# DS4SD/MarkushGrapher

Hardware: AMD Instinct MI355X
Metric: images/sec whole-node (greedy CXSMILES decode, 1024px crops, bs=32/GPU) (higher is better)
Workload: dtype bf16

## Files before the change

include/mgrapher.h:

```cpp
#ifndef MGRAPHER_H
#define MGRAPHER_H
#include <stddef.h>
#include <stdint.h>
#ifdef __cplusplus
extern "C" {
#endif

enum { MG_OK = 0, MG_E_SHAPE = -1, MG_E_ARG = -2, MG_E_STATE = -3, MG_E_HIP = -4, MG_E_UNSUPPORTED = -5,
       MG_E_WORKSPACE = -6, MG_E_KEY = -7, MG_E_INPUT = -8 };
enum { MG_KEY_IGNORED = 1 };
enum { MG_F32 = 0, MG_BF16 = 1 };

typedef struct mg_config {
    int vocab_size, d_model, d_kv, d_ff, num_layers, num_decoder_layers, num_heads;
    int relative_attention_num_buckets, relative_attention_max_distance;
    int max_2d_position_embeddings, image_size, patch_size, num_channels;
    int pad_token_id, eos_token_id, decoder_start_token_id;
    float layer_norm_epsilon;
    int max_decode_len;
    int tie_word_embeddings;
} mg_config;

typedef struct mg_model mg_model;

int mg_create(const mg_config* cfg, mg_model** out);
void mg_destroy(mg_model* m);
const char* mg_last_error(void);

size_t mg_weights_bytes(const mg_model* m);
int mg_bind_weights(mg_model* m, void* arena);
int mg_load_tensor(mg_model* m, void* stream, const char* hf_key, const void* src, int dtype, const int64_t* shape,
                   int ndim);
int mg_finalize(mg_model* m, void* stream);

int mg_clone(const mg_model* src, mg_model** out);

int mg_workspace_bytes(const mg_model* m, int B, int L, int num_beams, int max_length, int T, int M_e1, size_t* out_bytes);

int mg_encode(mg_model* m, void* stream, void* ws, size_t ws_bytes, const int64_t* input_ids, const float* bbox,
              const uint8_t* attention_mask, const float* pixel_values, const float* e1, int M_e1, int B, int L,
              float* enc_out, uint8_t* enc_mask);

int mg_decoder_forward(mg_model* m, void* stream, void* ws, size_t ws_bytes, const int64_t* decoder_input_ids,
                       const uint8_t* decoder_attention_mask, int B, int T, float* logits);

int mg_generate(mg_model* m, void* stream, void* ws, size_t ws_bytes, const int64_t* input_ids, const float* bbox,
                const uint8_t* attention_mask, const float* pixel_values, const float* e1 ,
                int M_e1, int B, int L, int num_beams, int max_length,
                int min_length, float length_penalty, int early_stopping, int64_t* out_ids, int* out_cols_host,
                float* out_scores, float* step_top2);

typedef struct mg_gen_opts {
    int num_return;
    float* token_scores;
    float* seq_scores;
    int32_t* beam_indices;
} mg_gen_opts;
int mg_generate_scored(mg_model* m, void* stream, void* ws, size_t ws_bytes, const int64_t* input_ids, const float* bbox,
                       const uint8_t* attention_mask, const float* pixel_values, const float* e1, int M_e1, int B, int L, int num_beams,
                       int max_length, int min_length, float length_penalty, int early_stopping, int64_t* out_ids, int* out_cols_host,
                       float* out_scores, float* step_top2, const mg_gen_opts* opts);


typedef struct mg_sample_opts {
    float temperature;
    int top_k;
    float top_p;
    uint64_t seed;
    const uint64_t* stream_ids;
    int num_return;
    float* token_scores;
} mg_sample_opts;
int mg_sampled_workspace_bytes(const mg_model* m, int B, int L, int num_return, int max_length, int M_e1, size_t* out_bytes);
int mg_generate_sampled(mg_model* m, void* stream, void* ws, size_t ws_bytes, const int64_t* input_ids, const float* bbox,
                        const uint8_t* attention_mask, const float* pixel_values, const float* e1, int M_e1, int B, int L, int max_length,
                        int min_length, int64_t* out_ids, int* out_cols_host, float* step_top2, const mg_sample_opts* opts);

int mg_stream_workspace_bytes(const mg_model* m, int chunk, int L, int slots, int pool_chunks, size_t* out_bytes);
int mg_generate_stream(mg_model* m, void* stream, void* ws, size_t ws_bytes, const int64_t* input_ids, const float* bbox,
                       const uint8_t* attention_mask, const float* pixel_values, int N, int L, int chunk, int slots, int pool_chunks,
                       int max_length, int min_length, int64_t* out_ids, int32_t* out_len, long* steps_host);
int mg_generate_stream_sampled(mg_model* m, void* stream, void* ws, size_t ws_bytes, const int64_t* input_ids, const float* bbox,
                               const uint8_t* attention_mask, const float* pixel_values, int N, int L, int chunk, int slots,
                               int pool_chunks, int max_length, int min_length, int64_t* out_ids, int32_t* out_len, long* steps_host,
                               const mg_sample_opts* opts);
int mg_stream_beam_workspace_bytes(const mg_model* m, int chunk, int L, int slots, int pool_chunks, int num_beams, int max_length, size_t* out_bytes);
int mg_generate_stream_beam(mg_model* m, void* stream, void* ws, size_t ws_bytes, const int64_t* input_ids, const float* bbox,
                            const uint8_t* attention_mask, const float* pixel_values, int N, int L, int chunk, int slots, int pool_chunks,
                            int num_beams, int max_length, int min_length, float length_penalty, int early_stopping, int64_t* out_ids,
                            int32_t* out_len, float* out_scores, long* steps_host);
int mg_generate_stream_scored(mg_model* m, void* stream, void* ws, size_t ws_bytes, const int64_t* input_ids, const float* bbox,
                              const uint8_t* attention_mask, const float* pixel_values, int N, int L, int chunk, int slots, int pool_chunks,
                              int max_length, int min_length, int64_t* out_ids, int32_t* out_len, long* steps_host, const mg_gen_opts* opts);
int mg_generate_stream_beam_scored(mg_model* m, void* stream, void* ws, size_t ws_bytes, const int64_t* input_ids, const float* bbox,
                                   const uint8_t* attention_mask, const float* pixel_values, int N, int L, int chunk, int slots, int pool_chunks,
                                   int num_beams, int max_length, int min_length, float length_penalty, int early_stopping, int64_t* out_ids,
                                   int32_t* out_len, long* steps_host, const mg_gen_opts* opts);
int mg_stream_encoder_mode(mg_model* m, int mode, const uint32_t* cu_mask, int nwords);

int mg_debug_decode_capture(mg_model* m, float* logits_capture, int capture_steps, const int64_t* forced_ids);

int mg_beam_reorder(void* stream, const void* kv_src, void* kv_dst, const int32_t* beam_idx, int layers, int rows,
                    int H, int t_cap, int t_used);

int mg_profile_cross_attention(mg_model* m, int every, int max_samples);
int mg_profile_read(mg_model* m, long* launches_host, double* total_ms_host, double* total_keys_host);
int mg_profile_read_overhead(mg_model* m, double* empty_ms_host);
int mg_profile_phases(mg_model* m, int enable);
int mg_profile_phases_read(mg_model* m, long* calls_host, double* enc_ms_host, double* dec_ms_host);
int mg_debug_bucket_table(const mg_model* m, int which, int* out_host, int n);

int mg_set_decode_graph(mg_model* m, int enable);
int mg_set_padding_semantics(mg_model* m, int per_image);
int mg_set_shared_gpu(mg_model* m, int shared);
int mg_set_cross_absorb(mg_model* m, int absorb, int key_splits);
int mg_set_beam_cross_absorb(mg_model* m, int absorb, int key_splits);
int mg_decode_graph_active(const mg_model* m);

typedef struct mg_dist mg_dist;
int mg_dist_unique_id(void* out, int bytes);
int mg_dist_create(const void* unique_id, int bytes, int rank, int world, mg_dist** out);
int mg_dist_allgather(mg_dist* d, void* stream, const void* send, void* recv, size_t bytes_per_rank);
void mg_dist_destroy(mg_dist* d);

size_t mg_preprocess_scratch_bytes(int B, int Hs, int Ws, int out_size);
int mg_preprocess_pages(void* stream, const uint8_t* pages_u8, int B, int Hs, int Ws, int out_size, float* pixel_values,
                        void* scratch, size_t scratch_bytes);

int mg_selftest(void* stream, void* scratch_256k, char* msg_host, int msg_len);

int mgk_pack_weight(void* stream, const void* src, int src_is_bf16, int N, int K, void* dst_pk, int Npad);
int mgk_rmsnorm_pack(void* stream, const float* h, const float* gain, void* x_pk, float* out_f32, int M, int d,
                     float eps, float scale);
int mgk_im2col_pack(void* stream, const float* pix, void* x_pk, int B, int C, int I, int ps);
int mgk_set_rows_split(int mode);
int mgk_set_resid_f16(int on);
int mgk_set_rows_ft2(int mode);
int mgk_set_rows_mt(int on);
int mgk_set_attention_qt(int qt);
int mgk_set_pp_parts(int mode);
int mgk_gemm_resid_mt(void* stream, const void* X_pk, const void* W_pk, float* h, const float* gain, float gscale, void* x_pk,
                      float* part, int M, int N, int K, const float* rs_part, int rs_nparts, float rs_inv_d, float rs_eps, int wide_tiles,
                      float* kpart, int* ticket);
int mgk_gemm(void* stream, int mode, int epi, const void* X_pk, const void* W_pk, int M, int N, int K, float* out_f32,
             int ldo, const float* bias, void* out_pk);
int mgk_gemm_norm(void* stream, int epi, const void* X_pk, const void* W_pk, int M, int N, int K, float* h_tiled, const float* gain,
                  void* out_pk, float* part, int part_ld, const float* rs_part, int rs_nparts, float rs_inv_d, float rs_eps);
int mgk_gemm_row_tiles(void* stream, int epi, const void* X_pk, const void* W_pk, int M, int N, int K, float* out_f32, const float* gain,
                       void* out_pk, float* part, int part_ld, const float* rs_part, int rs_nparts, float rs_inv_d, float rs_eps,
                       const uint8_t* row_mask, int* list_scratch);
int mgk_gemm_heads(void* stream, int mode, const void* X_pk, const void* W_pk, int M, int N, int K, void* p0, void* p1,
                   void* p2, int f0, int f1, int f2, int H, int S_in, int S_cap, const int* row_map, int pos);
int mgk_attention(void* stream, int mode, const void* Q, const void* K, const void* Vt, void* ctx_pk, int B, int H,
                  int Sq, int Sk, int Sq_cap, int Sk_cap, const uint8_t* kmask, const float* tab1, int tab1_len,
                  const float* tabh, const float* tabv, const double* cx, const double* cy, const int* bk1, const int* bkhv,
                  void* bidx_scratch);
int mgk_attention_enc_skip(void* stream, const void* Q, const void* K, const void* Vt, void* ctx_pk, int B, int H, int S, int S_cap,
                           const uint8_t* kmask, const float* tab1, const float* tabh, const float* tabv, const double* cx,
                           const double* cy, const int* bk1, const int* bkhv, void* bidx_scratch, int* kst_scratch,
                           uint8_t* qbv_scratch);
int mgk_attention_step(void* stream, const void* q, const void* Kc, const void* Vc, void* ctx_pk, int rows, int H,
                       int group, int cap, const int* len, int n_keys, const float* bias, const int* anc, int t);
int mgk_attention_step_ex(void* stream, const void* q, const void* Kc, const void* Vc, void* ctx_pk, int rows, int H, int group, int cap,
                          const int* len, int n_keys, const float* bias, const int* anc, int t, const int* t_dev, int t_off,
                          const int* pos_rows, const int* kv_owner, const int* live, const float* qrs_part, int qrs_nparts, float qrs_inv_d,
                          float qrs_eps, int ctx_ld, int ctx_col0, int one_wg_per_cu);
int mgk_attention_step_rope(void* stream, const float* qkv, int ld, const float* cs, const float* rs_part, int rs_nparts, float rs_inv_d,
                            float rs_eps, float qscale, void* Kc, void* Vc, void* ctx_pk, int rows, int H_kv, int group, int cap, int t,
                            const int* t_dev, int t_off, const int* pos_rows, const int* t_off_rows, const int* kv_owner, const int* live,
                            int ctx_ld, int ctx_col0);
int mgk_xattn(void* stream, const void* q, const float* wkv, const void* enc, const int* len, const int* kv_owner, int rows, int H, int d,
              int cap, int nsplit, int nstg, void* wk, void* wv, void* qx, void* part, float* ml, void* ctx_pk);
int mgk_xattn_beams(void* stream, const void* q, const float* wkv, const void* enc, const int* len, const int* kv_owner, const int* live,
                    int rows, int H, int d, int cap, int group, int nsplit, int nstg, int beams_per_wg, int nt, void* wk, void* wv, void* qx,
                    void* part, float* ml, void* ctx_pk);
int mgk_enc_rows(void* stream, const void* src_pk, const int* row_map, void* dst, int B, int rows_per_image, int cap, int d);
int mgk_embed_assemble(void* stream, void* meta_ws, const int64_t* input_ids, const float* bbox,
                       const uint8_t* attention_mask, const float* patch_emb, const void* tok_emb, const void* x_emb,
                       const void* y_emb, int B, int L, int P, int d, int n_side, int M2, int V, int S_cap,
                       float* hidden, double* cx, double* cy, uint8_t* mask, int* xrow, int* xlen, int* err);
size_t mgk_embed_meta_bytes(int B, int S_cap);
int mgk_greedy_select(void* stream, const float* logits, int rows, int V, int ldl, int eos, int pad, int min_len,
                      int64_t* next_ids, int64_t* out_ids, int max_len, int pos, int* unfinished, int* n_unfinished,
                      float* top2);

int mgk_sample_select(void* stream, const float* logits, int rows, int V, int ldl, int eos, int pad, int min_len, float temperature,
                      int top_k, float top_p, uint64_t seed, const uint64_t* stream_ids, int64_t* next_ids, int64_t* out_ids, int max_len,
                      int pos, int* unfinished, int* n_unfinished, float* token_scores, int ts_ld);
int mgk_philox(uint64_t seed, uint64_t stream_id, uint32_t pos, uint32_t* out_host);
typedef struct mgk_slot_table {
    int* pos; int* img; int* pool; int* ctr; int* out_len;
    int pool_cap, start_id;
    const int64_t* first_tok;
    int n_stop, stop[4], max_len, nsamp;
} mgk_slot_table;
typedef struct mgk_select_desc {
    int fused;
    const float* logits; int rows, V, ldl;
    int eos, pad, suppress_eos, n_eos_more, eos_more[3];
    int64_t* next_ids; int64_t* out_ids; int max_len, pos;
    const int* pos_dev;
    int min_len;
    int* unfinished; int* n_unfinished;
    float* top2;
    int* step_ctr;
    mgk_slot_table slots;
    const void* ptop; const float* stopv; int ntiles;
    const void* tok_emb; float* h; const float* gain; void* x_pk; void* x2_pk; int x2_ld, x2_col0, d; float eps;
    float* token_scores; int ts_ld;
} mgk_select_desc;
int mgk_select_ex(void* stream, const mgk_select_desc* s);
int mgk_sample_select_queue(void* stream, const float* logits, int rows, int V, int ldl, int eos, int pad, int min_len, float temperature,
                            int top_k, float top_p, uint64_t seed, const uint64_t* stream_ids, int64_t* next_ids, int64_t* out_ids, int max_len,
                            int pos, int* unfinished, int* n_unfinished, float* token_scores, int ts_ld, const mgk_slot_table* slots);
int mgk_slot_refill(void* stream, const mgk_slot_table* slots, int64_t* next_ids, int* unfinished, int rows);

int mgk_swin_attention(void* stream, const void* qkv_pk, void* ctx_pk, const float* table_HT, int B, int R, int C, int H, int w, int shift);
int mgk_swin_layernorm(void* stream, const float* h_in, int in_tiled, float* h_out, int h_out_norm, const float* w, const float* b,
                       const float* add_bias, void* x_pk, float* out_f32, int M, int C, int merge_R, float eps, int kaug);
int mgk_swin_resize(void* stream, const float* src, float* dst, int B, int C, int S, int I, const float* scale_host, const float* shift_host);
int mgk_swin_im2col_pack(void* stream, const float* pix, void* x_pk, int B, int C, int I, int ps, int Kp);
int mgk_swin_transpose(void* stream, const float* src, float* dst, int n, int H);

int mgk_ocr_layernorm_pack(void* stream, float* h, const float* w, const float* b, const float* add_bias, void* x_pk, float* out_f32, int M,
                           int d, int Kaug, float eps);
int mgk_ocr_gelu_pack(void* stream, const float* in, void* y_pk, int M, int N, int Kaug);
int mgk_ocr_silu_mul_pack(void* stream, const float* in, void* y_pk, int M, int I);
int mgk_ocr_silu_mul_rows(void* stream, const float* in, const float* rs_part, int rs_nparts, float rs_inv_d, float rs_eps, void* y_pk, int M,
                          int I);
int mgk_ocr_add_pos(void* stream, const float* patch, const void* pos, const int* pos_ids, const uint8_t* patch_mask, uint8_t* vmask,
                    float* hidden, int N, int P, int P_cap, int d);
int mgk_ocr_pixel_shuffle_pack(void* stream, const float* vis, void* x_pk, int N, int g, int P_cap, int e, int sf);
int mgk_ocr_merge_embed(void* stream, const int64_t* ids, const void* tok_emb, const float* feats, float* h, int B, int L, int T_cap, int d,
                        int V, int image_token, int per_seq, int* err);
int mgk_ocr_rope_heads(void* stream, const float* qkv, int B, int T, int T_cap, int H, int KV, float theta, void* Q, void* K, void* Vt, void* Kc,
                       void* Vc, int cap);
int mgk_ocr_rope_table(void* stream, float* cs, int positions, float theta);
int mgk_ocr_pack_aug(void* stream, const float* W, const float* bias, float scale, void* dst_pk, int row0, int N, int K, int Kaug, int Nfill,
                     int rstride);
int mgk_ocr_tile_f32(void* stream, const float* src, float* dst, int M, int d, int to_tiled);
int mgk_ocr_row_maps(void* stream, int* last_rows, int* all_rows, uint8_t* key_mask, int B, int T, int T_cap, const int* lens);
int mgk_ocr_len_delta(void* stream, const int* lens, int* delta, int N, int L, int* err);
int mgk_gemm_swiglu(void* stream, const void* X_pk, int x_kts, int x_k0, const void* W_pk, int M, int N, int K, const float* rs_part,
                    int rs_nparts, float rs_inv_d, float rs_eps, void* out_pk, int out_ld, int out_col0);
int mgk_rmsnorm_pack_tiled(void* stream, const float* h_tiled, const float* gain, void* x_pk, float* out_f32, int M, int d, float eps);
int mgk_embed_norm_rows(void* stream, const int64_t* ids, const void* tok_emb, float* h, const float* gain, void* x_pk, void* x2_pk, int x2_ld,
                        int x2_col0, int rows, int d, int V, int* err, float eps);

int mgk_gemm_splitk(void* stream, const void* X_pk, const void* W_pk, float* P, int M, int N, int K, int ldp,
                    size_t slab_stride, int KS);
int mgk_splitk_factor(int N, int K);
int mgk_gemm_set_variant(int v);
int mgk_gemm_resid(void* stream, const void* X_pk, const void* W_pk, float* h, const float* gain, float gscale, void* x_pk,
                   float* part, int M, int N, int K, const float* rs_part, int rs_nparts, float rs_inv_d, float rs_eps);
int mgk_gemm_pair(void* stream, const void* Wn_pk, const void* Wr_pk, const float* gain, int N2, int d, int inner, void* W2_pk,
                  float* scratch_f32, const void* xwin_pk, float* h, void* hb_out_pk, float* part, void* out2_pk, int M, int relu);
typedef struct mgk_resid_desc {
    const void* X; int x_kts, x_k0;
    const void* W;
    float* h;
    const float* gain; float gscale;
    void* x_pk; int x_ld, x_col0;
    void* x2_pk; int x2_ld, x2_col0;
    float* part;
    int M, N, K;
    const float* rs_part; int rs_nparts; float rs_inv_d, rs_eps;
    int wide_tiles, alone;
    float* kpart; int* ticket;
} mgk_resid_desc;
typedef struct mgk_proj_desc {
    const void* X; int x_kts, x_k0;
    const void* W;
    int N, K;
    const float* rs_part; int rs_nparts; float rs_inv_d, rs_eps;
    int both_halves;
    void* q;
    void* out_pk;
    float* out_f32; int ldo;
} mgk_proj_desc;
int mgk_gemm_resid_ex(void* stream, const mgk_resid_desc* r);
int mgk_gemm_pair_ex(void* stream, const mgk_resid_desc* r, const mgk_proj_desc* g, int epi);
int mgk_gemm_heads_step(void* stream, const void* X_pk, int x_kts, int x_k0, const void* W_pk, int M, int N, int K, void* p0, void* p1, void* p2,
                        int f0, int f1, int f2, int H, int S_cap, const float* rs_part, int rs_nparts, float rs_inv_d, float rs_eps, int pos,
                        const int* pos_dev, const int* pos_rows, int both_halves);
int mgk_lm_head_step(void* stream, const void* X_pk, const void* W_pk, float* P, int M, int N, int K, int ldp, const float* rs_part, int rs_nparts,
                     float rs_inv_d, float rs_eps, void* ptop, float* stopv, const int* stop4_host, int write_logits, int lse);
int mgk_add_norm_pack(void* stream, float* h, const float* P, int KS, int ldp, size_t slab_stride, const float* gain,
                      void* x_pk, int M, int d, float eps, float scale);
int mgk_relu_pack(void* stream, const float* P, int KS, int ldp, size_t slab_stride, void* y_pk, int M, int N);
size_t mgk_beam_state_bytes(int B, int K, int max_len);
float mgk_beam_length_divisor(int cur_len, float length_penalty);
int mgk_beam_init(void* stream, void* state, int B, int K, int max_len, int pad, int eos, int start, int64_t* next_ids, int* anc, int T_cap,
                  int* counters);
int mgk_beam_step(void* stream, void* state, const float* logits, int ldl, int V, int B, int K, int max_len, int cur_len, const int* tdev,
                  const float* div_table, int eos, int min_len, float length_penalty, int early_stopping, int64_t* next_ids, int* beam_idx,
                  int* counters, const int* slot_pos, const int* slot_live);
int mgk_beam_reorder_anc(void* stream, int* anc, const int* beam_idx, int rows, int t_written, const int* tdev, const int* counters,
                         const int* slot_pos, const int* slot_live);
int mgk_beam_finalize(void* stream, void* state, int B, int K, int max_len, int64_t* out_ids, int* out_cols, float* out_scores, int num_return,
                      int* beam_indices, float* token_scores);
int mgk_beam_slots_step(void* stream, void* state, int slots, int K, int max_len, int pad, int eos, int start, int early_stopping, int* pos,
                        int* img, int* pool, int* bpool, int* live, int* assign, int64_t* next_ids, int* anc, int T_cap, int pool_cap,
                        int64_t* out_ids, int* out_len, float* out_scores, int* ctr, int end_first, int num_return, int* beam_indices,
                        float* token_scores);

typedef struct mg_ocr_model mg_ocr_model;
typedef struct mg_ocr_config {
    int v_hidden, v_inter, v_layers, v_heads, image_size, patch_size;
    int t_hidden, t_inter, t_layers, t_heads, t_kv_heads, vocab;
    int scale_factor, image_token_id, eos_token_id, pad_token_id, tie_word_embeddings;
    float v_eps, rms_eps, rope_theta;
    int n_eos_extra, eos_extra[3];
} mg_ocr_config;

int mg_ocr_create(const mg_ocr_config* cfg, mg_ocr_model** out);
void mg_ocr_destroy(mg_ocr_model* m);
int mg_ocr_clone(const mg_ocr_model* src, mg_ocr_model** out);
size_t mg_ocr_weights_bytes(const mg_ocr_model* m);
int mg_ocr_bind_weights(mg_ocr_model* m, void* arena);
int mg_ocr_load_tensor(mg_ocr_model* m, void* stream, const char* hf_key, const void* src, int src_is_bf16, const int64_t* shape, int ndim);
int mg_ocr_finalize(mg_ocr_model* m, void* stream);
int mg_ocr_workspace_bytes(const mg_ocr_model* m, int B, int n_img, int L, int max_new_tokens, int full_logits, size_t* out_bytes);
int mg_ocr_image_features(mg_ocr_model* m, void* stream, void* ws, size_t ws_bytes, const float* pixel_values, const int32_t* patch_pos,
                          const uint8_t* patch_mask, int N, float* out);
int mg_ocr_forward(mg_ocr_model* m, void* stream, void* ws, size_t ws_bytes, const int64_t* input_ids, const float* pixel_values,
                   const int32_t* patch_pos, const uint8_t* patch_mask, int B, int n_img, int L, float* logits);
int mg_ocr_generate(mg_ocr_model* m, void* stream, void* ws, size_t ws_bytes, const int64_t* input_ids, const float* pixel_values,
                    const int32_t* patch_pos, const uint8_t* patch_mask, int B, int n_img, int L, int max_new_tokens, int64_t* out_ids,
                    int* out_cols_host, float* step_logits, int capture_steps);

int mg_ocr_stream_workspace_bytes(const mg_ocr_model* m, int N, int n_img, int L, int max_new_tokens, int slots, int chunk, size_t* out_bytes);
int mg_ocr_generate_stream(mg_ocr_model* m, void* stream, void* ws, size_t ws_bytes, const int64_t* input_ids, const float* pixel_values,
                           const int32_t* patch_pos, const uint8_t* patch_mask, int N, int n_img, int L, int max_new_tokens, int slots, int chunk,
                           int64_t* out_ids, int32_t* out_len, long* steps_host);
int mg_ocr_generate_stream_ragged(mg_ocr_model* m, void* stream, void* ws, size_t ws_bytes, const int64_t* input_ids, const int32_t* prompt_len,
                                  const float* pixel_values, const int32_t* patch_pos, const uint8_t* patch_mask, int N, int n_img, int L,
                                  int max_new_tokens, int slots, int chunk, int64_t* out_ids, int32_t* out_len, long* steps_host);

typedef struct mg_e1_model mg_e1_model;
typedef struct mg_e1_config {
    int image_size, patch_size, num_channels, embed_dim, n_stages;
    int depths[4], num_heads[4];
    int window_size, mlp_ratio;
    float layer_norm_eps;
    int n_proj, proj_dims[4], proj_act;
    int src_image_size;
    float pix_scale[3], pix_shift[3];
} mg_e1_config;

int mg_e1_create(const mg_e1_config* cfg, mg_e1_model** out);
void mg_e1_destroy(mg_e1_model* m);
size_t mg_e1_weights_bytes(const mg_e1_model* m);
int mg_e1_bind_weights(mg_e1_model* m, void* arena);
int mg_e1_load_tensor(mg_e1_model* m, void* stream, const char* key, const void* src, int src_is_bf16, const int64_t* shape, int ndim);
int mg_e1_finalize(mg_e1_model* m, void* stream);
int mg_e1_out_tokens(const mg_e1_model* m);
int mg_e1_workspace_bytes(const mg_e1_model* m, int B, size_t* out_bytes);
int mg_e1_encode(const mg_e1_model* m, void* stream, void* ws, size_t ws_bytes, const float* pixel_values, int B, float* e1_out,
                 float* features_out);
int mg_attach_e1(mg_model* m, const mg_e1_model* e1);

#ifdef __cplusplus
}
#endif
#endif
```

markushgrapher_amd/csrc/c_ops.hip:

```cpp
#include "mg_kernels.h"
#include "mg_swin.h"
#include "mg_ocr.h"
#include <stdlib.h>
#include "../../include/mgrapher.h"

using namespace mg;

extern "C" {

int mgk_pack_weight(void* stream, const void* src, int src_is_bf16, int N, int K, void* dst_pk, int Npad) {
    if ((K & 15) || (Npad & 31) || Npad < N) return MG_E_SHAPE;
    pack_weight(src, src_is_bf16, N, K, (uint16_t*)dst_pk, Npad, (mgStream_t)stream);
    return MG_OK;
}

int mgk_rmsnorm_pack(void* stream, const float* h, const float* gain, void* x_pk, float* out_f32, int M, int d,
                     float eps, float scale) {
    if (d & 15) return MG_E_SHAPE;
    rmsnorm_pack(h, gain, (uint16_t*)x_pk, out_f32, M, d, eps, scale, (mgStream_t)stream);
    return MG_OK;
}

int mgk_im2col_pack(void* stream, const float* pix, void* x_pk, int B, int C, int I, int ps) {
    if ((ps & 7) || (I % ps)) return MG_E_SHAPE;
    im2col_pack(pix, (uint16_t*)x_pk, B, C, I, ps, (mgStream_t)stream);
    return MG_OK;
}

int mgk_set_rows_split(int mode) { gemm_rows_set_split(mode); return MG_OK; }
int mgk_set_resid_f16(int on) { gemm_rows_set_resid_f16(on); return MG_OK; }
int mgk_set_rows_ft2(int mode) { gemm_rows_set_ft2(mode); return MG_OK; }
int mgk_gemm(void* stream, int mode, int epi, const void* X_pk, const void* W_pk, int M, int N, int K, float* out_f32,
             int ldo, const float* bias, void* out_pk) {
    const bool swin_epi = epi == EPI_PK_BIAS || epi == EPI_PK_GELU_ERF;
    if ((K & 63) || epi < 0 || (epi > EPI_PK && epi != EPI_PK_GELU && !swin_epi)) return MG_E_SHAPE;
    if (epi == EPI_PK_GELU && !(mode == 0 && gemm_has_gelu_epilogue(M, N))) return MG_E_UNSUPPORTED;
    if (swin_epi && mode != 0) return MG_E_UNSUPPORTED;
    if (swin_epi && ((N & 15) || !out_pk)) return MG_E_SHAPE;
    GemmArgs a{};
    a.X = (const uint16_t*)X_pk; a.W = (const uint16_t*)W_pk; a.M = M; a.N = N; a.K = K;
    a.out_f32 = out_f32; a.ldo = ldo; a.bias = bias; a.out_pk = (uint16_t*)out_pk;
    if (mode == 0) gemm(a, epi, (mgStream_t)stream); else gemm_rows(a, epi, (mgStream_t)stream);
    return MG_OK;
}

int mgk_gemm_norm(void* stream, int epi, const void* X_pk, const void* W_pk, int M, int N, int K, float* h_tiled, const float* gain,
                  void* out_pk, float* part, int part_ld, const float* rs_part, int rs_nparts, float rs_inv_d, float rs_eps) {
    const bool plain_resid = epi == EPI_RESID_NORM && !gain && !out_pk && !part && !rs_part;
    if ((K & 63) || (N & 31) || ((M & 31) && !plain_resid) || M < 1) return MG_E_SHAPE;
    GemmArgs a{};
    a.X = (const uint16_t*)X_pk; a.W = (const uint16_t*)W_pk; a.M = M; a.N = N; a.K = K;
    a.out_f32 = h_tiled; a.gain = gain; a.out_pk = (uint16_t*)out_pk; a.part = part; a.ldo = part_ld;
    a.rs = RowScale{rs_part, rs_nparts, rs_inv_d, rs_eps};
    gemm(a, epi, (mgStream_t)stream);
    return MG_OK;
}

int mgk_gemm_row_tiles(void* stream, int epi, const void* X_pk, const void* W_pk, int M, int N, int K, float* out_f32, const float* gain,
                       void* out_pk, float* part, int part_ld, const float* rs_part, int rs_nparts, float rs_inv_d, float rs_eps,
                       const uint8_t* row_mask, int* list_scratch) {
    if ((K & 63) || (N & 31) || (M & 31) || !row_mask || !list_scratch) return MG_E_SHAPE;
    row_tile_list(row_mask, M, list_scratch + 1, list_scratch, (mgStream_t)stream);
    GemmArgs a{};
    a.X = (const uint16_t*)X_pk; a.W = (const uint16_t*)W_pk; a.M = M; a.N = N; a.K = K;
    a.out_f32 = out_f32; a.gain = gain; a.out_pk = (uint16_t*)out_pk; a.part = part; a.ldo = (epi == EPI_RESID_NORM) ? part_ld : N;
    a.rs = RowScale{rs_part, rs_nparts, rs_inv_d, rs_eps};
    a.row_tiles = list_scratch + 1; a.n_row_tiles = list_scratch;
    gemm(a, epi, (mgStream_t)stream);
    return MG_OK;
}

int mgk_gemm_heads(void* stream, int mode, const void* X_pk, const void* W_pk, int M, int N, int K, void* p0, void* p1,
                   void* p2, int f0, int f1, int f2, int H, int S_in, int S_cap, const int* row_map, int pos) {
    if ((K & 63) || (N % (H * 64))) return MG_E_SHAPE;
    GemmArgs a{};
    a.X = (const uint16_t*)X_pk; a.W = (const uint16_t*)W_pk; a.M = M; a.N = N; a.K = K;
    a.heads.ptr[0] = (uint16_t*)p0; a.heads.ptr[1] = (uint16_t*)p1; a.heads.ptr[2] = (uint16_t*)p2;
    a.heads.fmt[0] = f0; a.heads.fmt[1] = f1; a.heads.fmt[2] = f2;
    a.heads.inner = H * 64; a.heads.H = H; a.heads.S_in = S_in; a.heads.S_cap = S_cap; a.heads.row_map = row_map;
    a.heads.pos = pos;
    if (mode == 0) gemm(a, EPI_HEADS, (mgStream_t)stream); else gemm_rows(a, EPI_HEADS, (mgStream_t)stream);
    return MG_OK;
}

int mgk_gemm_heads_step(void* stream, const void* X_pk, int x_kts, int x_k0, const void* W_pk, int M, int N, int K, void* p0, void* p1, void* p2,
                        int f0, int f1, int f2, int H, int S_cap, const float* rs_part, int rs_nparts, float rs_inv_d, float rs_eps, int pos,
                        const int* pos_dev, const int* pos_rows, int both_halves) {
    if (!X_pk || !W_pk) return MG_E_ARG;
    if (K < 64 || (K & 63) || H < 1 || N < H * 64 || (N % (H * 64)) || N > 3 * H * 64 || M < 1 || M > 256 || S_cap < 1) return MG_E_SHAPE;
    if (x_kts ? (x_k0 < 0 || x_k0 + (K >> 4) > x_kts) : x_k0 != 0) return MG_E_SHAPE;
    if (rs_part && (rs_nparts < 8 || (rs_nparts & 7))) return MG_E_SHAPE;
    void* const ptr[3] = {p0, p1, p2};
    const int fmt[3] = {f0, f1, f2};
    bool kv = false;
    for (int i = 0; i < 3; ++i) {
        if (fmt[i] != HF_NONE && fmt[i] != HF_STEP_Q && fmt[i] != HF_STEP_KV) return MG_E_UNSUPPORTED;
        if (i < N / (H * 64) && fmt[i] != HF_NONE && !ptr[i]) return MG_E_ARG;
        kv = kv || fmt[i] == HF_STEP_KV;
    }
    if (kv && !pos_dev && !pos_rows && (pos < 0 || pos >= S_cap)) return MG_E_SHAPE;
    GemmArgs a{};
    a.X = (const uint16_t*)X_pk; a.x_kts = x_kts; a.x_k0 = x_k0; a.W = (const uint16_t*)W_pk; a.M = M; a.N = N; a.K = K;
    for (int i = 0; i < 3; ++i) { a.heads.ptr[i] = (uint16_t*)ptr[i]; a.heads.fmt[i] = fmt[i]; }
    a.heads.inner = H * 64; a.heads.H = H; a.heads.S_in = M; a.heads.S_cap = S_cap;
    a.heads.pos = pos; a.heads.pos_dev = pos_dev; a.heads.pos_rows = pos_rows;
    a.rs = RowScale{rs_part, rs_nparts, rs_inv_d, rs_eps};
    a.both_halves = both_halves;
    gemm_rows(a, EPI_HEADS, (mgStream_t)stream);
    return MG_OK;
}

int mgk_attention(void* stream, int mode, const void* Q, const void* K, const void* Vt, void* ctx_pk, int B, int H,
                  int Sq, int Sk, int Sq_cap, int Sk_cap, const uint8_t* kmask, const float* tab1, int tab1_len,
                  const float* tabh, const float* tabv, const double* cx, const double* cy, const int* bk1, const int* bkhv,
                  void* bidx_scratch) {
    if ((Sq_cap & 31) || (Sk_cap & 63) || Sk > Sk_cap || Sq > Sq_cap || mode < 0 || mode > 2) return MG_E_SHAPE;
    AttnArgs a{};
    a.Q = (const uint16_t*)Q; a.K = (const uint16_t*)K; a.Vt = (const uint16_t*)Vt; a.ctx = (uint16_t*)ctx_pk;
    a.B = B; a.H = H; a.Sq = Sq; a.Sk = Sk; a.Sq_cap = Sq_cap; a.Sk_cap = Sk_cap; a.mode = mode; a.kmask = kmask;
    a.tab1 = tab1; a.tab1_len = tab1_len; a.tabh = tabh; a.tabv = tabv;
    if (mode == ATT_ENC) {
        if (!bidx_scratch || !bk1 || !bkhv || !cx || !cy || Sq_cap != Sk_cap) return MG_E_ARG;
        bias_index((uint16_t*)bidx_scratch, cx, cy, kmask, bk1, bkhv, B, Sk, Sk_cap, (mgStream_t)stream);
        a.bidx = (const uint16_t*)bidx_scratch;
        a.bk1 = bk1;
    }
    attention(a, (mgStream_t)stream);
    return MG_OK;
}

int mgk_attention_enc_skip(void* stream, const void* Q, const void* K, const void* Vt, void* ctx_pk, int B, int H, int S, int S_cap,
                           const uint8_t* kmask, const float* tab1, const float* tabh, const float* tabv, const double* cx,
                           const double* cy, const int* bk1, const int* bkhv, void* bidx_scratch, int* kst_scratch,
                           uint8_t* qbv_scratch) {
    if ((S_cap & 63) || S > S_cap || !kmask || !bidx_scratch || !kst_scratch || !qbv_scratch) return MG_E_ARG;
    AttnArgs a{};
    a.Q = (const uint16_t*)Q; a.K = (const uint16_t*)K; a.Vt = (const uint16_t*)Vt; a.ctx = (uint16_t*)ctx_pk;
    a.B = B; a.H = H; a.Sq = S; a.Sk = S; a.Sq_cap = S_cap; a.Sk_cap = S_cap; a.mode = ATT_ENC; a.kmask = kmask;
    a.tab1 = tab1; a.tab1_len = 32; a.tabh = tabh; a.tabv = tabv;
    bias_index((uint16_t*)bidx_scratch, cx, cy, kmask, bk1, bkhv, B, S, S_cap, (mgStream_t)stream);
    attn_lists(kmask, B, S, S_cap, kst_scratch, qbv_scratch, (mgStream_t)stream);
    a.bidx = (const uint16_t*)bidx_scratch; a.bk1 = bk1; a.kst = kst_scratch; a.qbv = qbv_scratch;
    attention(a, (mgStream_t)stream);
    return MG_OK;
}

int mgk_attention_step(void* stream, const void* q, const void* Kc, const void* Vc, void* ctx_pk, int rows, int H,
                       int group, int cap, const int* len, int n_keys, const float* bias, const int* anc, int t) {
    if (group < 1 || group > 8) return MG_E_SHAPE;
    AttnStepArgs a{};
    a.q = (const uint16_t*)q; a.Kc = (const uint16_t*)Kc; a.Vc = (const uint16_t*)Vc; a.ctx = (uint16_t*)ctx_pk;
    a.rows = rows; a.H = H; a.group = group; a.cap = cap; a.len = len; a.n_keys = n_keys; a.bias = bias; a.anc = anc;
    a.t = t;
    attention_step(a, (mgStream_t)stream);
    return MG_OK;
}

int mgk_attention_step_ex(void* stream, const void* q, const void* Kc, const void* Vc, void* ctx_pk, int rows, int H, int group, int cap,
                          const int* len, int n_keys, const float* bias, const int* anc, int t, const int* t_dev, int t_off,
                          const int* pos_rows, const int* kv_owner, const int* live, const float* qrs_part, int qrs_nparts, float qrs_inv_d,
                          float qrs_eps, int ctx_ld, int ctx_col0, int one_wg_per_cu) {
    if (group < 1 || group > 8 || rows < 1) return MG_E_SHAPE;
    if (ctx_ld ? ((ctx_ld & 15) || ctx_col0 < 0 || ctx_col0 + H * 64 > ctx_ld) : ctx_col0 != 0) return MG_E_SHAPE;
    if (one_wg_per_cu) attention_step_allow_shared();
    AttnStepArgs a{};
    a.q = (const uint16_t*)q; a.Kc = (const uint16_t*)Kc; a.Vc = (const uint16_t*)Vc; a.ctx = (uint16_t*)ctx_pk;
    a.rows = rows; a.H = H; a.group = group; a.cap = cap; a.len = len; a.n_keys = n_keys; a.bias = bias; a.anc = anc;
    a.t = t; a.t_dev = t_dev; a.t_off = t_off; a.pos_rows = pos_rows; a.kv_owner = kv_owner; a.live = live;
    a.qrs = RowScale{qrs_part, qrs_nparts, qrs_inv_d, qrs_eps};
    a.ctx_ld = ctx_ld; a.ctx_col0 = ctx_col0; a.one_wg_per_cu = one_wg_per_cu;
    attention_step(a, (mgStream_t)stream);
    return MG_OK;
}

int mgk_attention_step_rope(void* stream, const float* qkv, int ld, const float* cs, const float* rs_part, int rs_nparts, float rs_inv_d,
                            float rs_eps, float qscale, void* Kc, void* Vc, void* ctx_pk, int rows, int H_kv, int group, int cap, int t,
                            const int* t_dev, int t_off, const int* pos_rows, const int* t_off_rows, const int* kv_owner, const int* live,
                            int ctx_ld, int ctx_col0) {
    if (group < 1 || group > 8 || group == 5 || group == 7 || rows < 1) return MG_E_SHAPE;
    if (!qkv || !cs || ld < (group + 2) * H_kv * 64 || (ld & 3)) return MG_E_ARG;
    if (ctx_ld ? ((ctx_ld & 15) || ctx_col0 < 0 || ctx_col0 + H_kv * group * 64 > ctx_ld) : ctx_col0 != 0) return MG_E_SHAPE;
    AttnStepArgs a{};
    a.Kc = (const uint16_t*)Kc; a.Vc = (const uint16_t*)Vc; a.Kc_w = (uint16_t*)Kc; a.Vc_w = (uint16_t*)Vc; a.ctx = (uint16_t*)ctx_pk;
    a.rows = rows; a.H = H_kv; a.group = group; a.cap = cap; a.n_keys = t + 1; a.t = t; a.t_dev = t_dev; a.t_off = t_off;
    a.pos_rows = pos_rows; a.t_off_rows = t_off_rows; a.kv_owner = kv_owner; a.live = live;
    a.rope.qkv = qkv; a.rope.ld = ld; a.rope.cs = cs; a.rope.rs = RowScale{rs_part, rs_nparts, rs_inv_d, rs_eps}; a.rope.qscale = qscale;
    a.ctx_ld = ctx_ld; a.ctx_col0 = ctx_col0;
    attention_step(a, (mgStream_t)stream);
    return MG_OK;
}

#ifdef MG_TOOLS
int mgk_attention_step_trace(void* stream, const void* q, const void* Kc, const void* Vc, void* ctx_pk, int rows, int H, int cap,
                             const int* len, long long* trace) {
    AttnStepArgs a{};
    a.q = (const uint16_t*)q; a.Kc = (const uint16_t*)Kc; a.Vc = (const uint16_t*)Vc; a.ctx = (uint16_t*)ctx_pk;
    a.rows = rows; a.H = H; a.group = 1; a.cap = cap; a.len = len;
    attention_step_trace(a, trace, (mgStream_t)stream);
    return MG_OK;
}
#endif

int mgk_xattn(void* stream, const void* q, const float* wkv, const void* enc, const int* len, const int* kv_owner, int rows, int H, int d,
              int cap, int nsplit, int nstg, void* wk, void* wv, void* qx, void* part, float* ml, void* ctx_pk) {
    if (!xattn_supported(d, H) || nsplit < 1 || nsplit > 4 || (nstg != 3 && nstg != 4)) return MG_E_UNSUPPORTED;
    mgStream_t st = (mgStream_t)stream;
    xattn_pack_weights(wkv, (uint16_t*)wk, (uint16_t*)wv, H, d, st);
    xattn_stream_prepare(d, nstg);
    XAttnArgs a{};
    a.q = (const uint16_t*)q; a.qx = (uint16_t*)qx; a.wk = (const uint16_t*)wk; a.wv = (const uint16_t*)wv; a.enc = (const uint16_t*)enc;
    a.len = len; a.kv_owner = kv_owner; a.part = (uint16_t*)part; a.ml = ml; a.ctx = (uint16_t*)ctx_pk;
    a.rows = rows; a.H = H; a.d = d; a.cap = cap; a.nsplit = nsplit; a.nstg = nstg;
    { const char* e = getenv("MG_XATTN_NT"); a.nt = e ? atoi(e) : 1; }
    xattn_expand(a, st);
    xattn_stream(a, st);
    xattn_contract(a, st);
    return MG_OK;
}
int mgk_xattn_beams(void* stream, const void* q, const float* wkv, const void* enc, const int* len, const int* kv_owner, const int* live,
                    int rows, int H, int d, int cap, int group, int nsplit, int nstg, int beams_per_wg, int nt, void* wk, void* wv, void* qx,
                    void* part, float* ml, void* ctx_pk) {
    if (!xattn_supported(d, H) || nsplit < 1 || nsplit > 4 || (nstg != 3 && nstg != 4)) return MG_E_UNSUPPORTED;
    if (group < 1 || rows < group || rows % group != 0 || beams_per_wg < 0 || !xattn_beams_bp(d, nstg, beams_per_wg)) return MG_E_UNSUPPORTED;
    mgStream_t st = (mgStream_t)stream;
    xattn_pack_weights(wkv, (uint16_t*)wk, (uint16_t*)wv, H, d, st);
    xattn_beams_prepare(d);
    XAttnArgs a{};
    a.q = (const uint16_t*)q; a.qx = (uint16_t*)qx; a.wk = (const uint16_t*)wk; a.wv = (const uint16_t*)wv; a.enc = (const uint16_t*)enc;
    a.len = len; a.kv_owner = kv_owner; a.live = live; a.part = (uint16_t*)part; a.ml = ml; a.ctx = (uint16_t*)ctx_pk;
    a.rows = rows; a.H = H; a.d = d; a.cap = cap; a.nsplit = nsplit; a.nstg = nstg; a.nt = nt ? 1 : 0; a.group = group; a.bpw = beams_per_wg;
    xattn_expand(a, st);
    xattn_stream_beams(a, st);
    xattn_contract(a, st);
    return MG_OK;
}
int mgk_enc_rows(void* stream, const void* src_pk, const int* row_map, void* dst, int B, int rows_per_image, int cap, int d) {
    enc_rows((const uint16_t*)src_pk, row_map, (uint16_t*)dst, B, rows_per_image, cap, d, (mgStream_t)stream);
    return MG_OK;
}

size_t mgk_embed_meta_bytes(int B, int S_cap) { return embed_meta_bytes(B, S_cap); }

int mgk_embed_assemble(void* stream, void* meta_ws, const int64_t* input_ids, const float* bbox,
                       const uint8_t* attention_mask, const float* patch_emb, const void* tok_emb, const void* x_emb,
                       const void* y_emb, int B, int L, int P, int d, int n_side, int M2, int V, int S_cap,
                       float* hidden, double* cx, double* cy, uint8_t* mask, int* xrow, int* xlen, int* err) {
    if (S_cap < L + P || (d & 3) || P != n_side * n_side) return MG_E_SHAPE;
    EmbedArgs a{};
    a.input_ids = input_ids; a.bbox = bbox; a.attn_mask = attention_mask; a.patch_emb = patch_emb;
    a.tok_emb = (const uint16_t*)tok_emb; a.x_emb = (const uint16_t*)x_emb; a.y_emb = (const uint16_t*)y_emb;
    a.B = B; a.L = L; a.P = P; a.d = d; a.n_side = n_side; a.M2 = M2; a.V = V; a.S_cap = S_cap;
    a.hidden = hidden; a.cx = cx; a.cy = cy; a.mask = mask; a.xrow = xrow; a.xlen = xlen; a.err = err;
    embed_assemble(a, meta_ws, (mgStream_t)stream);
    return MG_OK;
}

int mgk_greedy_select(void* stream, const float* logits, int rows, int V, int ldl, int eos, int pad, int min_len,
                      int64_t* next_ids, int64_t* out_ids, int max_len, int pos, int* unfinished, int* n_unfinished,
                      float* top2) {
    ArgmaxArgs a{};
    a.logits = logits; a.rows = rows; a.V = V; a.ldl = ldl; a.eos = eos; a.pad = pad; a.min_len = min_len;
    a.next_ids = next_ids; a.out_ids = out_ids; a.max_len = max_len; a.pos = pos; a.unfinished = unfinished;
    a.n_unfinished = n_unfinished; a.top2 = top2;
    mg_memset_async(n_unfinished, 0, sizeof(int), (mgStream_t)stream);
    greedy_select(a, (mgStream_t)stream);
    return MG_OK;
}

int mgk_greedy_select_scored(void* stream, const float* logits, int rows, int V, int ldl, int eos, int pad, int min_len,
                             int64_t* next_ids, int64_t* out_ids, int max_len, int pos, int* unfinished, int* n_unfinished,
                             float* token_scores, int ts_ld) {
    ArgmaxArgs a{};
    a.logits = logits; a.rows = rows; a.V = V; a.ldl = ldl; a.eos = eos; a.pad = pad; a.min_len = min_len;
    a.next_ids = next_ids; a.out_ids = out_ids; a.max_len = max_len; a.pos = pos; a.unfinished = unfinished;
    a.n_unfinished = n_unfinished; a.token_scores = token_scores; a.ts_ld = ts_ld;
    mg_memset_async(n_unfinished, 0, sizeof(int), (mgStream_t)stream);
    greedy_select(a, (mgStream_t)stream);
    return MG_OK;
}

int mgk_sample_select(void* stream, const float* logits, int rows, int V, int ldl, int eos, int pad, int min_len, float temperature,
                      int top_k, float top_p, uint64_t seed, const uint64_t* stream_ids, int64_t* next_ids, int64_t* out_ids, int max_len,
                      int pos, int* unfinished, int* n_unfinished, float* token_scores, int ts_ld) {
    if (!logits || !next_ids || !out_ids || !unfinished || !n_unfinished || rows < 1 || ldl < V || (ldl & 3)) return MG_E_ARG;
    if (!(temperature > 0.f) || top_k < 0 || !(top_p >= 0.f)) return MG_E_ARG;
    if (!sample_select_supported(V)) return MG_E_UNSUPPORTED;
    SampleArgs a{};
    a.logits = logits; a.rows = rows; a.V = V; a.ldl = ldl; a.eos = eos; a.pad = pad; a.min_len = min_len;
    a.temperature = temperature; a.top_k = top_k; a.top_p = top_p; a.seed = seed; a.stream_ids = stream_ids;
    a.next_ids = next_ids; a.out_ids = out_ids; a.max_len = max_len; a.pos = pos; a.unfinished = unfinished;
    a.n_unfinished = n_unfinished; a.token_scores = token_scores; a.ts_ld = ts_ld;
    mg_memset_async(n_unfinished, 0, sizeof(int), (mgStream_t)stream);
    sample_select(a, (mgStream_t)stream);
    return MG_OK;
}

static SlotTable slot_table(const mgk_slot_table* t) {
    SlotTable s{};
    if (!t) return s;
    s.pos = t->pos; s.img = t->img; s.pool = t->pool; s.ctr = t->ctr; s.out_len = t->out_len; s.pool_cap = t->pool_cap; s.start_id = t->start_id;
    s.first_tok = t->first_tok; s.n_stop = t->n_stop; s.max_len = t->max_len; s.nsamp = t->nsamp;
    for (int k = 0; k < 4; ++k) s.stop[k] = t->stop[k];
    return s;
}
int mgk_select_ex(void* stream, const mgk_select_desc* s) {
    if (!s || !s->next_ids || !s->out_ids || !s->unfinished) return MG_E_ARG;
    const bool queue = s->slots.pos != nullptr;
    if (s->fused && queue) return MG_E_ARG;
    if (queue ? (!s->slots.img || !s->slots.ctr || !s->slots.out_len) : !s->n_unfinished) return MG_E_ARG;
    if (s->n_eos_more < 0 || s->n_eos_more > 3) return MG_E_ARG;
    if (s->rows < 1 || s->rows > 256 || s->V < 1 || s->max_len < 1 || s->pos < 0) return MG_E_SHAPE;
    if (s->token_scores && (s->ts_ld < s->max_len - 1 || (!queue && !s->pos_dev && s->pos < 1))) return MG_E_SHAPE;
    if (s->fused) {
        if (!s->ptop || !s->stopv || !s->tok_emb || !s->gain || !s->h || !s->x_pk) return MG_E_ARG;
        if (s->d < 16 || s->d > 2048 || (s->d & 15) || s->ntiles != (s->V + 31) / 32) return MG_E_SHAPE;
        if (s->pad < 0 || s->pad >= s->V) return MG_E_ARG;
        if (s->x2_pk && ((s->x2_ld & 15) || s->x2_col0 < 0 || (s->x2_col0 & 7) || s->x2_col0 + s->d > s->x2_ld)) return MG_E_SHAPE;
    } else {
        if (!s->logits) return MG_E_ARG;
        if (s->ldl < s->V || (s->ldl & 3)) return MG_E_SHAPE;
    }
    ArgmaxArgs a{};
    a.logits = s->logits; a.rows = s->rows; a.V = s->V; a.ldl = s->ldl; a.eos = s->eos; a.pad = s->pad; a.suppress_eos = s->suppress_eos;
    a.n_eos_more = s->n_eos_more;
    for (int k = 0; k < 3; ++k) a.eos_more[k] = s->eos_more[k];
    a.next_ids = s->next_ids; a.out_ids = s->out_ids; a.max_len = s->max_len; a.pos = s->pos; a.pos_dev = s->pos_dev; a.min_len = s->min_len;
    a.unfinished = s->unfinished; a.n_unfinished = s->n_unfinished; a.top2 = s->top2; a.step_ctr = s->step_ctr;
    if (queue) a.slots = slot_table(&s->slots);
    a.ptop = (const float4*)s->ptop; a.stopv = s->stopv; a.ntiles = s->ntiles; a.tok_emb = (const uint16_t*)s->tok_emb; a.h = s->h;
    a.gain = s->gain; a.x_pk = (uint16_t*)s->x_pk; a.x2_pk = (uint16_t*)s->x2_pk; a.x2_ld = s->x2_ld; a.x2_col0 = s->x2_col0; a.d = s->d;
    a.eps = s->eps; a.token_scores = s->token_scores; a.ts_ld = s->ts_ld;
    if (s->fused) greedy_select_fused(a, (mgStream_t)stream); else greedy_select(a, (mgStream_t)stream);
    return MG_OK;
}
// ... 412 lines not shown
```

markushgrapher_amd/csrc/k_gemm.hip:

```cpp
#include "k_gemm_epi.h"
#include <atomic>

namespace mg {

constexpr int GB_M = 128, GB_N = 128, GB_K = 64;
constexpr int GB_STAGE_BYTES = (GB_M + GB_N) / 32 * (GB_K / 16) * TILE_BYTES;

template <int EPI>
__global__ __launch_bounds__(256) void gemm_big_kernel(GemmArgs a) {
    MG_DYN_SMEM(smem);
    const int tid = threadIdx.x, lane = tid & 63, w = tid >> 6;
    const int nbn = (a.N + GB_N - 1) / GB_N;
    const int nbm = (a.M + GB_M - 1) / GB_M;
    int bid = blockIdx.x;
    const int nblk = nbm * nbn;
    if ((nblk & 7) == 0) bid = (bid & 7) * (nblk >> 3) + (bid >> 3);
    const int bm = bid / nbn, bn = bid - bm * nbn;
    const int mt32 = (a.M + 31) >> 5, nt32 = (a.N + 31) >> 5, kt16 = a.K >> 4;
    const int nks = a.K / GB_K;

    const char* src[8];
#pragma unroll
    for (int i = 0; i < 8; ++i) {
        const int f = w * 8 + i, ff = f & 15, rt = ff >> 2, kt = ff & 3;
// ... 172 lines not shown
                tile_epilogue<EPI, false>(a, acc[i][j], m0, n0, lane);
            } else if constexpr (EPI == EPI_HEADS) {
                if (tor) tile_epilogue<EPI_HEADS, true, true>(a, acc[i][j], m0, n0, lane, 3, rsv[i]);
                else tile_epilogue<EPI_HEADS, false, true>(a, acc[i][j], m0, n0, lane, 3, rsv[i]);
            } else if constexpr (EPI != EPI_RESID_NORM) {
                tile_epilogue<EPI, true, true>(a, acc[i][j], m0, n0, lane, 3, rsv[i]);
            }
        }
}



template <int EPI, int TI, int XP = 0>
__global__ __launch_bounds__(512) void gemm_xl_kernel(GemmArgs a) {
    MG_DYN_SMEM(smem);
    constexpr int BM = 64 * TI, XT = 2 * TI;
    constexpr int FRAGS = (XT + 8) * 4;
    constexpr int STAGE_BYTES = FRAGS * TILE_BYTES;
    constexpr int PER_WAVE = (FRAGS + 7) / 8;
    const int tid = threadIdx.x, lane = tid & 63, w = tid >> 6;
    const int nbn = (a.N + GX_N - 1) / GX_N;
    const int n_list = a.row_tiles ? *a.n_row_tiles : 0;
    const int M_run = a.row_tiles ? n_list * 32 : a.M;
    const int nbm = (M_run + BM - 1) / BM;
    int bid = blockIdx.x;
    const int nblk = nbm * nbn;
    if (bid >= nblk) return;
    if ((nblk & 7) == 0) bid = (bid & 7) * (nblk >> 3) + (bid >> 3);
    const int bm = bid / nbn, bn = bid - bm * nbn;
    const int mt32 = (a.M + 31) >> 5, nt32 = (a.N + 31) >> 5;
    const int nks = a.K / GX_K;

    const char* src[PER_WAVE];
#pragma unroll
    for (int i = 0; i < PER_WAVE; ++i) {
        int f = w * PER_WAVE + i;
        f = f < FRAGS ? f : FRAGS - 1;
        const bool isW = f >= 4 * XT;
        const int ff = isW ? f - 4 * XT : f, rt = ff >> 2, kt = ff & 3;
        int trow = isW ? (bn * 8 + rt) : (bm * XT + rt);
        if (!isW && a.row_tiles) trow = a.row_tiles[trow < n_list ? trow : n_list - 1];
        const int tmax = isW ? nt32 - 1 : mt32 - 1;
        trow = trow < tmax ? trow : tmax;
        src[i] = (const char*)((isW ? a.W : a.X) + pk_tile_off(trow, kt, a.K)) + lane * 16;
    }
    const mg_lds_t sm0 = mg_lds_addr(smem);
    auto stage = [&](int buf, int ks) {
#pragma unroll
        for (int i = 0; i < PER_WAVE; ++i)
            if (w * PER_WAVE + i < FRAGS)
                glds16_async_lds(src[i] + (size_t)ks * (4 * TILE_BYTES), sm0 + buf * STAGE_BYTES + (w * PER_WAVE + i) * TILE_BYTES);
    };

    const int wr = w >> 2, wc = w & 3;
    const int m0w = bm * BM + wr * (32 * TI), n0w = bn * GX_N + wc * 64;
    bool tor;
    if (EPI == EPI_F32_STORE || EPI == EPI_F32_RESID) tor = false;
    else if (EPI == EPI_HEADS) tor = !heads_region_is_T(a.heads, n0w < a.N ? n0w : 0);
    else tor = true;

    f32x16 acc[TI][2];
#pragma unroll
    for (int i = 0; i < TI; ++i)
#pragma unroll
        for (int j = 0; j < 2; ++j) acc[i][j] = acc_zero();

    struct Frags { mg_raw16 x[TI], w[2]; };
    const mg_lds_t lx0 = sm0 + lane * 16 + wr * (TI * 4 * TILE_BYTES);
    const mg_lds_t lw0 = sm0 + lane * 16 + (4 * XT + wc * 8) * TILE_BYTES;
    auto rd = [&](int buf, auto ktc, Frags& f) {
        constexpr int kt = (XP & 1) ? 0 : decltype(ktc)::value;
        const mg_lds_t lx = lx0 + buf * STAGE_BYTES, lw = lw0 + buf * STAGE_BYTES;
        lds_rd16_async<(0 * 4 + kt) * TILE_BYTES>(f.w[0], lw);
        lds_rd16_async<(1 * 4 + kt) * TILE_BYTES>(f.w[1], lw);
        lds_rd16_async<(0 * 4 + kt) * TILE_BYTES>(f.x[0], lx);
        lds_rd16_async<(1 * 4 + kt) * TILE_BYTES>(f.x[1], lx);
        lds_rd16_async<(2 * 4 + kt) * TILE_BYTES>(f.x[2], lx);
        lds_rd16_async<(3 * 4 + kt) * TILE_BYTES>(f.x[3], lx);
        if constexpr (TI > 4) lds_rd16_async<(4 * 4 + kt) * TILE_BYTES>(f.x[TI - 1], lx);
    };
    auto landed = [&](Frags& f) {
        MG_WAIT_LGKM_TIE(0, f.w[0]);
        MG_TIE(f.w[1]);
#pragma unroll
        for (int i = 0; i < TI; ++i) MG_TIE(f.x[i]);
    };
    auto mm = [&](const Frags& f) {
        uint4 xw[2], xx[TI];
#pragma unroll
        for (int j = 0; j < 2; ++j) xw[j] = raw16_get(f.w[j]);
#pragma unroll
        for (int i = 0; i < TI; ++i) xx[i] = raw16_get(f.x[i]);
        if (tor) {
#pragma unroll
            for (int i = 0; i < TI; ++i)
#pragma unroll
                for (int j = 0; j < 2; ++j) acc[i][j] = mfma32(xw[j], xx[i], acc[i][j]);
        } else {
#pragma unroll
            for (int i = 0; i < TI; ++i)
#pragma unroll
                for (int j = 0; j < 2; ++j) acc[i][j] = mfma32(xx[i], xw[j], acc[i][j]);
        }
    };
    Frags fa, fb;
    using K0 = std::integral_constant<int, 0>; using K1 = std::integral_constant<int, 1>;
    using K2 = std::integral_constant<int, 2>; using K3 = std::integral_constant<int, 3>;
    stage(0, 0);
    MG_WAIT_VMCNT(0);
    MG_BARRIER_RAW();
    if (nks > 1) stage(1, 1);
    rd(0, K0{}, fa);
    for (int ks = 0; ks < nks; ++ks) {
        const int cur = ks & 1;
        landed(fa);
        rd(cur, K1{}, fb);
        MG_SCHED_FENCE();
        mm(fa);
        MG_SCHED_FENCE();
        landed(fb);
        rd(cur, K2{}, fa);
        MG_SCHED_FENCE();
        mm(fb);
        MG_SCHED_FENCE();
        landed(fa);
        rd(cur, K3{}, fb);
        MG_SCHED_FENCE();
        mm(fa);
        MG_SCHED_FENCE();
        landed(fb);
        if (ks + 1 < nks) {
            MG_WAIT_VMCNT(0);
            MG_BARRIER_RAW();
            if (ks + 2 < nks && !(XP & 2)) stage(cur, ks + 2);
            rd(cur ^ 1, K0{}, fa);
        }
        MG_SCHED_FENCE();
        mm(fb);
        MG_SCHED_FENCE();
    }

    int mrow[TI];
#pragma unroll
    for (int i = 0; i < TI; ++i) {
        if (a.row_tiles) {
            const int e = bm * XT + wr * TI + i;
            mrow[i] = e < n_list ? a.row_tiles[e] * 32 : a.M;
        } else {
            mrow[i] = m0w + 32 * i;
        }
    }
    xl_epilogue<EPI, TI, XP>(a, acc, mrow, n0w, tor, lane);
}
template <int EPI, int TI>
static void launch_xl(const GemmArgs& a, mgStream_t stream) {
    constexpr int BM = 64 * TI;
    const int nblk = ((a.M + BM - 1) / BM) * ((a.N + GX_N - 1) / GX_N);
    const size_t sh = (size_t)2 * (2 * TI + 8) * 4 * TILE_BYTES;
    static bool once = false;
    if (!once) { MG_SET_MAX_SMEM((&gemm_xl_kernel<EPI, TI>), sh); once = true; }
#ifdef MG_TOOLS
    if constexpr (EPI == EPI_PK && TI == 5) {
        static int xp = -1;
        if (xp < 0) { const char* e = getenv("MG_GEMM_EXP"); xp = e ? atoi(e) : 0; }
        if (xp) {
#define MG_XP(N) case N: { static bool o = false; if (!o) { MG_SET_MAX_SMEM((&gemm_xl_kernel<EPI, TI, N>), sh); o = true; } \
                             MG_LAUNCH((gemm_xl_kernel<EPI, TI, N>), dim3(nblk), dim3(512), sh, stream, a); } break;
            switch (xp) { MG_XP(1) MG_XP(2) MG_XP(3) MG_XP(4) MG_XP(5) MG_XP(6) default: MG_XP(7) }
#undef MG_XP
            return;
        }
    }
#endif
    MG_LAUNCH((gemm_xl_kernel<EPI, TI>), dim3(nblk), dim3(512), sh, stream, a);
}

template <int EPI>
static void launch_wide(const GemmArgs& a, mgStream_t stream) {
    const int nblk = ((a.M + GW_M - 1) / GW_M) * ((a.N + GW_N - 1) / GW_N);
    const size_t sh = (size_t)GW_STAGES * GW_STAGE_BYTES;
    static bool once = false;
    if (!once) { MG_SET_MAX_SMEM(&gemm_wide_kernel<EPI>, sh); once = true; }
    MG_LAUNCH((gemm_wide_kernel<EPI>), dim3(nblk), dim3(512), sh, stream, a);
}

static std::atomic<int> g_gemm_variant{3};
void gemm_set_variant(int v) { g_gemm_variant = v; }

bool gemm_has_gelu_epilogue(int M, int N) { return g_gemm_variant >= 2 && M >= 320 && N >= GX_N; }

void gemm(const GemmArgs& a, int epi, mgStream_t stream) {
    static bool env_read = false;
    if (!env_read) { env_read = true; if (const char* e = getenv("MG_GEMM_VARIANT")) g_gemm_variant = atoi(e); }
    const int gv = g_gemm_variant;
    static int small_env = -1;
    if (small_env < 0) { const char* e = getenv("MG_GEMM_SMALL"); small_env = e ? atoi(e) : 256; if (small_env == 1) small_env = 256; }
    const long tiles_xl = (long)((a.M + 319) / 320) * ((a.N + GX_N - 1) / GX_N);
    const bool small = gv == 3 && small_env && tiles_xl < small_env && epi != EPI_PK_GELU && !a.row_tiles && !a.part && !a.gain && !a.rs.part;
    if (!small && (gv == 3 || gv == 5 || gv == 6) && a.M >= 320 && a.N >= GX_N) {
        if (gemm_pp(a, epi, gv == 5 ? 4 : 5, stream)) return;
    }
    if (!small && gv >= 2 && a.M >= 320 && a.N >= GX_N) {
        const bool five = gv >= 3;
        const bool four = gv == 2;
        if (five) {
            switch (epi) {
                case EPI_F32_STORE: launch_xl<EPI_F32_STORE, 5>(a, stream); break;
                case EPI_F32_RESID: launch_xl<EPI_F32_RESID, 5>(a, stream); break;
                case EPI_PK_RELU: launch_xl<EPI_PK_RELU, 5>(a, stream); break;
                case EPI_PK_GELU: launch_xl<EPI_PK_GELU, 5>(a, stream); break;
                case EPI_PK: launch_xl<EPI_PK, 5>(a, stream); break;
                case EPI_PK_BIAS: launch_xl<EPI_PK_BIAS, 5>(a, stream); break;
                case EPI_PK_GELU_ERF: launch_xl<EPI_PK_GELU_ERF, 5>(a, stream); break;
                case EPI_RESID_NORM: launch_xl<EPI_RESID_NORM, 5>(a, stream); break;
                default: launch_xl<EPI_HEADS, 5>(a, stream); break;
            }
            return;
        }
        if (four) {
            switch (epi) {
                case EPI_F32_STORE: launch_xl<EPI_F32_STORE, 4>(a, stream); break;
                case EPI_F32_RESID: launch_xl<EPI_F32_RESID, 4>(a, stream); break;
                case EPI_PK_RELU: launch_xl<EPI_PK_RELU, 4>(a, stream); break;
                case EPI_PK_GELU: launch_xl<EPI_PK_GELU, 4>(a, stream); break;
                case EPI_PK: launch_xl<EPI_PK, 4>(a, stream); break;
                case EPI_PK_BIAS: launch_xl<EPI_PK_BIAS, 4>(a, stream); break;
                case EPI_PK_GELU_ERF: launch_xl<EPI_PK_GELU_ERF, 4>(a, stream); break;
                case EPI_RESID_NORM: launch_xl<EPI_RESID_NORM, 4>(a, stream); break;
                default: launch_xl<EPI_HEADS, 4>(a, stream); break;
            }
            return;
        }
    }
    const long tiles_w = (long)((a.M + GW_M - 1) / GW_M) * ((a.N + GW_N - 1) / GW_N);
    if (gv >= 1 && a.M >= GW_M && !(small && tiles_w < 96)) {
        switch (epi) {
            case EPI_F32_STORE: launch_wide<EPI_F32_STORE>(a, stream); break;
            case EPI_F32_RESID: launch_wide<EPI_F32_RESID>(a, stream); break;
            case EPI_PK_RELU: launch_wide<EPI_PK_RELU>(a, stream); break;
            case EPI_PK: launch_wide<EPI_PK>(a, stream); break;
            case EPI_PK_BIAS: launch_wide<EPI_PK_BIAS>(a, stream); break;
            case EPI_PK_GELU_ERF: launch_wide<EPI_PK_GELU_ERF>(a, stream); break;
            case EPI_RESID_NORM: launch_wide<EPI_RESID_NORM>(a, stream); break;
            default: launch_wide<EPI_HEADS>(a, stream); break;
        }
        return;
    }
    const int nblk = ((a.M + GB_M - 1) / GB_M) * ((a.N + GB_N - 1) / GB_N);
    const dim3 grid(nblk), block(256);
    const size_t sh = 2 * GB_STAGE_BYTES;
    switch (epi) {
        case EPI_F32_STORE: MG_LAUNCH((gemm_big_kernel<EPI_F32_STORE>), grid, block, sh, stream, a); break;
        case EPI_F32_RESID: MG_LAUNCH((gemm_big_kernel<EPI_F32_RESID>), grid, block, sh, stream, a); break;
        case EPI_PK_RELU: MG_LAUNCH((gemm_big_kernel<EPI_PK_RELU>), grid, block, sh, stream, a); break;
        case EPI_PK: MG_LAUNCH((gemm_big_kernel<EPI_PK>), grid, block, sh, stream, a); break;
        case EPI_PK_BIAS: MG_LAUNCH((gemm_big_kernel<EPI_PK_BIAS>), grid, block, sh, stream, a); break;
        case EPI_PK_GELU_ERF: MG_LAUNCH((gemm_big_kernel<EPI_PK_GELU_ERF>), grid, block, sh, stream, a); break;
        case EPI_RESID_NORM: MG_LAUNCH((gemm_big_kernel<EPI_RESID_NORM>), grid, block, sh, stream, a); break;
        default: MG_LAUNCH((gemm_big_kernel<EPI_HEADS>), grid, block, sh, stream, a); break;
    }
}

static std::atomic<int> g_rows_split_mode{-1};
void gemm_rows_set_split(int mode) { g_rows_split_mode = mode; }
static int rows_split_tiles(int mt, size_t weight_elems) {
    static bool env_read = false;
    if (!env_read) { env_read = true; if (const char* e = getenv("MG_ROWS_SPLIT")) g_rows_split_mode = atoi(e); }
    if (mt <= 1 || g_rows_split_mode == 0) return mt;
    const bool small = weight_elems * sizeof(uint16_t) <= ((size_t)4 << 20);
    return (g_rows_split_mode == 1 || (g_rows_split_mode < 0 && small)) ? 1 : mt;
}
template <int EPI>
MG_DEV void shift_rows(GemmArgs& a, int rt) {
    if (rt == 0) return;
    const int xkts = a.x_kts ? a.x_kts : (a.K >> 4);
    a.X += (size_t)rt * xkts * TILE_ELEMS;
    if (a.out_f32) a.out_f32 += (size_t)rt * 32 * a.ldo;
    if (a.out_pk) a.out_pk += (size_t)rt * ((EPI == EPI_PK_SWIGLU ? (a.out_ld ? a.out_ld : a.N >> 1) : a.N) >> 4) * TILE_ELEMS;
    if constexpr (EPI == EPI_HEADS) {
#pragma unroll
        for (int ri = 0; ri < 3; ++ri) {
            if (!a.heads.ptr[ri]) continue;
            if (a.heads.fmt[ri] == HF_STEP_Q) a.heads.ptr[ri] += (size_t)rt * 32 * a.heads.H * 64;
            else if (a.heads.fmt[ri] == HF_STEP_KV && !a.heads.row_map) a.heads.ptr[ri] += (size_t)rt * 32 * a.heads.H * (size_t)a.heads.S_cap * 64;
        }
        if (a.heads.row_map) a.heads.row_map += 32 * rt;
        if (a.heads.pos_rows) a.heads.pos_rows += 32 * rt;
    }
    if (a.rs.part) a.rs.part += (size_t)rt * 32 * a.rs.nparts;
    a.M -= 32 * rt;
}
MG_DEV void shift_rows(ResidArgs& a, int rt) {
    if (rt == 0) return;
    const int xkts = a.x_kts ? a.x_kts : (a.K >> 4);
    a.X += (size_t)rt * xkts * TILE_ELEMS;
    a.h += (size_t)rt * 32 * a.N;
    if (a.x_pk) a.x_pk += (size_t)rt * ((a.x_ld ? a.x_ld : a.N) >> 4) * TILE_ELEMS;
    if (a.x2_pk) a.x2_pk += (size_t)rt * ((a.x2_ld ? a.x2_ld : a.N) >> 4) * TILE_ELEMS;
    if (a.part) a.part += (size_t)rt * 32 * (a.N >> 3);
    if (a.rs.part) a.rs.part += (size_t)rt * 32 * a.rs.nparts;
    a.M -= 32 * rt;
}

template <int EPI, int MT, bool HALF, int NW, int U>
MG_DEV void rows_block(const GemmArgs& a, int bid, char* smem) {
    const int tid = threadIdx.x, lane = tid & 63, w = tid >> 6;
    const int nt = HALF ? (bid >> 1) : bid;
    const int sub = HALF ? (bid & 1) : 0;
    const bool wvalid = !HALF || (((lane & 31) >> 4) == sub);
    const uint4 zero4 = make_uint4(0, 0, 0, 0);
    const int kt16 = a.K >> 4;
    const int per = (kt16 + NW - 1) / NW;
    const int k0 = w * per, k1 = (k0 + per) < kt16 ? (k0 + per) : kt16;
    constexpr bool TOR = !(EPI == EPI_F32_STORE || EPI == EPI_F32_RESID);
    float* rsl = (float*)(smem + NW * 16 * 64 * sizeof(float));
    const char* wp = (const char*)(a.W + pk_tile_off(nt, 0, a.K)) + lane * 16;
    const int xkts = a.x_kts ? a.x_kts : kt16;
    const char* xp = (const char*)a.X + ((size_t)a.x_k0 * TILE_BYTES + lane * 16);
    int kt = k0;
    uint4 wf[U];
    const bool first_full = kt + U <= k1;
    if (first_full) {
#pragma unroll
        for (int u = 0; u < U; ++u) wf[u] = wvalid ? ld16_stream(wp + (size_t)(kt + u) * TILE_BYTES) : zero4;
    }
    if (TOR) block_row_scales(a.rs, a.M, 32 * MT, rsl, tid, NW * 64);

    f32x16 acc[MT];
#pragma unroll
    for (int i = 0; i < MT; ++i) acc[i] = acc_zero();
    for (bool first = true; kt + U <= k1; kt += U, first = false) {
        if (!first) {
#pragma unroll
            for (int u = 0; u < U; ++u) wf[u] = wvalid ? ld16_stream(wp + (size_t)(kt + u) * TILE_BYTES) : zero4;
        }
#pragma unroll
        for (int u = 0; u < U; ++u) {
#pragma unroll
            for (int i = 0; i < MT; ++i) {
                const uint4 xf = ld16(xp + ((size_t)i * xkts + (kt + u)) * TILE_BYTES);
                acc[i] = TOR ? mfma32(wf[u], xf, acc[i]) : mfma32(xf, wf[u], acc[i]);
            }
        }
    }
    for (; kt < k1; ++kt) {
        const uint4 wf = wvalid ? ld16_stream(wp + (size_t)kt * TILE_BYTES) : zero4;
#pragma unroll
        for (int i = 0; i < MT; ++i) {
            const uint4 xf = ld16(xp + ((size_t)i * xkts + kt) * TILE_BYTES);
            acc[i] = TOR ? mfma32(wf, xf, acc[i]) : mfma32(xf, wf, acc[i]);
        }
    }
    float* slab = (float*)smem;
#pragma unroll
    for (int i = 0; i < MT; ++i) {
#pragma unroll
        for (int r = 0; r < 16; ++r) slab[(w * 16 + r) * 64 + lane] = acc[i][r];
        __syncthreads();
        if constexpr (TOR && !HALF) {
#pragma unroll
            for (int q = 0; q < 2; ++q) {
                if (((2 * i + q) % NW) == w) {
                    f32x16 s = acc_zero();
#pragma unroll
                    for (int r = 8 * q; r < 8 * q + 8; ++r) {
                        float v = 0.f;
#pragma unroll
                        for (int ww = 0; ww < NW; ++ww) v += slab[(ww * 16 + r) * 64 + lane];
                        s[r] = v * rsl[32 * i + (lane & 31)];
                    }
                    tile_epilogue<EPI, TOR>(a, s, 32 * i, 32 * nt, lane, 1 << q);
                }
            }
        } else if ((i % NW) == w) {
            f32x16 s;
#pragma unroll
            for (int r = 0; r < 16; ++r) {
                float v = 0.f;
#pragma unroll
                for (int ww = 0; ww < NW; ++ww) v += slab[(ww * 16 + r) * 64 + lane];
                s[r] = TOR ? v * rsl[32 * i + (lane & 31)] : v;
            }
            tile_epilogue<EPI, TOR>(a, s, 32 * i, 32 * nt, lane, HALF ? (1 << sub) : 3);
        }
        __syncthreads();
    }
}
template <int EPI, int MT, int NW, int U, int FT = 1>
MG_DEV void rows_block16(const GemmArgs& a, int bid, char* smem) {
    static_assert(EPI == EPI_PK || EPI == EPI_PK_RELU || EPI == EPI_HEADS || EPI == EPI_PK_SWIGLU || EPI == EPI_F32_STORE,
                  "half-tile form: packed, per-head, SwiGLU and plain fp32 epilogues");
    static_assert(FT == 1 || MT > 1, "both halves per workgroup: several row tiles only");
    const int tid = threadIdx.x, lane = tid & 63, w = tid >> 6;
    const int r16 = lane & 15, kg = lane >> 4;
    const int nt = FT == 2 ? bid : bid >> 1, sub0 = FT == 2 ? 0 : (bid & 1);
    const int kt16 = a.K >> 4, kp = kt16 >> 1;
    const int per = (kp + NW - 1) / NW;
    const int p0 = w * per, p1 = (p0 + per) < kp ? (p0 + per) : kp;
    float* rsl = (float*)(smem + NW * 8 * FT * 64 * sizeof(float));
    const size_t lane_off = (size_t)(kg >> 1) * TILE_BYTES + (size_t)(kg & 1) * 512;
    const char* wp = (const char*)(a.W + pk_tile_off(nt, 0, a.K)) + lane_off + (size_t)(16 * sub0 + r16) * 16;
    const int xkts = a.x_kts ? a.x_kts : kt16;
    const char* xp = (const char*)a.X + (size_t)a.x_k0 * TILE_BYTES + lane_off + (size_t)r16 * 16;
    RsRegs rsr;
    rs_issue(a.rs, a.M, 32 * MT, tid, NW * 64, rsr);
    int p = p0;
    uint4 wf[U][FT];
    constexpr bool XPF = MT == 1;
    uint4 xf[XPF ? U : 1][2];
    if (p + U <= p1) {
#pragma unroll
        for (int u = 0; u < U; ++u)
#pragma unroll
            for (int f = 0; f < FT; ++f) wf[u][f] = ld16_stream(wp + (size_t)(p + u) * (2 * TILE_BYTES) + f * 256);
        if constexpr (XPF) {
#pragma unroll
            for (int u = 0; u < U; ++u) {
                const char* xt = xp + (size_t)(2 * (p + u)) * TILE_BYTES;
                xf[u][0] = ld16(xt); xf[u][1] = ld16(xt + 256);
            }
        }
    }
    rs_finish(a.rs, a.M, 32 * MT, rsl, tid, NW * 64, rsr);
    f32x4 acc[MT][2][FT];
#pragma unroll
    for (int i = 0; i < MT; ++i)
#pragma unroll
        for (int f = 0; f < FT; ++f) { acc[i][0][f] = acc4_zero(); acc[i][1][f] = acc4_zero(); }
    for (bool first = true; p + U <= p1; p += U, first = false) {
        if (!first) {
#pragma unroll
            for (int u = 0; u < U; ++u)
#pragma unroll
                for (int f = 0; f < FT; ++f) wf[u][f] = ld16_stream(wp + (size_t)(p + u) * (2 * TILE_BYTES) + f * 256);
        }
#pragma unroll
        for (int u = 0; u < U; ++u) {
#pragma unroll
            for (int i = 0; i < MT; ++i) {
                const char* xt = xp + ((size_t)i * xkts + 2 * (p + u)) * TILE_BYTES;
                if (XPF && first) {
                    acc[i][0][0] = mfma16(wf[u][0], xf[XPF ? u : 0][0], acc[i][0][0]);
                    acc[i][1][0] = mfma16(wf[u][0], xf[XPF ? u : 0][1], acc[i][1][0]);
                } else {
                    const uint4 xa = ld16(xt), xb = ld16(xt + 256);
#pragma unroll
                    for (int f = 0; f < FT; ++f) {
                        acc[i][0][f] = mfma16(wf[u][f], xa, acc[i][0][f]);
                        acc[i][1][f] = mfma16(wf[u][f], xb, acc[i][1][f]);
                    }
                }
            }
        }
    }
    for (; p < p1; ++p) {
        uint4 w1[FT];
#pragma unroll
        for (int f = 0; f < FT; ++f) w1[f] = ld16_stream(wp + (size_t)p * (2 * TILE_BYTES) + f * 256);
#pragma unroll
        for (int i = 0; i < MT; ++i) {
            const char* xt = xp + ((size_t)i * xkts + 2 * p) * TILE_BYTES;
            const uint4 xa = ld16(xt), xb = ld16(xt + 256);
#pragma unroll
            for (int f = 0; f < FT; ++f) {
                acc[i][0][f] = mfma16(w1[f], xa, acc[i][0][f]);
                acc[i][1][f] = mfma16(w1[f], xb, acc[i][1][f]);
            }
        }
    }
    float* slab = (float*)smem;
#pragma unroll
    for (int i = 0; i < MT; ++i) {
#pragma unroll
        for (int f = 0; f < FT; ++f)
#pragma unroll
            for (int g = 0; g < 2; ++g)
#pragma unroll
                for (int j = 0; j < 4; ++j) slab[(w * 8 * FT + f * 8 + g * 4 + j) * 64 + lane] = acc[i][g][f][j];
        __syncthreads();
#pragma unroll
        for (int g = 0; g < 2; ++g) {
#pragma unroll
          for (int f = 0; f < FT; ++f) {
            if ((((2 * i + g) * FT + f) % NW) == w) {
                const int sub = sub0 + f;
                const int m = 32 * i + 16 * g + r16;
                float v[4];
#pragma unroll
                for (int j = 0; j < 4; ++j) {
                    float t = 0.f;
                    for (int ww = 0; ww < NW; ++ww) t += slab[(ww * 8 * FT + f * 8 + g * 4 + j) * 64 + lane];
                    t *= rsl[32 * i + 16 * g + r16];
                    v[j] = (EPI == EPI_PK_RELU) ? fmaxf(t, 0.f) : t;
                }
                if constexpr (EPI == EPI_F32_STORE) {
                    const int n = nt * 32 + 16 * sub + 4 * kg;
                    if (m < a.M && n < a.N) *(float4*)(a.out_f32 + (size_t)m * a.ldo + n) = make_float4(v[0], v[1], v[2], v[3]);
                    continue;
                }
                if constexpr (EPI == EPI_PK_SWIGLU) {
                    const uint32_t mine = pack_bf16(v[0] / (1.0f + fast_exp(-v[0])) * v[1], v[2] / (1.0f + fast_exp(-v[2])) * v[3]);
                    const uint32_t other = __shfl_xor(mine, 16);
                    const int n = nt * 32 + 16 * sub + 4 * kg;
                    if ((kg & 1) == 0 && m < a.M && n < a.N)
                        *(uint2*)(a.out_pk + pk_off(m, a.out_col0 + (n >> 1), a.out_ld ? a.out_ld : a.N >> 1)) = make_uint2(mine, other);
                    continue;
                }
                const uint32_t lo = pack_bf16(v[0], v[1]), hi = pack_bf16(v[2], v[3]);
                const uint32_t plo = __shfl_xor(lo, 16), phi = __shfl_xor(hi, 16);
                if ((kg & 1) == 0 && m < a.M) {
                    const uint4 ch = make_uint4(lo, hi, plo, phi);
                    const int n = nt * 32 + 16 * sub + 4 * kg;
                    if (n < a.N) {
                        if constexpr (EPI == EPI_HEADS) {
                            const HeadsOut& ho = a.heads;
                            const int ri = n / ho.inner, nn = n - ri * ho.inner;
                            heads_store(ho, ri, nn >> 6, m, nn & 63, ch);
                        } else {
                            st16(a.out_pk + pk_off(m, n, a.N), ch);
                        }
                    }
                }
            }
          }
        }
        __syncthreads();
    }
}
template <int EPI, int NW, int U>
MG_DEV void rows_split_block(const GemmArgs& a, int ht, int g, char* smem) {
    static_assert(EPI == EPI_PK || EPI == EPI_PK_RELU || EPI == EPI_HEADS, "packed / per-head epilogues only");
    const int tid = threadIdx.x, lane = tid & 63, w = tid >> 6;
    const int r16 = lane & 15, kg = lane >> 4;
    const int nt = ht >> 1, sub = ht & 1;
    const int kt16 = a.K >> 4, kp = kt16 >> 1;
    const int per = (kp + NW - 1) / NW;
    const int p0 = w * per, p1 = (p0 + per) < kp ? (p0 + per) : kp;
    float* rsl = (float*)(smem + NW * 4 * 64 * sizeof(float));
    const size_t lane_off = (size_t)(kg >> 1) * TILE_BYTES + (size_t)(kg & 1) * 512;
    const char* wp = (const char*)(a.W + pk_tile_off(nt, 0, a.K)) + lane_off + (size_t)(16 * sub + r16) * 16;
    const char* xp = (const char*)a.X + (size_t)a.x_k0 * TILE_BYTES + lane_off + (size_t)(16 * g + r16) * 16;
    RsRegs rsr;
    rs_issue(a.rs, a.M, 32, tid, NW * 64, rsr);
    int p = p0;
    uint4 wf[U], xf[U];
    const bool full = p + U <= p1;
    if (full) {
#pragma unroll
        for (int u = 0; u < U; ++u) wf[u] = ld16_stream(wp + (size_t)(p + u) * (2 * TILE_BYTES));
#pragma unroll
        for (int u = 0; u < U; ++u) xf[u] = ld16(xp + (size_t)(2 * (p + u)) * TILE_BYTES);
    }
    rs_finish(a.rs, a.M, 32, rsl, tid, NW * 64, rsr);
    f32x4 acc = acc4_zero();
    if (full) {
#pragma unroll
        for (int u = 0; u < U; ++u) acc = mfma16(wf[u], xf[u], acc);
        p += U;
    }
    for (; p < p1; ++p) acc = mfma16(ld16_stream(wp + (size_t)p * (2 * TILE_BYTES)), ld16(xp + (size_t)(2 * p) * TILE_BYTES), acc);
    float* slab = (float*)smem;
#pragma unroll
    for (int j = 0; j < 4; ++j) slab[(w * 4 + j) * 64 + lane] = acc[j];
    __syncthreads();
    if (w == 0) {
        const int m = 16 * g + r16;
        float v[4];
#pragma unroll
        for (int j = 0; j < 4; ++j) {
            float t = 0.f;
            for (int ww = 0; ww < NW; ++ww) t += slab[(ww * 4 + j) * 64 + lane];
            t *= rsl[m];
            v[j] = (EPI == EPI_PK_RELU) ? fmaxf(t, 0.f) : t;
        }
        const uint32_t lo = pack_bf16(v[0], v[1]), hi = pack_bf16(v[2], v[3]);
        const uint32_t plo = __shfl_xor(lo, 16), phi = __shfl_xor(hi, 16);
        if ((kg & 1) == 0 && m < a.M) {
            const uint4 ch = make_uint4(lo, hi, plo, phi);
            const int n = nt * 32 + 16 * sub + 4 * kg;
            if (n < a.N) {
                if constexpr (EPI == EPI_HEADS) {
                    const HeadsOut& ho = a.heads;
                    const int ri = n / ho.inner, nn = n - ri * ho.inner;
                    heads_store(ho, ri, nn >> 6, m, nn & 63, ch);
                } else {
                    st16(a.out_pk + pk_off(m, n, a.N), ch);
                }
            }
        }
    }
}
template <int EPI, int MT, bool HALF, int NW = 4, int FT = 1>
__global__ __launch_bounds__(NW * 64) void gemm_rows_kernel(GemmArgs a) {
    MG_DYN_SMEM(smem);
    if constexpr (HALF && (EPI == EPI_PK || EPI == EPI_PK_RELU || EPI == EPI_HEADS || EPI == EPI_PK_SWIGLU || EPI == EPI_F32_STORE)) rows_block16<EPI, MT, NW, 4, FT>(a, blockIdx.x, smem);
    else rows_block<EPI, MT, HALF, NW, 8>(a, blockIdx.x, smem);
}

template <int EPI, bool HALF, int NW>
__global__ __launch_bounds__(NW * 64) void gemm_rows_split_kernel(GemmArgs a) {
    MG_DYN_SMEM(smem);
    shift_rows<EPI>(a, blockIdx.y);
    if constexpr (HALF && (EPI == EPI_PK || EPI == EPI_PK_RELU || EPI == EPI_HEADS || EPI == EPI_PK_SWIGLU || EPI == EPI_F32_STORE)) rows_block16<EPI, 1, NW, 4>(a, blockIdx.x, smem);
    else rows_block<EPI, 1, HALF, NW, 8>(a, blockIdx.x, smem);
}

static int g_rows_ft2 = [] { const char* e = getenv("MG_ROWS_FT2"); return (e && (e[0] == '0' || e[0] == '1')) ? e[0] - '0' : -1; }();
void gemm_rows_set_ft2(int mode) { g_rows_ft2 = mode < 0 ? -1 : (mode ? 1 : 0); }
static bool rows_ft2(const GemmArgs& a) { return g_rows_ft2 < 0 ? a.both_halves != 0 : g_rows_ft2 != 0; }
template <int EPI>
static void gemm_rows_mt(const GemmArgs& a, int mt, bool half, mgStream_t stream) {
    const int NW = half ? 8 : 4;
    const int mts = rows_split_tiles(mt, (size_t)a.N * a.K);
    const bool split = mts < mt;
    const dim3 grid(((a.N + 31) / 32) * (half ? 2 : 1), split ? (mt + mts - 1) / mts : 1), block(NW * 64);
    if (split) mt = mts;
    const size_t sh = (size_t)NW * 16 * 64 * sizeof(float) + (size_t)32 * mt * sizeof(float);
    if (split) {
        if (half) MG_LAUNCH((gemm_rows_split_kernel<EPI, true, 8>), grid, block, sh, stream, a);
        else MG_LAUNCH((gemm_rows_split_kernel<EPI, false, 4>), grid, block, sh, stream, a);
        return;
    }
    if constexpr (EPI == EPI_PK || EPI == EPI_PK_RELU || EPI == EPI_HEADS || EPI == EPI_F32_STORE) {
        if (half && mt >= 3 && rows_ft2(a) && (a.N % 32) == 0) {
            const dim3 grid2((a.N + 31) / 32);
#define MG_GR2(MTV) case MTV: MG_LAUNCH((gemm_rows_kernel<EPI, MTV, true, 8, 2>), grid2, block, sh, stream, a); return;
            switch (mt) { MG_GR2(3) MG_GR2(4) MG_GR2(5) MG_GR2(6) MG_GR2(7) MG_GR2(8) default: break; }
#undef MG_GR2
        }
    }
#define MG_GR(MTV)                                                                                   \
    case MTV:                                                                                        \
        if (half) MG_LAUNCH((gemm_rows_kernel<EPI, MTV, true, 8>), grid, block, sh, stream, a);      \
        else MG_LAUNCH((gemm_rows_kernel<EPI, MTV, false, 4>), grid, block, sh, stream, a);          \
        break;
    switch (mt) {
        MG_GR(1) MG_GR(2) MG_GR(3) MG_GR(4) MG_GR(5) MG_GR(6) MG_GR(7) MG_GR(8)
        default: break;
    }
#undef MG_GR
}

template <int EPI>
static void gemm_rows_mt_half(const GemmArgs& a, int mt, mgStream_t stream) {
    const int mts = rows_split_tiles(mt, (size_t)a.N * a.K);
    const bool split = mts < mt;
    const dim3 grid(((a.N + 31) / 32) * 2, split ? (mt + mts - 1) / mts : 1), block(8 * 64);
    if (split) mt = mts;
    const size_t sh = (size_t)8 * 16 * 64 * sizeof(float) + (size_t)32 * mt * sizeof(float);
    if (split) { MG_LAUNCH((gemm_rows_split_kernel<EPI, true, 8>), grid, block, sh, stream, a); return; }
#define MG_GR(MTV) case MTV: MG_LAUNCH((gemm_rows_kernel<EPI, MTV, true, 8>), grid, block, sh, stream, a); break;
    switch (mt) {
        MG_GR(1) MG_GR(2) MG_GR(3) MG_GR(4) MG_GR(5) MG_GR(6) MG_GR(7) MG_GR(8)
        default: break;
    }
#undef MG_GR
}

template <int MT>
__global__ __launch_bounds__(256) void gemm_rows_splitk_kernel(const uint16_t* X, const uint16_t* W, float* P, int M, int N, int K, int ldp,
                                                          size_t slab_stride, int KS, RowScale rs, TopOut top) {
    MG_DYN_SMEM(smem);
    const int tid = threadIdx.x, lane = tid & 63, w = tid >> 6;
    float* rsl = (float*)(smem + 4 * 16 * 64 * sizeof(float));
    RsRegs rsr;
    rs_issue(rs, M, 32 * MT, tid, 256, rsr);
    const int ntiles = (N + 31) >> 5;
    const int nt = blockIdx.x % ntiles, ks = blockIdx.x / ntiles;
    const int kt16 = K >> 4;
    const int per_blk = (kt16 + KS - 1) / KS;
    const int kb0 = ks * per_blk, kb1 = (kb0 + per_blk) < kt16 ? (kb0 + per_blk) : kt16;
    const int per = (kb1 - kb0 + 3) >> 2;
    const int k0 = kb0 + w * per, k1 = (k0 + per) < kb1 ? (k0 + per) : kb1;

    f32x16 acc[MT];
#pragma unroll
    for (int i = 0; i < MT; ++i) acc[i] = acc_zero();
    const char* wp = (const char*)(W + pk_tile_off(nt, 0, K)) + lane * 16;
    const char* xp = (const char*)X + lane * 16;
    constexpr int U = MT <= 2 ? 16 : 8;
    int kt = k0;
    uint4 wf[U];
    const bool first_full = kt + U <= k1;
    if (first_full) {
#pragma unroll
        for (int u = 0; u < U; ++u) wf[u] = ld16_stream(wp + (size_t)(kt + u) * TILE_BYTES);
    }
    rs_finish(rs, M, 32 * MT, rsl, tid, 256, rsr);
    for (bool first = true; kt + U <= k1; kt += U, first = false) {
        if (!first) {
#pragma unroll
            for (int u = 0; u < U; ++u) wf[u] = ld16_stream(wp + (size_t)(kt + u) * TILE_BYTES);
        }
#pragma unroll
        for (int u = 0; u < U; ++u) {
#pragma unroll
            for (int i = 0; i < MT; ++i)
                acc[i] = mfma32(ld16(xp + ((size_t)i * kt16 + (kt + u)) * TILE_BYTES), wf[u], acc[i]);
        }
    }
    for (; kt < k1; ++kt) {
        const uint4 wf = ld16_stream(wp + (size_t)kt * TILE_BYTES);
#pragma unroll
        for (int i = 0; i < MT; ++i) acc[i] = mfma32(ld16(xp + ((size_t)i * kt16 + kt) * TILE_BYTES), wf, acc[i]);
    }
    float* slab = (float*)smem;
    float* tl = (float*)(smem + 4 * 16 * 64 * sizeof(float) + 32 * MT * sizeof(float));
    float* out = P + (size_t)ks * slab_stride;
    const int half = lane >> 5, n = nt * 32 + (lane & 31);
#pragma unroll
    for (int i = 0; i < MT; ++i) {
#pragma unroll
        for (int r = 0; r < 16; ++r) slab[(w * 16 + r) * 64 + lane] = acc[i][r];
        __syncthreads();
#pragma unroll
        for (int j = 0; j < 4; ++j) {
            const int r = w * 4 + j;
            float v = slab[(0 * 16 + r) * 64 + lane];
            v += slab[(1 * 16 + r) * 64 + lane];
            v += slab[(2 * 16 + r) * 64 + lane];
            v += slab[(3 * 16 + r) * 64 + lane];
            const int m = 32 * i + acc_row(r, half);
            const float lg = v * rsl[m < M ? m : 0];
            if (m < M && n < N && (!top.ptop || top.write_logits)) out[(size_t)m * ldp + n] = lg;
            if (top.ptop) {
                const bool is_stop = n == top.stop[0] || n == top.stop[1] || n == top.stop[2] || n == top.stop[3];
                if (is_stop && m < M) {
                    const int k = n == top.stop[0] ? 0 : (n == top.stop[1] ? 1 : (n == top.stop[2] ? 2 : 3));
                    top.stopv[(size_t)m * 4 + k] = lg;
                }
                tl[(w * 8 + j * 2 + half) * 33 + (lane & 31)] = (n < N && !is_stop) ? lg : -3.0e38f;
            }
        }
        if (top.ptop) {
            __syncthreads();
            if (lane < 8) {
                const float* rowv = tl + (w * 8 + lane) * 33;
                float b1 = -3.0e38f, b2 = -3.0e38f;
                int i1 = 0x7fffffff;
#pragma unroll
                for (int k = 0; k < 32; ++k) {
                    const float x = rowv[k];
                    if (x > b1) { b2 = b1; b1 = x; i1 = k; }
                    else b2 = fmaxf(b2, x);
                }
                float se = 0.f;
                if (top.lse) {
#pragma unroll
                    for (int k = 0; k < 32; ++k) {
                        const float x = rowv[k];
                        se += x > -3.0e38f ? expf(x - b1) : 0.f;
                    }
                }
                const int jj = lane >> 1, hh = lane & 1;
                const int m = 32 * i + acc_row(w * 4 + jj, hh);
                if (m < M) top.ptop[(size_t)m * ntiles + nt] = make_float4(b1, b2, __int_as_float(b1 > -3.0e38f ? nt * 32 + i1 : 0x7fffffff), se);
            }
        }
        __syncthreads();
    }
}

template <int MT, int NW>
MG_DEV void resid_block(const ResidArgs& a, int bid, char* smem) {
    const int tid = threadIdx.x, lane = tid & 63, w = tid >> 6;
    const int half = lane >> 5, l32 = lane & 31;
    const int nt = bid >> 2, sub = bid & 3;
    const bool wvalid = (l32 >> 3) == sub;
    const uint4 zero4 = make_uint4(0, 0, 0, 0);
    const int M = a.M, N = a.N;
    const int kt16 = a.K >> 4;
    const int per = (kt16 + NW - 1) / NW;
    const int k0 = w * per, k1 = (k0 + per) < kt16 ? (k0 + per) : kt16;
    float* rsl = (float*)(smem + NW * 4 * 64 * sizeof(float));
    const char* wp = (const char*)(a.W + pk_tile_off(nt, 0, a.K)) + lane * 16;
    const int xkts = a.x_kts ? a.x_kts : kt16;
    const char* xp = (const char*)a.X + ((size_t)a.x_k0 * TILE_BYTES + lane * 16);
    constexpr int U = (NW >= 16 && MT <= 2) ? 16 : 8;
    int kt = k0;
    uint4 wf[U];
    const bool first_full = kt + U <= k1;
    if (first_full) {
#pragma unroll
        for (int u = 0; u < U; ++u) wf[u] = wvalid ? ld16_stream(wp + (size_t)(kt + u) * TILE_BYTES) : zero4;
    }
    const int n0 = nt * 32 + sub * 8 + half * 4;
    const int my_i = w < MT ? w : -1;
    float4 h_pre = make_float4(0.f, 0.f, 0.f, 0.f);
    if (my_i >= 0 && 32 * my_i + l32 < M) h_pre = *(const float4*)(a.h + (size_t)(32 * my_i + l32) * N + n0);
    block_row_scales(a.rs, M, 32 * MT, rsl, tid, NW * 64);
    f32x16 acc[MT];
#pragma unroll
    for (int i = 0; i < MT; ++i) acc[i] = acc_zero();
    for (bool first = true; kt + U <= k1; kt += U, first = false) {
        if (!first) {
#pragma unroll
            for (int u = 0; u < U; ++u) wf[u] = wvalid ? ld16_stream(wp + (size_t)(kt + u) * TILE_BYTES) : zero4;
        }
#pragma unroll
        for (int u = 0; u < U; ++u) {
#pragma unroll
            for (int i = 0; i < MT; ++i) acc[i] = mfma32(wf[u], ld16(xp + ((size_t)i * xkts + (kt + u)) * TILE_BYTES), acc[i]);
        }
    }
    for (; kt < k1; ++kt) {
        const uint4 wf = wvalid ? ld16_stream(wp + (size_t)kt * TILE_BYTES) : zero4;
#pragma unroll
        for (int i = 0; i < MT; ++i) acc[i] = mfma32(wf, ld16(xp + ((size_t)i * xkts + kt) * TILE_BYTES), acc[i]);
    }
    float* slab = (float*)smem;
    const int nparts = N >> 3;
    const int x_ld = a.x_ld ? a.x_ld : N, x2_ld = a.x2_ld ? a.x2_ld : N;
#pragma unroll
    for (int i = 0; i < MT; ++i) {
#pragma unroll
        for (int j = 0; j < 4; ++j) {
            float v = 0.f;
#pragma unroll
            for (int r = 0; r < 16; ++r) if (r == 4 * sub + j) v = acc[i][r];
            slab[(w * 4 + j) * 64 + lane] = v;
        }
        __syncthreads();
        if ((i % NW) == w) {
            float v[4];
#pragma unroll
            for (int j = 0; j < 4; ++j) {
                float t = 0.f;
                for (int ww = 0; ww < NW; ++ww) t += slab[(ww * 4 + j) * 64 + lane];
                v[j] = t * rsl[32 * i + l32];
            }
            const int m = 32 * i + l32;
            float ss = 0.f;
            if (m < M) {
                float4 hv = h_pre;
                hv.x += v[0]; hv.y += v[1]; hv.z += v[2]; hv.w += v[3];
                *(float4*)(a.h + (size_t)m * N + n0) = hv;
                ss = (hv.x * hv.x + hv.y * hv.y) + (hv.z * hv.z + hv.w * hv.w);
                if (a.x_pk) {
                    const float4 g = *(const float4*)(a.gain + n0);
                    const float gs = a.gscale;
                    *(uint2*)(a.x_pk + pk_off(m, a.x_col0 + n0, x_ld)) =
                        make_uint2(pack_bf16(hv.x * g.x * gs, hv.y * g.y * gs), pack_bf16(hv.z * g.z * gs, hv.w * g.w * gs));
                }
                if (a.x2_pk)
                    *(uint2*)(a.x2_pk + pk_off(m, a.x2_col0 + n0, x2_ld)) = make_uint2(pack_bf16(hv.x, hv.y), pack_bf16(hv.z, hv.w));
            }
            ss += __shfl_xor(ss, 32);
            if (m < M && half == 0) a.part[(size_t)m * nparts + bid] = ss;
        }
        __syncthreads();
    }
}
template <int MT, int NW, int U, bool TRACE = false, bool F16 = false>
MG_DEV void resid_block16(const ResidArgs& a, int bid, char* smem, long long* trace = nullptr) {
    static_assert(MT <= NW, "at most two finishing units per wave");
    const int tid = threadIdx.x, lane = tid & 63, w = tid >> 6;
    auto stamp = [&](int k) {
#ifndef MG_EMU
        if constexpr (TRACE) { if (lane == 0) trace[((size_t)bid * NW + w) * 8 + k] = (long long)__builtin_readcyclecounter(); }
#endif
        (void)k;
    };
    stamp(0);
    const int r16 = lane & 15, kg = lane >> 4;
    const int nt = F16 ? bid >> 1 : bid >> 2, sub = F16 ? bid & 1 : bid & 3;
    const bool wvalid = F16 || r16 < 8;
    const bool kgvalid = F16 || kg < 2;
    const uint4 zero4 = make_uint4(0, 0, 0, 0);
    const int M = a.M, N = a.N;
    const int kt16 = a.K >> 4, kp = kt16 >> 1;
    const int per = (kp + NW - 1) / NW;
    const int p0 = w * per, p1 = (p0 + per) < kp ? (p0 + per) : kp;
    float* rsl = (float*)(smem + NW * 8 * 64 * sizeof(float));
    const size_t lane_off = (size_t)(kg >> 1) * TILE_BYTES + (size_t)(kg & 1) * 512;
    const char* wp = (const char*)(a.W + pk_tile_off(nt, 0, a.K)) + lane_off + (size_t)((F16 ? 16 : 8) * sub + r16) * 16;
    const int xkts = a.x_kts ? a.x_kts : kt16;
    const char* xp = (const char*)a.X + (size_t)a.x_k0 * TILE_BYTES + lane_off + (size_t)r16 * 16;
    RsRegs rsr;
    rs_issue(a.rs, M, 32 * MT, tid, NW * 64, rsr);
    const int n0 = nt * 32 + sub * (F16 ? 16 : 8) + kg * 4;
    float4 h_pre[2] = {make_float4(0.f, 0.f, 0.f, 0.f), make_float4(0.f, 0.f, 0.f, 0.f)};
#pragma unroll
    for (int q = 0; q < 2; ++q) {
        const int f = w + q * NW;
        if (f < 2 * MT && kgvalid) {
            const int m = 32 * (f >> 1) + 16 * (f & 1) + r16;
            if (m < M) h_pre[q] = *(const float4*)(a.h + (size_t)m * N + n0);
        }
    }
    int p = p0;
    uint4 wf[U];
    constexpr bool XPF = MT == 1 && NW <= 8;
    uint4 xf[XPF ? U : 1][2];
    if (p + U <= p1) {
#pragma unroll
        for (int u = 0; u < U; ++u) wf[u] = wvalid ? ld16_stream(wp + (size_t)(p + u) * (2 * TILE_BYTES)) : zero4;
        if constexpr (XPF) {
#pragma unroll
            for (int u = 0; u < U; ++u) {
                const char* xt = xp + (size_t)(2 * (p + u)) * TILE_BYTES;
                xf[u][0] = ld16(xt); xf[u][1] = ld16(xt + 256);
            }
        }
    }
    stamp(1);
    rs_finish(a.rs, M, 32 * MT, rsl, tid, NW * 64, rsr);
    stamp(2);
    f32x4 acc[MT][2];
#pragma unroll
    for (int i = 0; i < MT; ++i) { acc[i][0] = acc4_zero(); acc[i][1] = acc4_zero(); }
    for (bool first = true; p + U <= p1; p += U, first = false) {
        if (!first) {
#pragma unroll
            for (int u = 0; u < U; ++u) wf[u] = wvalid ? ld16_stream(wp + (size_t)(p + u) * (2 * TILE_BYTES)) : zero4;
        }
#pragma unroll
        for (int u = 0; u < U; ++u) {
#pragma unroll
            for (int i = 0; i < MT; ++i) {
                const char* xt = xp + ((size_t)i * xkts + 2 * (p + u)) * TILE_BYTES;
                if (XPF && first) {
                    acc[i][0] = mfma16(wf[u], xf[XPF ? u : 0][0], acc[i][0]);
                    acc[i][1] = mfma16(wf[u], xf[XPF ? u : 0][1], acc[i][1]);
                } else {
                    acc[i][0] = mfma16(wf[u], ld16(xt), acc[i][0]);
                    acc[i][1] = mfma16(wf[u], ld16(xt + 256), acc[i][1]);
                }
            }
        }
    }
    for (; p < p1; ++p) {
        const uint4 w1 = wvalid ? ld16_stream(wp + (size_t)p * (2 * TILE_BYTES)) : zero4;
#pragma unroll
        for (int i = 0; i < MT; ++i) {
            const char* xt = xp + ((size_t)i * xkts + 2 * p) * TILE_BYTES;
            acc[i][0] = mfma16(w1, ld16(xt), acc[i][0]);
            acc[i][1] = mfma16(w1, ld16(xt + 256), acc[i][1]);
        }
    }
    if constexpr (TRACE) { if (acc[0][0][0] == 123456.f) a.part[0] = 0.f; }
    stamp(3);
    float* slab = (float*)smem;
    const int nparts = N >> 3;
    const int x_ld = a.x_ld ? a.x_ld : N, x2_ld = a.x2_ld ? a.x2_ld : N;
#pragma unroll
    for (int i = 0; i < MT; ++i) {
#pragma unroll
        for (int g = 0; g < 2; ++g)
#pragma unroll
            for (int j = 0; j < 4; ++j) slab[(w * 8 + g * 4 + j) * 64 + lane] = acc[i][g][j];
        __syncthreads();
        stamp(4);
#pragma unroll
        for (int q = 0; q < 2; ++q) {
            const int f = w + q * NW;
            if (f < 2 * MT && (f >> 1) == i) {
                const int g = f & 1;
                const int m = 32 * i + 16 * g + r16;
                float v[4];
#pragma unroll
                for (int j = 0; j < 4; ++j) {
                    float t = 0.f;
                    for (int ww = 0; ww < NW; ++ww) t += slab[(ww * 8 + g * 4 + j) * 64 + lane];
                    v[j] = t * rsl[32 * i + 16 * g + r16];
                }
                float ss = 0.f;
                if (m < M && kgvalid) {
                    float4 hv = h_pre[q];
                    hv.x += v[0]; hv.y += v[1]; hv.z += v[2]; hv.w += v[3];
                    *(float4*)(a.h + (size_t)m * N + n0) = hv;
                    ss = (hv.x * hv.x + hv.y * hv.y) + (hv.z * hv.z + hv.w * hv.w);
                    if (a.x_pk) {
                        const float4 gn = *(const float4*)(a.gain + n0);
                        const float gs = a.gscale;
                        *(uint2*)(a.x_pk + pk_off(m, a.x_col0 + n0, x_ld)) =
                            make_uint2(pack_bf16(hv.x * gn.x * gs, hv.y * gn.y * gs), pack_bf16(hv.z * gn.z * gs, hv.w * gn.w * gs));
                    }
                    if (a.x2_pk)
                        *(uint2*)(a.x2_pk + pk_off(m, a.x2_col0 + n0, x2_ld)) = make_uint2(pack_bf16(hv.x, hv.y), pack_bf16(hv.z, hv.w));
                }
                ss += __shfl_xor(ss, 16);
                if (F16) { if (m < M && (kg & 1) == 0) a.part[(size_t)m * nparts + 2 * bid + (kg >> 1)] = ss; }
                else if (m < M && kg == 0) a.part[(size_t)m * nparts + bid] = ss;
            }
            stamp(5);
        }
        __syncthreads();
    }
    stamp(6);
}
template <int MT, int NW, bool F16 = false>
__global__ __launch_bounds__(NW * 64) void gemm_rows_resid_kernel(ResidArgs a) {
    MG_DYN_SMEM(smem);
    resid_block16<MT, NW, (NW >= 16 ? 8 : 4), false, F16>(a, blockIdx.x, smem);
}

template <int MT, int PER>
__global__ __launch_bounds__(64 * MT) void gemm_rows_resid_mt_kernel(ResidArgs a, int S, int fmode) {
    MG_DYN_SMEM(smem);
    float* rsl = (float*)smem;
    int* flag = (int*)(rsl + 32 * MT);
    const int tid = threadIdx.x, lane = tid & 63, w = tid >> 6;
    const int r16 = lane & 15, kg = lane >> 4;
    const int M = a.M, N = a.N;
    const int bid = blockIdx.x, xcd = bid & 7, j = bid >> 3;
    const int nt = (j / S) * 8 + xcd, s = j - (j / S) * S;
    const int kt16 = a.K >> 4, xkts = a.x_kts ? a.x_kts : kt16;
    const int p0 = s * PER;
    const size_t lane_off = (size_t)(kg >> 1) * TILE_BYTES + (size_t)(kg & 1) * 512;
    const char* wp = (const char*)(a.W + pk_tile_off(nt, 0, a.K)) + lane_off + (size_t)r16 * 16 + (size_t)(2 * p0) * TILE_BYTES;
    const char* xp = (const char*)a.X + ((size_t)a.x_k0 + (size_t)w * xkts + 2 * p0) * TILE_BYTES + lane_off + (size_t)r16 * 16;
    uint4 wf[2][PER], xf[PER][2];
#pragma unroll
    for (int u = 0; u < PER; ++u) {
        wf[0][u] = ld16_stream(wp + (size_t)u * (2 * TILE_BYTES));
        wf[1][u] = ld16_stream(wp + (size_t)u * (2 * TILE_BYTES) + 256);
        xf[u][0] = ld16(xp + (size_t)u * (2 * TILE_BYTES));
        xf[u][1] = ld16(xp + (size_t)u * (2 * TILE_BYTES) + 256);
    }
    f32x4 acc[2][2];
#pragma unroll
    for (int ft = 0; ft < 2; ++ft)
#pragma unroll
        for (int g = 0; g < 2; ++g) acc[ft][g] = acc4_zero();
#pragma unroll
    for (int u = 0; u < PER; ++u)
#pragma unroll
        for (int ft = 0; ft < 2; ++ft)
#pragma unroll
            for (int g = 0; g < 2; ++g) acc[ft][g] = mfma16(wf[ft][u], xf[u][g], acc[ft][g]);
    const int Mp = 32 * MT;
#pragma unroll
    for (int ft = 0; ft < 2; ++ft)
#pragma unroll
        for (int g = 0; g < 2; ++g) {
            float* dst = a.kpart + ((size_t)s * Mp + (size_t)(32 * w + 16 * g + r16)) * N + nt * 32 + 16 * ft + 4 * kg;
            *(float4*)dst = make_float4(acc[ft][g][0], acc[ft][g][1], acc[ft][g][2], acc[ft][g][3]);
        }
    if (fmode == 6) return;
#ifndef MG_EMU
    asm volatile("s_waitcnt vmcnt(0)" ::: "memory");
#endif
    __syncthreads();
    if (tid == 0) {
#ifndef MG_EMU
        __builtin_amdgcn_fence(__ATOMIC_RELEASE, "agent");
        asm volatile("s_waitcnt vmcnt(0)" ::: "memory");
        *flag = __hip_atomic_fetch_add(a.ticket + nt, 1, __ATOMIC_RELAXED, __HIP_MEMORY_SCOPE_AGENT);
#else
        *flag = atomicAdd(a.ticket + nt, 1);
#endif
    }
    __syncthreads();
    if (*flag != S - 1) return;
    if (fmode == 5) { if (tid == 0) a.ticket[nt] = 0; return; }
    if (tid == 0) {
#ifndef MG_EMU
        __builtin_amdgcn_fence(__ATOMIC_ACQUIRE, "agent");
#endif
        a.ticket[nt] = 0;
    }
    __syncthreads();
    block_row_scales(a.rs, M, Mp, rsl, tid, 64 * MT);
    __syncthreads();
    const int nparts = N >> 3;
    const int x_ld = a.x_ld ? a.x_ld : N, x2_ld = a.x2_ld ? a.x2_ld : N;
#pragma unroll
    for (int ft = 0; ft < 2; ++ft)
#pragma unroll
        for (int g = 0; g < 2; ++g) {
            const int m = 32 * w + 16 * g + r16;
            const int n0 = nt * 32 + 16 * ft + 4 * kg;
            const float* src = a.kpart + (size_t)m * N + n0;
            float v[4] = {0.f, 0.f, 0.f, 0.f};
            for (int s0 = 0; s0 < S; s0 += 8) {
                float4 pv[8];
#pragma unroll
                for (int q = 0; q < 8; ++q) pv[q] = *(const float4*)(src + (size_t)(s0 + q < S ? s0 + q : S - 1) * Mp * N);
#pragma unroll
                for (int q = 0; q < 8; ++q)
                    if (s0 + q < S) { v[0] += pv[q].x; v[1] += pv[q].y; v[2] += pv[q].z; v[3] += pv[q].w; }
            }
            const float rs = rsl[m];
#pragma unroll
            for (int q = 0; q < 4; ++q) v[q] *= rs;
            float ss2 = 0.f;
            if (m < M) {
                float4 hv = *(const float4*)(a.h + (size_t)m * N + n0);
                hv.x += v[0]; hv.y += v[1]; hv.z += v[2]; hv.w += v[3];
                *(float4*)(a.h + (size_t)m * N + n0) = hv;
                ss2 = (hv.x * hv.x + hv.y * hv.y) + (hv.z * hv.z + hv.w * hv.w);
                if (a.x_pk) {
                    const float4 gn = *(const float4*)(a.gain + n0);
                    const float gs = a.gscale;
                    *(uint2*)(a.x_pk + pk_off(m, a.x_col0 + n0, x_ld)) =
                        make_uint2(pack_bf16(hv.x * gn.x * gs, hv.y * gn.y * gs), pack_bf16(hv.z * gn.z * gs, hv.w * gn.w * gs));
                }
                if (a.x2_pk)
                    *(uint2*)(a.x2_pk + pk_off(m, a.x2_col0 + n0, x2_ld)) = make_uint2(pack_bf16(hv.x, hv.y), pack_bf16(hv.z, hv.w));
            }
            ss2 += __shfl_xor(ss2, 16);
            if (m < M && (kg & 1) == 0) a.part[(size_t)m * nparts + 2 * (2 * nt + ft) + (kg >> 1)] = ss2;
        }
}

__global__ __launch_bounds__(256) void gemm_rows_resid_merge_kernel(ResidArgs a, int S, int Mp) {
    MG_DYN_SMEM(smem);
    float* rsl = (float*)smem;
    const int tid = threadIdx.x, lane = tid & 63, wv = tid >> 6;
    const int r16 = lane & 15, kg = lane >> 4;
    const int ft = wv >> 1, g = wv & 1;
    const int nt = blockIdx.x, w = blockIdx.y;
    const int M = a.M, N = a.N;
    const int m = 32 * w + 16 * g + r16;
    const int n0 = nt * 32 + 16 * ft + 4 * kg;
    const float* src = a.kpart + (size_t)m * N + n0;
    float4 pv[16];
#pragma unroll
    for (int q = 0; q < 16; ++q) pv[q] = *(const float4*)(src + (size_t)(q < S ? q : S - 1) * Mp * N);
    float4 hv = make_float4(0.f, 0.f, 0.f, 0.f);
    if (m < M) hv = *(const float4*)(a.h + (size_t)m * N + n0);
    {
        RowScale rs = a.rs;
        if (rs.part) rs.part += (size_t)32 * w * rs.nparts;
        block_row_scales(rs, M - 32 * w, 32, rsl, tid, 256);
    }
    __syncthreads();
    float v[4] = {0.f, 0.f, 0.f, 0.f};
#pragma unroll
    for (int q = 0; q < 16; ++q)
        if (q < S) { v[0] += pv[q].x; v[1] += pv[q].y; v[2] += pv[q].z; v[3] += pv[q].w; }
    const float rs = rsl[16 * g + r16];
#pragma unroll
    for (int q = 0; q < 4; ++q) v[q] *= rs;
    const int nparts = N >> 3;
    const int x_ld = a.x_ld ? a.x_ld : N, x2_ld = a.x2_ld ? a.x2_ld : N;
    float ss2 = 0.f;
    if (m < M) {
        hv.x += v[0]; hv.y += v[1]; hv.z += v[2]; hv.w += v[3];
        *(float4*)(a.h + (size_t)m * N + n0) = hv;
        ss2 = (hv.x * hv.x + hv.y * hv.y) + (hv.z * hv.z + hv.w * hv.w);
        if (a.x_pk) {
            const float4 gn = *(const float4*)(a.gain + n0);
            const float gs = a.gscale;
            *(uint2*)(a.x_pk + pk_off(m, a.x_col0 + n0, x_ld)) =
                make_uint2(pack_bf16(hv.x * gn.x * gs, hv.y * gn.y * gs), pack_bf16(hv.z * gn.z * gs, hv.w * gn.w * gs));
        }
        if (a.x2_pk)
            *(uint2*)(a.x2_pk + pk_off(m, a.x2_col0 + n0, x2_ld)) = make_uint2(pack_bf16(hv.x, hv.y), pack_bf16(hv.z, hv.w));
    }
    ss2 += __shfl_xor(ss2, 16);
    if (m < M && (kg & 1) == 0) a.part[(size_t)m * nparts + 2 * (2 * nt + ft) + (kg >> 1)] = ss2;
}

template <int NW>
__global__ __launch_bounds__(NW * 64) void gemm_rows_resid_rowsplit_kernel(ResidArgs a) {
    MG_DYN_SMEM(smem);
    shift_rows(a, blockIdx.y);
    resid_block16<1, NW, (NW >= 16 ? 8 : 4)>(a, blockIdx.x, smem);
}

template <int NW, int U>
__global__ __launch_bounds__(NW * 64) void gemm_rows_resid_split_kernel(ResidArgs a) {
    MG_DYN_SMEM(smem);
    const int tid = threadIdx.x, lane = tid & 63, w = tid >> 6;
    const int r16 = lane & 15, kg = lane >> 4;
    const int bid = blockIdx.x;
    const int g = (bid >> 3) & 1, slice = (bid >> 4) * 8 + (bid & 7);
    const int nt = slice >> 2, sub = slice & 3;
    const bool wvalid = r16 < 8;
    const uint4 zero4 = make_uint4(0, 0, 0, 0);
    const int M = a.M, N = a.N;
    const int kt16 = a.K >> 4, kp = kt16 >> 1;
    const int per = (kp + NW - 1) / NW;
    const int p0 = w * per, p1 = (p0 + per) < kp ? (p0 + per) : kp;
    float* rsl = (float*)(smem + NW * 4 * 64 * sizeof(float));
    const size_t lane_off = (size_t)(kg >> 1) * TILE_BYTES + (size_t)(kg & 1) * 512;
    const char* wp = (const char*)(a.W + pk_tile_off(nt, 0, a.K)) + lane_off + (size_t)(8 * sub + r16) * 16;
    const int xkts = a.x_kts ? a.x_kts : kt16;
    (void)xkts;
    const char* xp = (const char*)a.X + (size_t)a.x_k0 * TILE_BYTES + lane_off + (size_t)(16 * g + r16) * 16;
    RsRegs rsr;
    rs_issue(a.rs, M, 32, tid, NW * 64, rsr);
    const int n0 = nt * 32 + sub * 8 + kg * 4;
    const int m = 16 * g + r16;
    float4 h_pre = make_float4(0.f, 0.f, 0.f, 0.f);
    if (w == 0 && kg < 2 && m < M) h_pre = *(const float4*)(a.h + (size_t)m * N + n0);
    int p = p0;
    uint4 wf[U];
    if (p + U <= p1) {
#pragma unroll
        for (int u = 0; u < U; ++u) wf[u] = wvalid ? ld16_stream(wp + (size_t)(p + u) * (2 * TILE_BYTES)) : zero4;
    }
    rs_finish(a.rs, M, 32, rsl, tid, NW * 64, rsr);
    f32x4 acc = acc4_zero();
    for (bool first = true; p + U <= p1; p += U, first = false) {
        if (!first) {
#pragma unroll
            for (int u = 0; u < U; ++u) wf[u] = wvalid ? ld16_stream(wp + (size_t)(p + u) * (2 * TILE_BYTES)) : zero4;
        }
#pragma unroll
        for (int u = 0; u < U; ++u) acc = mfma16(wf[u], ld16(xp + (size_t)(2 * (p + u)) * TILE_BYTES), acc);
    }
    for (; p < p1; ++p) {
        const uint4 w1 = wvalid ? ld16_stream(wp + (size_t)p * (2 * TILE_BYTES)) : zero4;
        acc = mfma16(w1, ld16(xp + (size_t)(2 * p) * TILE_BYTES), acc);
    }
    float* slab = (float*)smem;
#pragma unroll
    for (int j = 0; j < 4; ++j) slab[(w * 4 + j) * 64 + lane] = acc[j];
    __syncthreads();
    if (w == 0) {
        float v[4];
#pragma unroll
        for (int j = 0; j < 4; ++j) {
            float t = 0.f;
            for (int ww = 0; ww < NW; ++ww) t += slab[(ww * 4 + j) * 64 + lane];
            v[j] = t * rsl[m];
        }
        const int nparts = N >> 3;
        const int x_ld = a.x_ld ? a.x_ld : N, x2_ld = a.x2_ld ? a.x2_ld : N;
        float ss = 0.f;
        if (m < M && kg < 2) {
            float4 hv = h_pre;
            hv.x += v[0]; hv.y += v[1]; hv.z += v[2]; hv.w += v[3];
            *(float4*)(a.h + (size_t)m * N + n0) = hv;
            ss = (hv.x * hv.x + hv.y * hv.y) + (hv.z * hv.z + hv.w * hv.w);
            if (a.x_pk) {
                const float4 gn = *(const float4*)(a.gain + n0);
                const float gs = a.gscale;
                *(uint2*)(a.x_pk + pk_off(m, a.x_col0 + n0, x_ld)) =
                    make_uint2(pack_bf16(hv.x * gn.x * gs, hv.y * gn.y * gs), pack_bf16(hv.z * gn.z * gs, hv.w * gn.w * gs));
            }
            if (a.x2_pk)
                *(uint2*)(a.x2_pk + pk_off(m, a.x2_col0 + n0, x2_ld)) = make_uint2(pack_bf16(hv.x, hv.y), pack_bf16(hv.z, hv.w));
        }
        ss += __shfl_xor(ss, 16);
        if (m < M && kg == 0) a.part[(size_t)m * nparts + slice] = ss;
    }
}

#ifdef MG_TOOLS
__global__ __launch_bounds__(1024) void gemm_rows_resid_trace_kernel(ResidArgs a, long long* trace) {
    MG_DYN_SMEM(smem);
    resid_block16<1, 16, 8, true>(a, blockIdx.x, smem, trace);
}
void gemm_rows_resid_trace(const ResidArgs& r, long long* trace, mgStream_t stream) {
    const size_t sh = (size_t)16 * 8 * 64 * sizeof(float) + 32 * sizeof(float);
    MG_LAUNCH(gemm_rows_resid_trace_kernel, dim3(r.N / 8), dim3(1024), sh, stream, r, trace);
}
#endif

static std::atomic<int> g_resid_f16{1};
static std::atomic<int> g_rows_mt{0};
void gemm_rows_set_mt(int on) { g_rows_mt = on; }
void gemm_rows_set_resid_f16(int on) { g_resid_f16 = on; }
void gemm_rows_resid(const ResidArgs& r, mgStream_t stream) {
    int mt = (r.M + 31) / 32;
    const int mts = rows_split_tiles(mt, (size_t)r.N * r.K);
    const bool split = mts < mt;
    const dim3 grid(r.N / 8, split ? (mt + mts - 1) / mts : 1);
    if (split) mt = mts;
    const bool wide = r.K > 2048 && mt <= (r.wide_tiles > 4 ? r.wide_tiles : 4);
    if (wide && mt == 1 && !split && r.M > 16 && ((r.N >> 3) & 7) == 0 && r.x_kts == 0) {
        const size_t shs = (size_t)16 * 4 * 64 * sizeof(float) + 32 * sizeof(float);
        MG_LAUNCH((gemm_rows_resid_split_kernel<16, 8>), dim3(2 * (r.N >> 3)), dim3(1024), shs, stream, r);
        return;
    }
    const int NW = wide ? 16 : 8;
    const dim3 block(NW * 64);
    const size_t sh = (size_t)NW * 8 * 64 * sizeof(float) + (size_t)32 * mt * sizeof(float);
    if (split) {
        if (wide) MG_LAUNCH((gemm_rows_resid_rowsplit_kernel<16>), grid, block, sh, stream, r);
        else MG_LAUNCH((gemm_rows_resid_rowsplit_kernel<8>), grid, block, sh, stream, r);
        return;
    }
    { static bool env_read = false; if (!env_read) { env_read = true; if (const char* e = getenv("MG_ROWS_MT")) g_rows_mt = atoi(e); } }
    static int alone_env = -1;
    if (alone_env < 0) { const char* e = getenv("MG_ROWS_MT_ALONE"); alone_env = e ? atoi(e) : 0; }
    const int rows_mt = g_rows_mt ? g_rows_mt.load() : ((r.alone && alone_env && mt >= 4) ? 2 : 0);
    if (r.kpart && r.ticket && mt >= 2 && !split && (r.N & 255) == 0 && rows_mt) {
        const int NWf = wide ? 16 : 8, kp = r.K >> 5, per = (kp + NWf - 1) / NWf;
        if (per * NWf == kp && (per == 8 || per == 4 || per == 2)) {
            const int S = NWf;
            static int fmode = -1;
            if (fmode < 0) { const char* e = getenv("MG_MT_FENCE"); fmode = e ? atoi(e) : 0; }
            const dim3 gridk((r.N / 32) * S), blockk(64 * mt);
            const size_t shk = (size_t)32 * mt * sizeof(float) + 16;
            const bool two = rows_mt == 2 && S <= 16;
            const int fm = two ? 6 : fmode;
#define MG_RMT(MTV)                                                                                   \
    case MTV:                                                                                         \
        if (per == 8) MG_LAUNCH((gemm_rows_resid_mt_kernel<MTV, 8>), gridk, blockk, shk, stream, r, S, fm);       \
        else if (per == 4) MG_LAUNCH((gemm_rows_resid_mt_kernel<MTV, 4>), gridk, blockk, shk, stream, r, S, fm);  \
        else MG_LAUNCH((gemm_rows_resid_mt_kernel<MTV, 2>), gridk, blockk, shk, stream, r, S, fm);                \
        break;
            switch (mt) { MG_RMT(2) MG_RMT(3) MG_RMT(4) MG_RMT(5) MG_RMT(6) MG_RMT(7) MG_RMT(8) default: break; }
#undef MG_RMT
            if (two) MG_LAUNCH(gemm_rows_resid_merge_kernel, dim3(r.N / 32, mt), dim3(256), 32 * sizeof(float), stream, r, S, 32 * mt);
            return;
        }
    }
    const bool f16 = mt >= 2 && (r.N & 15) == 0 && g_resid_f16;
    const dim3 grid16(r.N / 16);
#define MG_RR(MTV)                                                                                 \
    case MTV:                                                                                      \
        if (f16 && wide) MG_LAUNCH((gemm_rows_resid_kernel<MTV, 16, true>), grid16, block, sh, stream, r);   \
        else if (f16) MG_LAUNCH((gemm_rows_resid_kernel<MTV, 8, true>), grid16, block, sh, stream, r);       \
        else if (wide) MG_LAUNCH((gemm_rows_resid_kernel<MTV, 16>), grid, block, sh, stream, r);   \
        else MG_LAUNCH((gemm_rows_resid_kernel<MTV, 8>), grid, block, sh, stream, r);              \
        break;
    switch (mt) {
        MG_RR(1) MG_RR(2) MG_RR(3) MG_RR(4) MG_RR(5) MG_RR(6) MG_RR(7) MG_RR(8)
        default: break;
    }
#undef MG_RR
}
void gemm_rows_resid(const uint16_t* X, const uint16_t* W, float* h, const float* gain, float gscale, uint16_t* x_pk, float* part,
                     int M, int N, int K, const RowScale& rs, mgStream_t stream) {
    ResidArgs r{};
    r.X = X; r.W = W; r.h = h; r.gain = gain; r.gscale = gscale; r.x_pk = x_pk; r.part = part; r.M = M; r.N = N; r.K = K; r.rs = rs;
    gemm_rows_resid(r, stream);
}

template <int EPI>
__global__ __launch_bounds__(512) void gemm_rows_pair_split_kernel(ResidArgs r, GemmArgs g, int nres) {
    MG_DYN_SMEM(smem);
    if ((int)blockIdx.x < nres) { resid_block16<1, 8, 4>(r, blockIdx.x, smem); return; }
    const int u = (int)blockIdx.x - nres;
    rows_split_block<EPI, 8, 8>(g, (u >> 4) * 8 + (u & 7), (u >> 3) & 1, smem);
}
template <int EPI, int MT, bool HALF, bool F16 = false, int FT = 1>
__global__ __launch_bounds__(512) void gemm_rows_pair_kernel(ResidArgs r, GemmArgs g, int nres) {
    MG_DYN_SMEM(smem);
    if ((int)blockIdx.x < nres) resid_block16<MT, 8, 4, false, F16>(r, blockIdx.x, smem);
    else if constexpr (HALF) rows_block16<EPI, MT, 8, 8, FT>(g, (int)blockIdx.x - nres, smem);
    else rows_block<EPI, MT, false, 8, 16>(g, (int)blockIdx.x - nres, smem);
}
void gemm_rows_pair(const ResidArgs& r, const GemmArgs& g, int epi, mgStream_t stream) {
    const int mt = (r.M + 31) / 32;
    const bool full = g.N >= 2048 && epi != EPI_F32_STORE;
    const int nhalf = (g.N + 15) / 16;
    if (!full && mt == 1 && r.M > 16 && (nhalf & 7) == 0 && (r.N & 63) == 0 && epi == EPI_HEADS) {
        const int nres_s = r.N / 8;
        const size_t shs = (size_t)8 * 8 * 64 * sizeof(float) + 32 * sizeof(float);
        MG_LAUNCH((gemm_rows_pair_split_kernel<EPI_HEADS>), dim3(nres_s + 2 * nhalf), dim3(512), shs, stream, r, g, nres_s);
        return;
    }
    const bool f16 = mt >= 2 && (r.N & 15) == 0 && g_resid_f16;
    const bool ft2 = !full && mt >= 3 && rows_ft2(g) && (g.N % 32) == 0 && epi == EPI_HEADS && f16;
    const int nres = f16 ? r.N / 16 : r.N / 8, nrows = ((g.N + 31) / 32) * ((full || ft2) ? 1 : 2);
    const dim3 grid(nres + nrows), block(512);
    const size_t sh = (size_t)8 * 16 * 64 * sizeof(float) + (size_t)32 * mt * sizeof(float);
    if (ft2) {
#define MG_RPF(MTV) case MTV: MG_LAUNCH((gemm_rows_pair_kernel<EPI_HEADS, MTV, true, true, 2>), grid, block, sh, stream, r, g, nres); return;
        switch (mt) { MG_RPF(3) MG_RPF(4) MG_RPF(5) MG_RPF(6) MG_RPF(7) MG_RPF(8) default: break; }
#undef MG_RPF
    }
#define MG_RP2(MTV, FV)                                                                                              \
        if (epi == EPI_PK_RELU && full) MG_LAUNCH((gemm_rows_pair_kernel<EPI_PK_RELU, MTV, false, FV>), grid, block, sh, stream, r, g, nres); \
        else if (epi == EPI_PK_RELU) MG_LAUNCH((gemm_rows_pair_kernel<EPI_PK_RELU, MTV, true, FV>), grid, block, sh, stream, r, g, nres); \
        else if (epi == EPI_F32_STORE) MG_LAUNCH((gemm_rows_pair_kernel<EPI_F32_STORE, MTV, true, FV>), grid, block, sh, stream, r, g, nres); \
        else MG_LAUNCH((gemm_rows_pair_kernel<EPI_HEADS, MTV, true, FV>), grid, block, sh, stream, r, g, nres);
#define MG_RP(MTV)                                                                                                   \
    case MTV:                                                                                                        \
        if (f16) { MG_RP2(MTV, true) } else { MG_RP2(MTV, false) }                                                   \
        break;
    switch (mt) {
        MG_RP(1) MG_RP(2) MG_RP(3) MG_RP(4) MG_RP(5) MG_RP(6) MG_RP(7) MG_RP(8)
        default: break;
    }
#undef MG_RP2
#undef MG_RP
}

__global__ __launch_bounds__(256) void unpack_weight_kernel(const uint16_t* W, float* out, int N, int K) {
    const size_t n_el = (size_t)N * K;
    for (size_t i = (size_t)blockIdx.x * blockDim.x + threadIdx.x; i < n_el; i += (size_t)gridDim.x * blockDim.x) {
        const int n = (int)(i / K), k = (int)(i - (size_t)n * K);
        out[i] = bf16_to_f32(W[pk_off(n, k, K)]);
    }
}
void unpack_weight(const uint16_t* W_pk, float* out, int N, int K, mgStream_t stream) {
    MG_LAUNCH(unpack_weight_kernel, dim3(1024), dim3(256), 0, stream, W_pk, out, N, K);
}
__global__ __launch_bounds__(256) void gemm_f32_scaled_kernel(const float* A, const float* gain, const float* B, float* C, int N, int K,
                                                         int J, int ldc) {
    MG_DYN_SMEM(smem);
    float* As = (float*)smem;
    float* Bs = As + 32 * 33;
    const int tx = threadIdx.x & 15, ty = threadIdx.x >> 4;
    const int tiles_j = (J + 31) / 32;
    const int n0 = (blockIdx.x / tiles_j) * 32, j0 = (blockIdx.x % tiles_j) * 32;
    float c00 = 0.f, c01 = 0.f, c10 = 0.f, c11 = 0.f;
    for (int k0 = 0; k0 < K; k0 += 32) {
        for (int e = threadIdx.x; e < 1024; e += 256) {
            const int r = e >> 5, c = e & 31;
            const int n = n0 + r, k = k0 + c;
            As[r * 33 + c] = (n < N && k < K) ? A[(size_t)n * K + k] * gain[k] : 0.f;
            const int kb = k0 + r, j = j0 + c;
            Bs[r * 33 + c] = (kb < K && j < J) ? B[(size_t)kb * J + j] : 0.f;
        }
        __syncthreads();
        for (int kk = 0; kk < 32; ++kk) {
            const float a0 = As[(2 * ty) * 33 + kk], a1 = As[(2 * ty + 1) * 33 + kk];
            const float b0 = Bs[kk * 33 + 2 * tx], b1 = Bs[kk * 33 + 2 * tx + 1];
            c00 += a0 * b0; c01 += a0 * b1; c10 += a1 * b0; c11 += a1 * b1;
        }
        __syncthreads();
    }
    const int n = n0 + 2 * ty, j = j0 + 2 * tx;
    if (n < N && j < J) C[(size_t)n * ldc + j] = c00;
    if (n < N && j + 1 < J) C[(size_t)n * ldc + j + 1] = c01;
    if (n + 1 < N && j < J) C[(size_t)(n + 1) * ldc + j] = c10;
    if (n + 1 < N && j + 1 < J) C[(size_t)(n + 1) * ldc + j + 1] = c11;
}
void gemm_f32_scaled(const float* A, const float* gain, const float* B, float* C, int N, int K, int J, int ldc, mgStream_t stream) {
    const int blocks = ((N + 31) / 32) * ((J + 31) / 32);
    MG_LAUNCH(gemm_f32_scaled_kernel, dim3(blocks), dim3(256), 2 * 32 * 33 * sizeof(float), stream, A, gain, B, C, N, K, J, ldc);
}
__global__ __launch_bounds__(256) void scale_cols_f32_kernel(const float* A, const float* gain, float* C, int N, int J, int ldc) {
    const size_t n_el = (size_t)N * J;
    for (size_t i = (size_t)blockIdx.x * blockDim.x + threadIdx.x; i < n_el; i += (size_t)gridDim.x * blockDim.x) {
        const int n = (int)(i / J), j = (int)(i - (size_t)n * J);
        C[(size_t)n * ldc + j] = A[i] * gain[j];
    }
}
void scale_cols_f32(const float* A, const float* gain, float* C, int N, int J, int ldc, mgStream_t stream) {
    MG_LAUNCH(scale_cols_f32_kernel, dim3(1024), dim3(256), 0, stream, A, gain, C, N, J, ldc);
}

int splitk_factor(int N, int K) {
    const int ntiles = (N + 31) / 32;
    int ks = (320 + ntiles - 1) / ntiles;
    const int ks_max = K / 64;
    if (ks > ks_max) ks = ks_max;
    if (ks > 16) ks = 16;
    if (ks < 1) ks = 1;
    return ks;
}

void gemm_rows_splitk(const uint16_t* X, const uint16_t* W, float* P, int M, int N, int K, int ldp, size_t slab_stride, int KS,
                      const RowScale& rs, mgStream_t stream, const TopOut* top_in) {
    TopOut top{};
    if (top_in && KS == 1) top = *top_in;
    const int mt = (M + 31) / 32;
    const dim3 grid(((N + 31) / 32) * KS), block(256);
    const size_t sh = (size_t)4 * 16 * 64 * sizeof(float) + (size_t)32 * mt * sizeof(float) + (top.ptop ? (size_t)4 * 8 * 33 * sizeof(float) : 0);
    switch (mt) {
        case 1: MG_LAUNCH((gemm_rows_splitk_kernel<1>), grid, block, sh, stream, X, W, P, M, N, K, ldp, slab_stride, KS, rs, top); break;
        case 2: MG_LAUNCH((gemm_rows_splitk_kernel<2>), grid, block, sh, stream, X, W, P, M, N, K, ldp, slab_stride, KS, rs, top); break;
        case 3: MG_LAUNCH((gemm_rows_splitk_kernel<3>), grid, block, sh, stream, X, W, P, M, N, K, ldp, slab_stride, KS, rs, top); break;
        case 4: MG_LAUNCH((gemm_rows_splitk_kernel<4>), grid, block, sh, stream, X, W, P, M, N, K, ldp, slab_stride, KS, rs, top); break;
        case 5: MG_LAUNCH((gemm_rows_splitk_kernel<5>), grid, block, sh, stream, X, W, P, M, N, K, ldp, slab_stride, KS, rs, top); break;
        case 6: MG_LAUNCH((gemm_rows_splitk_kernel<6>), grid, block, sh, stream, X, W, P, M, N, K, ldp, slab_stride, KS, rs, top); break;
        case 7: MG_LAUNCH((gemm_rows_splitk_kernel<7>), grid, block, sh, stream, X, W, P, M, N, K, ldp, slab_stride, KS, rs, top); break;
        case 8: MG_LAUNCH((gemm_rows_splitk_kernel<8>), grid, block, sh, stream, X, W, P, M, N, K, ldp, slab_stride, KS, rs, top); break;
        default: break;
    }
}

void gemm_rows(const GemmArgs& a_in, int epi, mgStream_t stream) {
#ifdef MG_TOOLS
    GemmArgs a = a_in;
    {
        static int wi = -1;
        if (wi < 0) { const char* e = getenv("MG_WHATIF_KV"); wi = e ? atoi(e) : 0; }
        if (wi && epi == EPI_HEADS) {
            for (int ri = 0; ri < 3; ++ri)
                if (a.heads.fmt[ri] == HF_STEP_KV) {
                    if (wi == 1) a.heads.fmt[ri] = HF_NONE;
                    else { a.heads.pos_rows = nullptr; a.heads.pos_dev = nullptr; a.heads.pos = 0; }
                }
        }
    }
#else
    const GemmArgs& a = a_in;
#endif
    const int mt = (a.M + 31) / 32;
    if (mt > 8) {
        gemm(a, epi, stream);
        return;
    }
    const bool half = (epi == EPI_PK_RELU || epi == EPI_PK || epi == EPI_HEADS) && ((a.N + 31) / 32) < 256 && (a.N % 16) == 0;
    switch (epi) {
        case EPI_F32_STORE:
            gemm_rows_mt<EPI_F32_STORE>(a, mt, !a.bias && ((a.N + 31) / 32) < 128 && (a.N % 16) == 0 && (a.ldo % 4) == 0, stream); break;
        case EPI_F32_RESID: gemm_rows_mt<EPI_F32_RESID>(a, mt, false, stream); break;
        case EPI_PK_RELU: gemm_rows_mt<EPI_PK_RELU>(a, mt, half, stream); break;
        case EPI_PK: gemm_rows_mt<EPI_PK>(a, mt, half, stream); break;
        case EPI_PK_SWIGLU: gemm_rows_mt_half<EPI_PK_SWIGLU>(a, mt, stream); break;
        default: gemm_rows_mt<EPI_HEADS>(a, mt, half, stream); break;
    }
}

}
```

markushgrapher_amd/csrc/k_gemm_epi.h:

```cpp
#pragma once
#include "mg_kernels.h"
#include <type_traits>

namespace mg {

MG_DEV void block_row_scales(const RowScale& rs, int M, int nrows, float* out, int tid, int nthreads) {
    for (int base = 0; base < nrows; base += nthreads >> 3) {
        const int row = base + (tid >> 3), j = tid & 7;
        float s = 0.f;
        if (rs.part && row < nrows) {
            const int mr = row < M ? row : M - 1;
            const int per = rs.nparts >> 3;
            const float* p = rs.part + (size_t)mr * rs.nparts + j * per;
            if ((per & 3) == 0) {
                for (int i = 0; i < per; i += 4) { const float4 a = *(const float4*)(p + i); s += (a.x + a.y) + (a.z + a.w); }
            } else {
                for (int i = 0; i < per; ++i) s += p[i];
            }
        }
        s = sum8(s);
        if (j == 0 && row < nrows) out[row] = rs.part ? rsqrtf(s * rs.inv_d + rs.eps) : 1.0f;
    }
}

struct RsRegs { float4 v[4]; bool fast; };
MG_DEV void rs_issue(const RowScale& rs, int M, int nrows, int tid, int nthreads, RsRegs& r) {
    const int per = rs.nparts >> 3;
    r.fast = rs.part && nrows <= (nthreads >> 3) && per <= 16 && (per & 3) == 0;
#pragma unroll
    for (int i = 0; i < 4; ++i) r.v[i] = make_float4(0.f, 0.f, 0.f, 0.f);
    if (r.fast) {
        const int row = tid >> 3, j = tid & 7;
        if (row < nrows) {
            const int mr = row < M ? row : M - 1;
            const float* p = rs.part + (size_t)mr * rs.nparts + j * per;
#pragma unroll
            for (int i = 0; i < 4; ++i)
                if (4 * i < per) r.v[i] = *(const float4*)(p + 4 * i);
        }
    }
}
MG_DEV void rs_finish(const RowScale& rs, int M, int nrows, float* out, int tid, int nthreads, const RsRegs& r) {
    if (!r.fast) { block_row_scales(rs, M, nrows, out, tid, nthreads); return; }
    float s = 0.f;
#pragma unroll
    for (int i = 0; i < 4; ++i) s += (r.v[i].x + r.v[i].y) + (r.v[i].z + r.v[i].w);
    s = sum8(s);
    const int row = tid >> 3;
    if ((tid & 7) == 0 && row < nrows) out[row] = rsqrtf(s * rs.inv_d + rs.eps);
}

MG_DEV void heads_store(const HeadsOut& ho, int ri, int h, int m, int dim0, const uint4& c) {
    const int fmt = ho.fmt[ri];
    uint16_t* base = ho.ptr[ri];
    if (fmt == HF_PK_ROWS) {
        const int b = m / ho.S_in, s = m - b * ho.S_in + ho.s_off;
        size_t off = (((size_t)b * ho.H + h) * (size_t)(ho.S_cap >> 5) + (size_t)(s >> 5)) * (4 * TILE_ELEMS) +
                     (size_t)(dim0 >> 4) * TILE_ELEMS + (size_t)(((dim0 >> 3) & 1) * 256 + (s & 31) * 8);
        st16(base + off, c);
    } else if (fmt == HF_PK_T) {
        const int b = m / ho.S_in, s = m - b * ho.S_in + ho.s_off;
        size_t off = ((((size_t)b * ho.H + h) * 2 + (size_t)(dim0 >> 5)) * (size_t)(ho.S_cap >> 4) + (size_t)(s >> 4)) *
                         TILE_ELEMS +
                     (size_t)(((s >> 3) & 1) * 256 + (dim0 & 31) * 8);
        st16(base + off, c);
    } else if (fmt == HF_NATURAL) {
        const int b = m / ho.S_in, s = m - b * ho.S_in;
        const int row = ho.row_map ? ho.row_map[m] : s;
        if (row >= 0) st16(base + (((size_t)b * ho.H + h) * (size_t)ho.S_cap + (size_t)row) * 64 + dim0, c);
    } else if (fmt == HF_STEP_Q) {
        st16(base + ((size_t)m * ho.H + h) * 64 + dim0, c);
    } else if (fmt == HF_STEP_KV) {
        const int row = ho.row_map ? ho.row_map[m] : m;
        const int pos = ho.pos_rows ? ho.pos_rows[m] : (ho.pos_dev ? *ho.pos_dev : ho.pos);
        st16_stream(base + (((size_t)row * ho.H + h) * (size_t)ho.S_cap + (size_t)pos) * 64 + dim0, c);
    }
}

MG_DEV float row_scale_of(const RowScale& rs, int m, int M) {
    if (!rs.part) return 1.0f;
    const int mr = m < M ? m : M - 1;
    const float* p = rs.part + (size_t)mr * rs.nparts;
    float s = 0.f;
    for (int i = 0; i < rs.nparts; i += 4) { const float4 v = *(const float4*)(p + i); s += (v.x + v.y) + (v.z + v.w); }
    return rsqrtf(s * rs.inv_d + rs.eps);
}

template <int NT>
MG_DEV void row_scales_tiles(const RowScale& rs, const int (&mrow)[NT], int M, int lane, float (&out)[NT]) {
#pragma unroll
    for (int i = 0; i < NT; ++i) out[i] = 1.0f;
    if (!rs.part) return;
    float s[NT];
#pragma unroll
    for (int i = 0; i < NT; ++i) s[i] = 0.f;
    for (int g0 = 0; g0 < rs.nparts; g0 += 16) {
        float4 v[NT][4];
#pragma unroll
        for (int i = 0; i < NT; ++i) {
            int m = mrow[i] + (lane & 31);
            m = m < M ? m : M - 1;
            const float* p = rs.part + (size_t)m * rs.nparts;
#pragma unroll
            for (int k = 0; k < 4; ++k) v[i][k] = *(const float4*)(p + (g0 + 4 * k < rs.nparts ? g0 + 4 * k : rs.nparts - 4));
        }
#pragma unroll
        for (int i = 0; i < NT; ++i) {
#pragma unroll
            for (int k = 0; k < 4; ++k) s[i] += (g0 + 4 * k < rs.nparts) ? (v[i][k].x + v[i][k].y) + (v[i][k].z + v[i][k].w) : 0.f;
        }
    }
#pragma unroll
    for (int i = 0; i < NT; ++i) out[i] = rsqrtf(s[i] * rs.inv_d + rs.eps);
}

MG_DEV float gelu_erf(float x) {
    const float z = fabsf(x) * 0.70710678118654752f;
    const float t = 1.0f / (1.0f + 0.3275911f * z);
    const float poly = ((((1.061405429f * t - 1.453152027f) * t + 1.421413741f) * t - 0.284496736f) * t + 0.254829592f) * t;
    const float e = 1.0f - poly * fast_exp(-z * z);
    return 0.5f * x * (1.0f + (x < 0.f ? -e : e));
}

template <int EPI, bool TOR, bool APPLY_RS = false>
MG_DEV void tile_epilogue(const GemmArgs& a, const f32x16& acc_in, int m0, int n0, int lane, int qmask = 3, float rsl = 1.0f) {
    const int half = lane >> 5, l32 = lane & 31;
    f32x16 acc = acc_in;
    if constexpr (APPLY_RS && (EPI == EPI_PK || EPI == EPI_PK_RELU || EPI == EPI_PK_GELU || EPI == EPI_HEADS || EPI == EPI_PK_BIAS || EPI == EPI_PK_GELU_ERF)) {
        if (a.rs.part) {
            if (TOR) {
#pragma unroll
                for (int r = 0; r < 16; ++r) acc[r] *= rsl;
            } else {
#pragma unroll
                for (int r = 0; r < 16; ++r) acc[r] *= __shfl(rsl, acc_row(r, half));
            }
        }
    }
    if constexpr (EPI == EPI_F32_STORE || EPI == EPI_F32_RESID) {
        static_assert(!TOR, "fp32 epilogues use D = X·W^T");
        const int n = n0 + l32;
        if (n >= a.N) return;
        const float bv = (EPI == EPI_F32_STORE && a.bias) ? a.bias[n] : 0.f;
#pragma unroll
        for (int r = 0; r < 16; ++r) {
            const int m = m0 + acc_row(r, half);
            if (m < a.M) {
                float* p = a.out_f32 + (size_t)m * a.ldo + n;
                if (EPI == EPI_F32_RESID) *p = *p + acc[r];
                else *p = acc[r] + bv;
            }
        }
    } else if constexpr (EPI == EPI_PK || EPI == EPI_PK_RELU || EPI == EPI_PK_GELU || EPI == EPI_PK_BIAS || EPI == EPI_PK_GELU_ERF) {
        f32x16 v = acc;
        if constexpr (EPI == EPI_PK_BIAS || EPI == EPI_PK_GELU_ERF || EPI == EPI_PK_GELU) {
            static_assert(TOR, "bias epilogues use D = W·X^T (a lane owns a token, its registers are output features)");
            if (a.bias) {
#pragma unroll
                for (int g = 0; g < 4; ++g) {
                    const int n = n0 + 8 * g + 4 * half;
                    const float4 bv = *(const float4*)(a.bias + (n + 3 < a.N ? n : 0));
                    v[4 * g] += bv.x; v[4 * g + 1] += bv.y; v[4 * g + 2] += bv.z; v[4 * g + 3] += bv.w;
                }
            }
            if constexpr (EPI == EPI_PK_GELU_ERF) {
#pragma unroll
                for (int r = 0; r < 16; ++r) v[r] = gelu_erf(v[r]);
            }
        }
        if (EPI == EPI_PK_RELU) {
#pragma unroll
            for (int r = 0; r < 16; ++r) v[r] = fmaxf(v[r], 0.f);
        }
        if (EPI == EPI_PK_GELU) {
#pragma unroll
            for (int r = 0; r < 16; ++r) {
                const float x = v[r], u = 0.7978845608028654f * (x + 0.044715f * x * x * x);
                v[r] = x / (1.0f + fast_exp(-2.0f * u));
            }
        }
        uint4 ch[2];
        acc_to_chunks(v, half, ch);
        const int m = m0 + l32;
#pragma unroll
        for (int q = 0; q < 2; ++q) {
            const int n = n0 + 16 * q + 8 * half;
            if (m < a.M && n < a.N && ((qmask >> q) & 1)) st16(a.out_pk + pk_off(m, n, a.N), ch[q]);
        }
    } else {
        const HeadsOut& ho = a.heads;
        uint4 ch[2];
        acc_to_chunks(acc, half, ch);
        if (TOR) {
            const int m = m0 + l32;
#pragma unroll
            for (int q = 0; q < 2; ++q) {
                const int n = n0 + 16 * q + 8 * half;
                if (m < a.M && n < a.N && ((qmask >> q) & 1)) {
                    const int ri = n / ho.inner, nn = n - ri * ho.inner;
                    heads_store(ho, ri, nn >> 6, m, nn & 63, ch[q]);
                }
            }
        } else {
            const int n = n0 + l32;
#pragma unroll
            for (int q = 0; q < 2; ++q) {
                const int m = m0 + 16 * q + 8 * half;
                if (m < a.M && n < a.N) {
                    const int ri = n / ho.inner, nn = n - ri * ho.inner;
                    heads_store(ho, ri, nn >> 6, m, nn & 63, ch[q]);
                }
            }
        }
    }
}

MG_DEV void resid_norm_epilogue(const GemmArgs& a, const f32x16& acc0, const f32x16& acc1, int m0, int n0, int lane) {
    const int half = lane >> 5, l32 = lane & 31, m = m0 + l32;
    const bool row_ok = m < a.M;
    float ss = 0.f;
#pragma unroll
    for (int j = 0; j < 2; ++j) {
        const f32x16& acc = j ? acc1 : acc0;
        const int nj = n0 + 32 * j;
        if (nj >= a.N) continue;
        f32x16 xg;
#pragma unroll
        for (int g = 0; g < 4; ++g) {
            const int n = nj + 8 * g + 4 * half;
            float* p = a.out_f32 + ht_off(row_ok ? m : 0, n, a.N);
            float4 hv = *(const float4*)p;
            hv.x += acc[4 * g]; hv.y += acc[4 * g + 1]; hv.z += acc[4 * g + 2]; hv.w += acc[4 * g + 3];
            if (row_ok) { *(float4*)p = hv; ss += (hv.x * hv.x + hv.y * hv.y) + (hv.z * hv.z + hv.w * hv.w); }
            if (a.gain) {
                const float4 gn = *(const float4*)(a.gain + n);
                xg[4 * g] = hv.x * gn.x; xg[4 * g + 1] = hv.y * gn.y; xg[4 * g + 2] = hv.z * gn.z; xg[4 * g + 3] = hv.w * gn.w;
            }
        }
        if (a.gain) {
            uint4 ch[2];
            acc_to_chunks(xg, half, ch);
#pragma unroll
            for (int q = 0; q < 2; ++q)
                if (row_ok) st16(a.out_pk + pk_off(m, nj + 16 * q + 8 * half, a.N), ch[q]);
        }
    }
    if (a.part) {
        ss += __shfl_xor(ss, 32);
        if (half == 0 && row_ok && n0 < a.N) a.part[(size_t)m * a.ldo + (n0 >> 6)] = ss;
    }
}

template <int TI, bool staged>
MG_DEV void resid_norm_epilogue_tiles(const GemmArgs& a, f32x16 (&acc)[TI][2], const int (&mrow)[TI], int n0, int lane, mg_lds_t gl) {
    const int half = lane >> 5, l32 = lane & 31;
    const bool col_ok[2] = {n0 < a.N, n0 + 32 < a.N};
    auto hbase = [&](int i, int j) -> float* {
        const int m = mrow[i] + l32;
        return a.out_f32 + ht_off(m < a.M ? m : 0, (col_ok[j] ? n0 + 32 * j : 0) + 4 * half, a.N);
    };
    mg_raw16 h[8];
    auto issue = [&](int i) {
#pragma unroll
        for (int j = 0; j < 2; ++j) {
            const float* b = hbase(i, j);
            gld16_async_off<0>(h[j * 4 + 0], b);
            gld16_async_off<1024>(h[j * 4 + 1], b);
            gld16_async_off<2048>(h[j * 4 + 2], b);
            gld16_async_off<3072>(h[j * 4 + 3], b);
        }
    };
    issue(0);
#pragma unroll
    for (int i = 0; i < TI; ++i) {
        MG_WAIT_VMCNT_TIE4(0, h[0], h[1], h[2], h[3]);
        MG_TIE(h[4]); MG_TIE(h[5]); MG_TIE(h[6]); MG_TIE(h[7]);
#pragma unroll
        for (int j = 0; j < 2; ++j)
#pragma unroll
            for (int g = 0; g < 4; ++g) {
                const uint4 r = raw16_get(h[j * 4 + g]);
                f32x16& ac = acc[i][j];
                ac[4 * g] += __uint_as_float(r.x); ac[4 * g + 1] += __uint_as_float(r.y);
                ac[4 * g + 2] += __uint_as_float(r.z); ac[4 * g + 3] += __uint_as_float(r.w);
            }
        MG_TIE(acc[i][0]); MG_TIE(acc[i][1]);
        if (i + 1 < TI) issue(i + 1);
        const int m = mrow[i] + l32;
        const bool row_ok = m < a.M;
        float ss = 0.f;
#pragma unroll
        for (int j = 0; j < 2; ++j) {
            if (!col_ok[j]) continue;
            const f32x16& ac = acc[i][j];
            float* const hb = hbase(i, j);
            f32x16 xg;
            const mg_lds_t ga = gl + (32 * j + 4 * half) * 4;
#pragma unroll
            for (int g = 0; g < 4; ++g) {
                const float4 hv = make_float4(ac[4 * g], ac[4 * g + 1], ac[4 * g + 2], ac[4 * g + 3]);
                if (row_ok) { *(float4*)(hb + g * 256) = hv; ss += (hv.x * hv.x + hv.y * hv.y) + (hv.z * hv.z + hv.w * hv.w); }
                if (a.gain) {
                    float4 gv;
                    if (staged) {
                        mg_raw16 gr;
                        if (g == 0) lds_rd16_async<0>(gr, ga); else if (g == 1) lds_rd16_async<32>(gr, ga);
                        else if (g == 2) lds_rd16_async<64>(gr, ga); else lds_rd16_async<96>(gr, ga);
                        MG_WAIT_LGKM_TIE(0, gr);
                        const uint4 r = raw16_get(gr);
                        gv = make_float4(__uint_as_float(r.x), __uint_as_float(r.y), __uint_as_float(r.z), __uint_as_float(r.w));
                    } else {
                        gv = *(const float4*)(a.gain + n0 + 32 * j + 8 * g + 4 * half);
                    }
                    xg[4 * g] = hv.x * gv.x; xg[4 * g + 1] = hv.y * gv.y; xg[4 * g + 2] = hv.z * gv.z; xg[4 * g + 3] = hv.w * gv.w;
                }
            }
            if (a.gain) {
                uint4 ch[2];
                acc_to_chunks(xg, half, ch);
                uint16_t* const pb = a.out_pk + pk_off(m, n0 + 32 * j + 8 * half, a.N);
#pragma unroll
                for (int q = 0; q < 2; ++q)
                    if (row_ok) st16(pb + q * TILE_ELEMS, ch[q]);
            }
        }
        if (a.part) {
            ss += __shfl_xor(ss, 32);
            if (half == 0 && row_ok && col_ok[0]) a.part[(size_t)m * a.ldo + (n0 >> 6)] = ss;
        }
    }
}

MG_DEV bool heads_region_is_T(const HeadsOut& ho, int n) {
    const int ri = n / ho.inner;
    return ho.fmt[ri] == HF_PK_T;
}


template <int EPI, int TI, int XP = 0, bool GAIN_LDS = false>
MG_DEV void xl_epilogue(const GemmArgs& a, f32x16 (&acc)[TI][2], const int (&mrow)[TI], int n0w, bool tor, int lane, mg_lds_t gain_lds = mg_lds_t()) {
    if constexpr (EPI == EPI_RESID_NORM) {
        resid_norm_epilogue_tiles<TI, GAIN_LDS>(a, acc, mrow, n0w, lane, gain_lds);
        return;
    }
    float rsv[TI];
    row_scales_tiles<TI>(a.rs, mrow, a.M, lane, rsv);
    if constexpr (EPI == EPI_HEADS) {
        if (tor) {
#pragma unroll
            for (int i = 0; i < TI; ++i)
#pragma unroll
                for (int j = 0; j < 2; ++j) tile_epilogue<EPI_HEADS, true, true>(a, acc[i][j], mrow[i], n0w + 32 * j, lane, 3, rsv[i]);
// ... 26 lines not shown
```

markushgrapher_amd/csrc/mg_kernels.h:

```cpp
#pragma once
#include "mg_device.h"

namespace mg {

enum GemmEpi : int {
    EPI_F32_STORE = 0,
    EPI_F32_RESID = 1,
    EPI_PK_RELU = 2,
    EPI_PK = 3,
    EPI_HEADS = 4,
    EPI_RESID_NORM = 5,
    EPI_PK_SWIGLU = 6,
    EPI_PK_GELU = 7,
    EPI_PK_BIAS = 8,
    EPI_PK_GELU_ERF = 9,
};
enum HeadFmt : int {
    HF_NONE = 0,
    HF_PK_ROWS = 1,
    HF_PK_T = 2,
    HF_NATURAL = 3,
    HF_STEP_Q = 4,
    HF_STEP_KV = 5,
};
struct HeadsOut {
    uint16_t* ptr[3];
    int fmt[3];
    int inner;
    int H;
    int S_in;
    int S_cap;
    const int* row_map;
    int s_off;
    int pos;
    const int* pos_dev;
    const int* pos_rows;
};
struct RowScale {
    const float* part;
    int nparts;
    float inv_d, eps;
};
struct GemmArgs {
    const uint16_t* X;
    const uint16_t* W;
    int M, N, K;
    float* out_f32;
    int ldo;
    const float* bias;
    uint16_t* out_pk;
    HeadsOut heads;
    RowScale rs;
    const float* gain;
    float* part;
    int x_kts, x_k0;
    int out_ld, out_col0;
    const int* row_tiles;
    const int* n_row_tiles;
    int both_halves;
    int pp_colgroup;
    int pp_balance;
    int pp_part, pp_parts;
};
void gemm(const GemmArgs& a, int epi, mgStream_t stream);
bool gemm_has_gelu_epilogue(int M, int N);
bool gemm_pp(const GemmArgs& a, int epi, int ti, mgStream_t stream);
void gemm_pp_set_parts(int mode);
void gemm_set_variant(int v);

void gemm_rows(const GemmArgs& a, int epi, mgStream_t stream);
void gemm_rows_set_resid_f16(int on);
void gemm_rows_set_mt(int on);
void gemm_rows_set_ft2(int mode);
void gemm_rows_set_split(int mode);

int splitk_factor(int N, int K);
struct TopOut {
    float4* ptop;
    float* stopv;
    int stop[4];
    int write_logits;
    int lse;
};
void gemm_rows_splitk(const uint16_t* X, const uint16_t* W, float* P, int M, int N, int K, int ldp, size_t slab_stride, int KS,
                      const RowScale& rs, mgStream_t stream, const TopOut* top = nullptr);
void gemm_rows_resid(const uint16_t* X, const uint16_t* W, float* h, const float* gain, float gscale, uint16_t* x_pk, float* part,
                     int M, int N, int K, const RowScale& rs, mgStream_t stream);
struct ResidArgs {
    const uint16_t* X;
    int x_kts, x_k0;
    const uint16_t* W;
    float* h;
    const float* gain;
    float gscale;
    uint16_t* x_pk;
    int x_ld, x_col0;
    uint16_t* x2_pk;
    int x2_ld, x2_col0;
    float* part;
    int M, N, K;
    RowScale rs;
    int alone;
    int wide_tiles;
    float* kpart;
    int* ticket;
};
void gemm_rows_resid(const ResidArgs& r, mgStream_t stream);
void gemm_rows_resid_trace(const ResidArgs& r, long long* trace, mgStream_t stream);
void gemm_rows_pair(const ResidArgs& r, const GemmArgs& g, int epi, mgStream_t stream);
void unpack_weight(const uint16_t* W_pk, float* out, int N, int K, mgStream_t stream);
void gemm_f32_scaled(const float* A, const float* gain, const float* B, float* C, int N, int K, int J, int ldc, mgStream_t stream);
void scale_cols_f32(const float* A, const float* gain, float* C, int N, int J, int ldc, mgStream_t stream);
struct Slabs {
    const float* P;
    int KS, ldp;
    size_t stride;
};

void rmsnorm_pack(const float* h, const float* gain, uint16_t* x_pk, float* out_f32, int M, int d, float eps,
                  float scale, mgStream_t stream);
void rmsnorm_pack_tiled(const float* h_tiled, const float* gain, uint16_t* x_pk, float* out_f32, int M, int d, float eps,
                        mgStream_t stream);
void rmsnorm_pack_rows(const float* h, const float* gain, uint16_t* x_pk, const int* dst_row, int M, int d, float eps,
                       float scale, mgStream_t stream);
void add_norm_pack(float* h, const Slabs& add, const float* gain, uint16_t* x_pk, int M, int d, float eps, float scale,
                   mgStream_t stream);
void relu_pack(const Slabs& in, uint16_t* y_pk, int M, int N, mgStream_t stream);
void pack_weight(const void* src, int src_is_bf16, int N, int K, uint16_t* dst, int Npad, mgStream_t stream);
void convert_to_f32(const void* src, int src_is_bf16, float* dst, size_t n, mgStream_t stream);
void convert_to_bf16(const void* src, int src_is_bf16, uint16_t* dst, size_t n, mgStream_t stream);
void pack_e1(const float* e1, int B, int M, int M_pad, int d, uint16_t* e1_pk, int* row_map, const uint8_t* enc_mask, int S_cap,
             uint8_t* xmask, mgStream_t stream);
void im2col_pack(const float* pix, uint16_t* x_pk, int B, int C, int I, int ps, mgStream_t stream);

struct EmbedArgs {
    const int64_t* input_ids;
    const float* bbox;
    const uint8_t* attn_mask;
    const float* patch_emb;
    const uint16_t* tok_emb;
    const uint16_t* x_emb;
    const uint16_t* y_emb;
    int B, L, P, d, n_side, M2, V, S_cap;
    float* hidden;
    int hidden_tiled;
    double* cx;
    double* cy;
    uint8_t* mask;
    int* xrow;
    int* xlen;
    int x_row0;
    int trim_padding;
    int* text_len;
    int* err;
};
size_t embed_meta_bytes(int B, int S_cap);
void embed_assemble(const EmbedArgs& a, void* meta_ws, mgStream_t stream);

enum AttnMode : int { ATT_ENC = 0, ATT_DEC_SELF = 1, ATT_CROSS = 2 };
struct AttnArgs {
    const uint16_t* Q;
    const uint16_t* K;
    const uint16_t* Vt;
    uint16_t* ctx;
    int B, H, Sq, Sk, Sq_cap, Sk_cap;
    int mode;
    const uint8_t* kmask;
    const float* tab1;
    const float* tabh;
    const float* tabv;
    const uint16_t* bidx;
    const int* bk1;
    int tab1_len;
    const int* kst;
    const uint8_t* qbv;
    int dbg;
};
void bias_index(uint16_t* out, const double* cx, const double* cy, const uint8_t* kmask, const int* bk1, const int* bkhv, int B,
                int Sk, int S_cap, mgStream_t stream);
void attn_lists(const uint8_t* kmask, int B, int Sk, int S_cap, int* kst, uint8_t* qbv, mgStream_t stream);
void row_tile_list(const uint8_t* kmask, int rows, int* list, int* count, mgStream_t stream);
void attention(const AttnArgs& a, mgStream_t stream);
void attention_set_qt(int qt);

struct AttnStepArgs {
    const uint16_t* q;
    const uint16_t* Kc;
    const uint16_t* Vc;
    uint16_t* ctx;
    int rows, H, group;
    int cap;
    const int* len;
    int n_keys;
    const float* bias;
    const int* anc;
    int t;
    const int* t_dev;
    int t_off;
    RowScale qrs;
    int ctx_ld, ctx_col0;
    Slabs qkv;
    int self_append;
    uint16_t* Kc_w;
    uint16_t* Vc_w;
    struct Rope { const float* qkv; int ld; const float* cs; RowScale rs; float qscale; } rope;
    const int* pos_rows;
    const int* t_off_rows;
    const int* kv_owner;
    int one_wg_per_cu;
    const int* live;
};
void attention_step(const AttnStepArgs& a, mgStream_t stream);
void attention_step_allow_shared();
void attention_step_trace(const AttnStepArgs& a, long long* trace, mgStream_t stream);

struct XAttnArgs {
    const uint16_t* q;
    uint16_t* qx;
    const uint16_t* wk;
    const uint16_t* wv;
    const uint16_t* enc;
    const int* len;
    const int* kv_owner;
    const int* live;
    RowScale qrs;
    uint16_t* part;
    float* ml;
    uint16_t* ctx;
    int ctx_ld, ctx_col0;
    int rows, H, d, cap;
    int nsplit;
    int nstg;
    int nt;
    int group;
    int bpw;
};
bool xattn_supported(int d, int H);
int xattn_nf(int d);
size_t xattn_stream_lds(int d, int nstg);
void xattn_stream_prepare(int d, int nstg);
void xattn_expand(const XAttnArgs& a, mgStream_t stream);
void xattn_stream(const XAttnArgs& a, mgStream_t stream);
void xattn_contract(const XAttnArgs& a, mgStream_t stream);
int xattn_beams_bp(int d, int nstg, int bp);
size_t xattn_beams_lds(int d, int nstg, int bp);
void xattn_beams_prepare(int d);
void xattn_stream_beams(const XAttnArgs& a, mgStream_t stream);
void xattn_pack_weights(const float* wkv_f32, uint16_t* wk, uint16_t* wv, int H, int d, mgStream_t stream);
void enc_rows(const uint16_t* src_pk, const int* row_map, uint16_t* dst, int B, int rows_per_image, int cap, int d, mgStream_t stream);
void enc_pad_rows(uint16_t* dst, const int* len, int B, int cap, int d, mgStream_t stream);

void embed_norm_rows(const int64_t* ids, const uint16_t* tok_emb, float* h, const float* gain, uint16_t* x_pk, uint16_t* x2_pk, int x2_ld,
                     int x2_col0, int rows, int d, int V, int* err, float eps, mgStream_t stream);
void embed_rows(const int64_t* ids, const uint16_t* tok_emb, float* h, int rows, int d, int V, int* err,
                mgStream_t stream, uint16_t* x_pk = nullptr, int x_ld = 0, int x_col0 = 0);

struct SlotTable {
    int* pos;
    int* img;
    int* pool;
    int* ctr;
    int* out_len;
    int pool_cap;
    int start_id;
    const int64_t* first_tok;
    int n_stop, stop[4], max_len;
    int nsamp = 1;
};
struct ArgmaxArgs {
    const float* logits;
    int rows, V, ldl;
    int eos, pad, suppress_eos;
    int n_eos_more, eos_more[3];
    int64_t* next_ids;
    int64_t* out_ids;
    int max_len, pos;
    const int* pos_dev;
    int min_len;
    int* unfinished;
    int* n_unfinished;
    float* top2;
    int* step_ctr;
    SlotTable slots;
    const float4* ptop;
    const float* stopv;
    int ntiles;
    const uint16_t* tok_emb;
    float* h;
    const float* gain;
    uint16_t* x_pk;
    uint16_t* x2_pk;
    int x2_ld, x2_col0, d;
    float eps;
    float* token_scores;
    int ts_ld;
};
void greedy_select(const ArgmaxArgs& a, mgStream_t stream);
void greedy_select_fused(const ArgmaxArgs& a, mgStream_t stream);
struct SampleArgs {
    const float* logits;
    int rows, V, ldl;
    int eos, pad, min_len;
    float temperature;
    int top_k;
    float top_p;
    uint64_t seed;
    const uint64_t* stream_ids;
    int64_t* next_ids;
    int64_t* out_ids;
    int max_len, pos;
    const int* pos_dev;
    int* unfinished;
    int* n_unfinished;
    float* top2;
    int* step_ctr;
    float* token_scores;
    int ts_ld;
    SlotTable slots;
};
bool sample_select_supported(int V);
void sample_select(const SampleArgs& a, mgStream_t stream);
MG_HD void philox4x32_10(uint64_t seed, uint64_t stream_id, uint32_t pos, uint32_t out[4]) {
    uint32_t c0 = (uint32_t)stream_id, c1 = (uint32_t)(stream_id >> 32), c2 = pos, c3 = 0;
    uint32_t k0 = (uint32_t)seed, k1 = (uint32_t)(seed >> 32);
    for (int round = 0; round < 10; ++round) {
        const uint64_t p0 = (uint64_t)0xD2511F53u * c0, p1 = (uint64_t)0xCD9E8D57u * c2;
        const uint32_t n0 = (uint32_t)(p1 >> 32) ^ c1 ^ k0, n2 = (uint32_t)(p0 >> 32) ^ c3 ^ k1;
        c1 = (uint32_t)p1; c3 = (uint32_t)p0; c0 = n0; c2 = n2;
        k0 += 0x9E3779B9u; k1 += 0xBB67AE85u;
    }
    out[0] = c0; out[1] = c1; out[2] = c2; out[3] = c3;
}
void slot_refill(const SlotTable& s, int64_t* next_ids, int* unfinished, int rows, mgStream_t stream);

struct BeamSlots { const int* pos; const int* live; };
size_t beam_state_bytes(int B, int K, int max_len);
void beam_init(void* state, int B, int K, int max_len, int pad, int eos, int start, int64_t* next_ids, int* anc, int T_cap,
               int* counters, mgStream_t stream);
float beam_length_divisor(int cur_len, float length_penalty);
void beam_step(void* state, const float* logits, int ldl, int V, int B, int K, int max_len, int cur_len, const int* tdev,
               const float* div_table, int eos, int min_len, float length_penalty, int early_stopping, int64_t* next_ids,
               int* beam_idx, int* counters, mgStream_t stream, const BeamSlots* slots = nullptr);
struct BeamOut {
    int num_return;
    int* beam_indices;
    float* token_scores;
};
void beam_finalize(void* state, int B, int K, int max_len, int64_t* out_ids, int* out_cols, float* out_scores, mgStream_t stream,
                   const BeamOut* nbest = nullptr);
void beam_reorder_anc(int* anc, const int* beam_idx, int rows, int t_written, const int* tdev, const int* counters, mgStream_t stream,
                      const BeamSlots* slots = nullptr);
void beam_slots_step(void* state, int slots, int K, int max_len, int pad, int eos, int start, int early_stopping, int* pos, int* img, int* pool,
                     int* bpool, int* live, int* assign, int64_t* next_ids, int* anc, int T_cap, int pool_cap, int64_t* out_ids, int* out_len,
                     float* out_scores, int* ctr, bool end_first, mgStream_t stream, const BeamOut* nbest = nullptr);
void beam_reorder_copy(const uint16_t* src, uint16_t* dst, const int* beam_idx, int nlk, int rows, int H, int t_cap, int t_used,
                       mgStream_t stream);

size_t preprocess_scratch_bytes(int B, int Hs, int Ws, int out_size);
void preprocess_pages(const uint8_t* pages, int B, int Hs, int Ws, int out_size, float* pixel_values, void* scratch, mgStream_t stream);


}
```

Baseline: 153.5.

## Add half-size LDS two-round reduction for row GEMMs and multi-pass row-scale prefetch

Adds an optional SMALL mode to the row, pair and residual GEMM kernels. Each M tile's cross-wave reduction goes through LDS in two rounds of half-tiles, which halves the slab shared-memory footprint and is meant to let more blocks fit per CU. The mode is gated by a per-call field, an environment variable and a kind mask, and adds extra barriers per tile. Separately, the row-scale register prefetch now covers multiple passes of rows. This lets larger MT blocks overlap the RMS partial loads with the weight prefetch instead of falling back to the synchronous block_row_scales path.

```diff
diff --git a/include/mgrapher.h b/include/mgrapher.h
--- a/include/mgrapher.h
+++ b/include/mgrapher.h
@@ -136,6 +136,9 @@
 int mgk_set_rows_split(int mode);
 int mgk_set_resid_f16(int on);
 int mgk_set_rows_ft2(int mode);
+int mgk_set_rows_small_lds(int mode);
+long long mgk_rows_lds_bytes(int kind, int mt, int small_lds);
+long long mgk_xattn_stream_lds(int d, int nstg);
 int mgk_set_rows_mt(int on);
 int mgk_set_attention_qt(int qt);
 int mgk_set_pp_parts(int mode);
diff --git a/markushgrapher_amd/csrc/c_ops.hip b/markushgrapher_amd/csrc/c_ops.hip
--- a/markushgrapher_amd/csrc/c_ops.hip
+++ b/markushgrapher_amd/csrc/c_ops.hip
@@ -30,6 +30,9 @@
 int mgk_set_rows_split(int mode) { gemm_rows_set_split(mode); return MG_OK; }
 int mgk_set_resid_f16(int on) { gemm_rows_set_resid_f16(on); return MG_OK; }
 int mgk_set_rows_ft2(int mode) { gemm_rows_set_ft2(mode); return MG_OK; }
+int mgk_set_rows_small_lds(int mode) { gemm_rows_set_small_lds(mode); return MG_OK; }
+long long mgk_rows_lds_bytes(int kind, int mt, int small_lds) { return (kind < 0 || kind >= RL_KINDS || mt < 1 || mt > 8) ? -1 : (long long)gemm_rows_lds_bytes(kind, mt, small_lds); }
+long long mgk_xattn_stream_lds(int d, int nstg) { return (long long)xattn_stream_lds(d, nstg); }
 int mgk_gemm(void* stream, int mode, int epi, const void* X_pk, const void* W_pk, int M, int N, int K, float* out_f32,
              int ldo, const float* bias, void* out_pk) {
     const bool swin_epi = epi == EPI_PK_BIAS || epi == EPI_PK_GELU_ERF;
diff --git a/markushgrapher_amd/csrc/k_gemm.hip b/markushgrapher_amd/csrc/k_gemm.hip
--- a/markushgrapher_amd/csrc/k_gemm.hip
+++ b/markushgrapher_amd/csrc/k_gemm.hip
@@ -498,7 +498,7 @@
     a.M -= 32 * rt;
 }
 
-template <int EPI, int MT, bool HALF, int NW, int U>
+template <int EPI, int MT, bool HALF, int NW, int U, bool SMALL = false>
 MG_DEV void rows_block(const GemmArgs& a, int bid, char* smem) {
     const int tid = threadIdx.x, lane = tid & 63, w = tid >> 6;
     const int nt = HALF ? (bid >> 1) : bid;
@@ -509,10 +509,14 @@
     const int per = (kt16 + NW - 1) / NW;
     const int k0 = w * per, k1 = (k0 + per) < kt16 ? (k0 + per) : kt16;
     constexpr bool TOR = !(EPI == EPI_F32_STORE || EPI == EPI_F32_RESID);
-    float* rsl = (float*)(smem + NW * 16 * 64 * sizeof(float));
+    static_assert(!SMALL || (TOR && !HALF), "two-round exchange: whole tiles, token-major epilogue");
+    float* rsl = (float*)(smem + NW * (SMALL ? 8 : 16) * 64 * sizeof(float));
     const char* wp = (const char*)(a.W + pk_tile_off(nt, 0, a.K)) + lane * 16;
     const int xkts = a.x_kts ? a.x_kts : kt16;
     const char* xp = (const char*)a.X + ((size_t)a.x_k0 * TILE_BYTES + lane * 16);
+    constexpr bool RSPRE = TOR && NW >= 8;
+    RsRegs<RSPRE ? rs_passes(32 * MT, NW * 64, 3) : 1> rsr;
+    if constexpr (RSPRE) rs_issue(a.rs, a.M, 32 * MT, tid, NW * 64, rsr);
     int kt = k0;
     uint4 wf[U];
     const bool first_full = kt + U <= k1;
@@ -520,7 +524,8 @@
 #pragma unroll
         for (int u = 0; u < U; ++u) wf[u] = wvalid ? ld16_stream(wp + (size_t)(kt + u) * TILE_BYTES) : zero4;
     }
-    if (TOR) block_row_scales(a.rs, a.M, 32 * MT, rsl, tid, NW * 64);
+    if constexpr (RSPRE) rs_finish(a.rs, a.M, 32 * MT, rsl, tid, NW * 64, rsr);
+    else if (TOR) block_row_scales(a.rs, a.M, 32 * MT, rsl, tid, NW * 64);
 
     f32x16 acc[MT];
 #pragma unroll
@@ -550,6 +555,27 @@
     float* slab = (float*)smem;
 #pragma unroll
     for (int i = 0; i < MT; ++i) {
+        if constexpr (SMALL) {
+#pragma unroll
+            for (int q = 0; q < 2; ++q) {
+#pragma unroll
+                for (int r = 0; r < 8; ++r) slab[(w * 8 + r) * 64 + lane] = acc[i][8 * q + r];
+                __syncthreads();
+                if (((2 * i + q) % NW) == w) {
+                    f32x16 s = acc_zero();
+#pragma unroll
+                    for (int r = 0; r < 8; ++r) {
+                        float v = 0.f;
+#pragma unroll
+                        for (int ww = 0; ww < NW; ++ww) v += slab[(ww * 8 + r) * 64 + lane];
+                        s[8 * q + r] = v * rsl[32 * i + (lane & 31)];
+                    }
+                    tile_epilogue<EPI, TOR>(a, s, 32 * i, 32 * nt, lane, 1 << q);
+                }
+                __syncthreads();
+            }
+            continue;
+        }
 #pragma unroll
         for (int r = 0; r < 16; ++r) slab[(w * 16 + r) * 64 + lane] = acc[i][r];
         __syncthreads();
@@ -582,7 +608,7 @@
         __syncthreads();
     }
 }
-template <int EPI, int MT, int NW, int U, int FT = 1>
+template <int EPI, int MT, int NW, int U, int FT = 1, bool SMALL = false>
 MG_DEV void rows_block16(const GemmArgs& a, int bid, char* smem) {
     static_assert(EPI == EPI_PK || EPI == EPI_PK_RELU || EPI == EPI_HEADS || EPI == EPI_PK_SWIGLU || EPI == EPI_F32_STORE,
                   "half-tile form: packed, per-head, SwiGLU and plain fp32 epilogues");
@@ -593,12 +619,14 @@
     const int kt16 = a.K >> 4, kp = kt16 >> 1;
     const int per = (kp + NW - 1) / NW;
     const int p0 = w * per, p1 = (p0 + per) < kp ? (p0 + per) : kp;
-    float* rsl = (float*)(smem + NW * 8 * FT * 64 * sizeof(float));
+    constexpr int GS = (SMALL ? 4 : 8) * FT;
+    constexpr int NR = SMALL ? 2 : 1;
+    float* rsl = (float*)(smem + NW * GS * 64 * sizeof(float));
     const size_t lane_off = (size_t)(kg >> 1) * TILE_BYTES + (size_t)(kg & 1) * 512;
     const char* wp = (const char*)(a.W + pk_tile_off(nt, 0, a.K)) + lane_off + (size_t)(16 * sub0 + r16) * 16;
     const int xkts = a.x_kts ? a.x_kts : kt16;
     const char* xp = (const char*)a.X + (size_t)a.x_k0 * TILE_BYTES + lane_off + (size_t)r16 * 16;
-    RsRegs rsr;
+    RsRegs<rs_passes(32 * MT, NW * 64, 4)> rsr;
     rs_issue(a.rs, a.M, 32 * MT, tid, NW * 64, rsr);
     int p = p0;
     uint4 wf[U][FT];
@@ -668,14 +696,19 @@
 #pragma unroll
     for (int i = 0; i < MT; ++i) {
 #pragma unroll
+      for (int rd = 0; rd < NR; ++rd) {
+#pragma unroll
         for (int f = 0; f < FT; ++f)
 #pragma unroll
-            for (int g = 0; g < 2; ++g)
-#pragma unroll
-                for (int j = 0; j < 4; ++j) slab[(w * 8 * FT + f * 8 + g * 4 + j) * 64 + lane] = acc[i][g][f][j];
+            for (int g = 0; g < 2; ++g) {
+                if (SMALL && g != rd) continue;
+#pragma unroll
+                for (int j = 0; j < 4; ++j) slab[(w * GS + f * (GS / FT) + (SMALL ? 0 : g * 4) + j) * 64 + lane] = acc[i][g][f][j];
+            }
         __syncthreads();
 #pragma unroll
         for (int g = 0; g < 2; ++g) {
+          if (SMALL && g != rd) continue;
 #pragma unroll
           for (int f = 0; f < FT; ++f) {
             if ((((2 * i + g) * FT + f) % NW) == w) {
@@ -685,7 +718,7 @@
 #pragma unroll
                 for (int j = 0; j < 4; ++j) {
                     float t = 0.f;
-                    for (int ww = 0; ww < NW; ++ww) t += slab[(ww * 8 * FT + f * 8 + g * 4 + j) * 64 + lane];
+                    for (int ww = 0; ww < NW; ++ww) t += slab[(ww * GS + f * (GS / FT) + (SMALL ? 0 : g * 4) + j) * 64 + lane];
                     t *= rsl[32 * i + 16 * g + r16];
                     v[j] = (EPI == EPI_PK_RELU) ? fmaxf(t, 0.f) : t;
                 }
@@ -721,6 +754,7 @@
           }
         }
         __syncthreads();
+      }
     }
 }
 template <int EPI, int NW, int U>
@@ -736,7 +770,7 @@
     const size_t lane_off = (size_t)(kg >> 1) * TILE_BYTES + (size_t)(kg & 1) * 512;
     const char* wp = (const char*)(a.W + pk_tile_off(nt, 0, a.K)) + lane_off + (size_t)(16 * sub + r16) * 16;
     const char* xp = (const char*)a.X + (size_t)a.x_k0 * TILE_BYTES + lane_off + (size_t)(16 * g + r16) * 16;
-    RsRegs rsr;
+    RsRegs<1> rsr;
     rs_issue(a.rs, a.M, 32, tid, NW * 64, rsr);
     int p = p0;
     uint4 wf[U], xf[U];
@@ -786,11 +820,30 @@
         }
     }
 }
-template <int EPI, int MT, bool HALF, int NW = 4, int FT = 1>
+template <int EPI, int MT, bool HALF, int NW = 4, int FT = 1, bool SMALL = false>
 __global__ __launch_bounds__(NW * 64) void gemm_rows_kernel(GemmArgs a) {
     MG_DYN_SMEM(smem);
-    if constexpr (HALF && (EPI == EPI_PK || EPI == EPI_PK_RELU || EPI == EPI_HEADS || EPI == EPI_PK_SWIGLU || EPI == EPI_F32_STORE)) rows_block16<EPI, MT, NW, 4, FT>(a, blockIdx.x, smem);
+    if constexpr (HALF && (EPI == EPI_PK || EPI == EPI_PK_RELU || EPI == EPI_HEADS || EPI == EPI_PK_SWIGLU || EPI == EPI_F32_STORE)) rows_block16<EPI, MT, NW, 4, FT, SMALL>(a, blockIdx.x, smem);
     else rows_block<EPI, MT, HALF, NW, 8>(a, blockIdx.x, smem);
+}
+
+static int g_rows_small_lds = [] { const char* e = getenv("MG_ROWS_SMALL_LDS"); return (e && (e[0] == '0' || e[0] == '1')) ? e[0] - '0' : -1; }();
+void gemm_rows_set_small_lds(int mode) { g_rows_small_lds = mode < 0 ? -1 : (mode ? 1 : 0); }
+static const int g_rows_small_kinds = [] { const char* e = getenv("MG_ROWS_SMALL_LDS_KINDS"); return e ? atoi(e) : 7; }();
+static bool rows_small(int asked, int mt, int launcher) {
+    return mt >= 3 && (g_rows_small_kinds & launcher) && (g_rows_small_lds < 0 ? asked != 0 : g_rows_small_lds != 0);
+}
+size_t gemm_rows_lds_bytes(int kind, int mt, int small) {
+    const bool sm = small && mt >= 3;
+    int nw = 8, rows = 8;
+    switch (kind) {
+        case RL_ROWS16: case RL_PAIR16: case RL_RESID8: break;
+        case RL_ROWS16_FT2: case RL_PAIR16_FT2: case RL_PAIR32: rows = 16; break;
+        case RL_RESID16: nw = 16; break;
+        case RL_ROWS32: return (size_t)4 * 16 * 64 * sizeof(float) + (size_t)32 * mt * sizeof(float);
+        default: return 0;
+    }
+    return (size_t)nw * (sm ? rows / 2 : rows) * 64 * sizeof(float) + (size_t)32 * mt * sizeof(float);
 }
 
 template <int EPI, bool HALF, int NW>
@@ -811,16 +864,30 @@
     const bool split = mts < mt;
     const dim3 grid(((a.N + 31) / 32) * (half ? 2 : 1), split ? (mt + mts - 1) / mts : 1), block(NW * 64);
     if (split) mt = mts;
-    const size_t sh = (size_t)NW * 16 * 64 * sizeof(float) + (size_t)32 * mt * sizeof(float);
+    const size_t sh = gemm_rows_lds_bytes(half ? RL_ROWS16 : RL_ROWS32, mt, 0);
     if (split) {
         if (half) MG_LAUNCH((gemm_rows_split_kernel<EPI, true, 8>), grid, block, sh, stream, a);
         else MG_LAUNCH((gemm_rows_split_kernel<EPI, false, 4>), grid, block, sh, stream, a);
         return;
     }
+    const bool ft2 = half && mt >= 3 && rows_ft2(a) && (a.N % 32) == 0;
+    if constexpr (EPI == EPI_HEADS) {
+        if (half && rows_small(a.small_lds, mt, 1)) {
+            const size_t shs = gemm_rows_lds_bytes(ft2 ? RL_ROWS16_FT2 : RL_ROWS16, mt, 1);
+            const dim3 grids(ft2 ? (a.N + 31) / 32 : grid.x);
+#define MG_GRS(MTV) case MTV:                                                                                         \
+        if (ft2) MG_LAUNCH((gemm_rows_kernel<EPI, MTV, true, 8, 2, true>), grids, block, shs, stream, a);            \
+        else MG_LAUNCH((gemm_rows_kernel<EPI, MTV, true, 8, 1, true>), grids, block, shs, stream, a);                \
+        return;
+            switch (mt) { MG_GRS(3) MG_GRS(4) MG_GRS(5) MG_GRS(6) MG_GRS(7) MG_GRS(8) default: break; }
+#undef MG_GRS
+        }
+    }
     if constexpr (EPI == EPI_PK || EPI == EPI_PK_RELU || EPI == EPI_HEADS || EPI == EPI_F32_STORE) {
-        if (half && mt >= 3 && rows_ft2(a) && (a.N % 32) == 0) {
+        if (ft2) {
             const dim3 grid2((a.N + 31) / 32);
-#define MG_GR2(MTV) case MTV: MG_LAUNCH((gemm_rows_kernel<EPI, MTV, true, 8, 2>), grid2, block, sh, stream, a); return;
+            const size_t sh2 = gemm_rows_lds_bytes(RL_ROWS16_FT2, mt, 0);
+#define MG_GR2(MTV) case MTV: MG_LAUNCH((gemm_rows_kernel<EPI, MTV, true, 8, 2>), grid2, block, sh2, stream, a); return;
             switch (mt) { MG_GR2(3) MG_GR2(4) MG_GR2(5) MG_GR2(6) MG_GR2(7) MG_GR2(8) default: break; }
 #undef MG_GR2
         }
@@ -843,7 +910,7 @@
     const bool split = mts < mt;
     const dim3 grid(((a.N + 31) / 32) * 2, split ? (mt + mts - 1) / mts : 1), block(8 * 64);
     if (split) mt = mts;
-    const size_t sh = (size_t)8 * 16 * 64 * sizeof(float) + (size_t)32 * mt * sizeof(float);
+    const size_t sh = gemm_rows_lds_bytes(RL_ROWS16, mt, 0);
     if (split) { MG_LAUNCH((gemm_rows_split_kernel<EPI, true, 8>), grid, block, sh, stream, a); return; }
 #define MG_GR(MTV) case MTV: MG_LAUNCH((gemm_rows_kernel<EPI, MTV, true, 8>), grid, block, sh, stream, a); break;
     switch (mt) {
@@ -859,7 +926,7 @@
     MG_DYN_SMEM(smem);
     const int tid = threadIdx.x, lane = tid & 63, w = tid >> 6;
     float* rsl = (float*)(smem + 4 * 16 * 64 * sizeof(float));
-    RsRegs rsr;
+    RsRegs<rs_passes(32 * MT, 256, 8)> rsr;
     rs_issue(rs, M, 32 * MT, tid, 256, rsr);
     const int ntiles = (N + 31) >> 5;
     const int nt = blockIdx.x % ntiles, ks = blockIdx.x / ntiles;
@@ -1047,7 +1114,7 @@
         __syncthreads();
     }
 }
-template <int MT, int NW, int U, bool TRACE = false, bool F16 = false>
+template <int MT, int NW, int U, bool TRACE = false, bool F16 = false, bool SMALL = false>
 MG_DEV void resid_block16(const ResidArgs& a, int bid, char* smem, long long* trace = nullptr) {
     static_assert(MT <= NW, "at most two finishing units per wave");
     const int tid = threadIdx.x, lane = tid & 63, w = tid >> 6;
@@ -1067,12 +1134,13 @@
     const int kt16 = a.K >> 4, kp = kt16 >> 1;
     const int per = (kp + NW - 1) / NW;
     const int p0 = w * per, p1 = (p0 + per) < kp ? (p0 + per) : kp;
-    float* rsl = (float*)(smem + NW * 8 * 64 * sizeof(float));
+    constexpr int GS = SMALL ? 4 : 8, NR = SMALL ? 2 : 1;
+    float* rsl = (float*)(smem + NW * GS * 64 * sizeof(float));
     const size_t lane_off = (size_t)(kg >> 1) * TILE_BYTES + (size_t)(kg & 1) * 512;
     const char* wp = (const char*)(a.W + pk_tile_off(nt, 0, a.K)) + lane_off + (size_t)((F16 ? 16 : 8) * sub + r16) * 16;
     const int xkts = a.x_kts ? a.x_kts : kt16;
     const char* xp = (const char*)a.X + (size_t)a.x_k0 * TILE_BYTES + lane_off + (size_t)r16 * 16;
-    RsRegs rsr;
+    RsRegs<rs_passes(32 * MT, NW * 64, 4)> rsr;
     rs_issue(a.rs, M, 32 * MT, tid, NW * 64, rsr);
     const int n0 = nt * 32 + sub * (F16 ? 16 : 8) + kg * 4;
     float4 h_pre[2] = {make_float4(0.f, 0.f, 0.f, 0.f), make_float4(0.f, 0.f, 0.f, 0.f)};
@@ -1142,22 +1210,26 @@
 #pragma unroll
     for (int i = 0; i < MT; ++i) {
 #pragma unroll
-        for (int g = 0; g < 2; ++g)
-#pragma unroll
-            for (int j = 0; j < 4; ++j) slab[(w * 8 + g * 4 + j) * 64 + lane] = acc[i][g][j];
+      for (int rd = 0; rd < NR; ++rd) {
+#pragma unroll
+        for (int g = 0; g < 2; ++g) {
+            if (SMALL && g != rd) continue;
+#pragma unroll
+            for (int j = 0; j < 4; ++j) slab[(w * GS + (SMALL ? 0 : g * 4) + j) * 64 + lane] = acc[i][g][j];
+        }
         __syncthreads();
         stamp(4);
 #pragma unroll
         for (int q = 0; q < 2; ++q) {
             const int f = w + q * NW;
-            if (f < 2 * MT && (f >> 1) == i) {
+            if (f < 2 * MT && (f >> 1) == i && (!SMALL || (f & 1) == rd)) {
                 const int g = f & 1;
                 const int m = 32 * i + 16 * g + r16;
                 float v[4];
 #pragma unroll
                 for (int j = 0; j < 4; ++j) {
                     float t = 0.f;
-                    for (int ww = 0; ww < NW; ++ww) t += slab[(ww * 8 + g * 4 + j) * 64 + lane];
+                    for (int ww = 0; ww < NW; ++ww) t += slab[(ww * GS + (SMALL ? 0 : g * 4) + j) * 64 + lane];
                     v[j] = t * rsl[32 * i + 16 * g + r16];
                 }
                 float ss = 0.f;
@@ -1182,13 +1254,14 @@
             stamp(5);
         }
         __syncthreads();
+      }
     }
     stamp(6);
 }
-template <int MT, int NW, bool F16 = false>
+template <int MT, int NW, bool F16 = false, bool SMALL = false>
 __global__ __launch_bounds__(NW * 64) void gemm_rows_resid_kernel(ResidArgs a) {
     MG_DYN_SMEM(smem);
-    resid_block16<MT, NW, (NW >= 16 ? 8 : 4), false, F16>(a, blockIdx.x, smem);
+    resid_block16<MT, NW, (NW >= 16 ? 8 : 4), false, F16, SMALL>(a, blockIdx.x, smem);
 }
 
 template <int MT, int PER>
@@ -1376,7 +1449,7 @@
     const int xkts = a.x_kts ? a.x_kts : kt16;
     (void)xkts;
     const char* xp = (const char*)a.X + (size_t)a.x_k0 * TILE_BYTES + lane_off + (size_t)(16 * g + r16) * 16;
-    RsRegs rsr;
+    RsRegs<1> rsr;
     rs_issue(a.rs, M, 32, tid, NW * 64, rsr);
     const int n0 = nt * 32 + sub * 8 + kg * 4;
     const int m = 16 * g + r16;
@@ -1499,6 +1572,15 @@
     }
     const bool f16 = mt >= 2 && (r.N & 15) == 0 && g_resid_f16;
     const dim3 grid16(r.N / 16);
+    if (f16 && rows_small(r.small_lds, mt, 4)) {
+        const size_t shs = gemm_rows_lds_bytes(wide ? RL_RESID16 : RL_RESID8, mt, 1);
+#define MG_RRS(MTV) case MTV:                                                                                \
+        if (wide) MG_LAUNCH((gemm_rows_resid_kernel<MTV, 16, true, true>), grid16, block, shs, stream, r);  \
+        else MG_LAUNCH((gemm_rows_resid_kernel<MTV, 8, true, true>), grid16, block, shs, stream, r);        \
+        return;
+        switch (mt) { MG_RRS(3) MG_RRS(4) MG_RRS(5) MG_RRS(6) MG_RRS(7) MG_RRS(8) default: break; }
+#undef MG_RRS
+    }
 #define MG_RR(MTV)                                                                                 \
     case MTV:                                                                                      \
         if (f16 && wide) MG_LAUNCH((gemm_rows_resid_kernel<MTV, 16, true>), grid16, block, sh, stream, r);   \
@@ -1526,12 +1608,12 @@
     const int u = (int)blockIdx.x - nres;
     rows_split_block<EPI, 8, 8>(g, (u >> 4) * 8 + (u & 7), (u >> 3) & 1, smem);
 }
-template <int EPI, int MT, bool HALF, bool F16 = false, int FT = 1>
+template <int EPI, int MT, bool HALF, bool F16 = false, int FT = 1, bool SMALL = false>
 __global__ __launch_bounds__(512) void gemm_rows_pair_kernel(ResidArgs r, GemmArgs g, int nres) {
     MG_DYN_SMEM(smem);
-    if ((int)blockIdx.x < nres) resid_block16<MT, 8, 4, false, F16>(r, blockIdx.x, smem);
-    else if constexpr (HALF) rows_block16<EPI, MT, 8, 8, FT>(g, (int)blockIdx.x - nres, smem);
-    else rows_block<EPI, MT, false, 8, 16>(g, (int)blockIdx.x - nres, smem);
+    if ((int)blockIdx.x < nres) resid_block16<MT, 8, 4, false, F16, SMALL>(r, blockIdx.x, smem);
+    else if constexpr (HALF) rows_block16<EPI, MT, 8, 8, FT, SMALL>(g, (int)blockIdx.x - nres, smem);
+    else rows_block<EPI, MT, false, 8, 16, SMALL>(g, (int)blockIdx.x - nres, smem);
 }
 void gemm_rows_pair(const ResidArgs& r, const GemmArgs& g, int epi, mgStream_t stream) {
     const int mt = (r.M + 31) / 32;
@@ -1547,7 +1629,19 @@
     const bool ft2 = !full && mt >= 3 && rows_ft2(g) && (g.N % 32) == 0 && epi == EPI_HEADS && f16;
     const int nres = f16 ? r.N / 16 : r.N / 8, nrows = ((g.N + 31) / 32) * ((full || ft2) ? 1 : 2);
     const dim3 grid(nres + nrows), block(512);
-    const size_t sh = (size_t)8 * 16 * 64 * sizeof(float) + (size_t)32 * mt * sizeof(float);
+    const int kind = full ? RL_PAIR32 : (ft2 ? RL_PAIR16_FT2 : RL_PAIR16);
+    const size_t sh = gemm_rows_lds_bytes(kind, mt, 0);
+    if (f16 && (epi == EPI_HEADS || epi == EPI_PK_RELU) && rows_small(r.small_lds | g.small_lds, mt, 2)) {
+        const size_t shs = gemm_rows_lds_bytes(kind, mt, 1);
+#define MG_RPS(MTV) case MTV:                                                                                                              \
+        if (epi == EPI_PK_RELU && full) MG_LAUNCH((gemm_rows_pair_kernel<EPI_PK_RELU, MTV, false, true, 1, true>), grid, block, shs, stream, r, g, nres); \
+        else if (epi == EPI_PK_RELU) MG_LAUNCH((gemm_rows_pair_kernel<EPI_PK_RELU, MTV, true, true, 1, true>), grid, block, shs, stream, r, g, nres);     \
+        else if (ft2) MG_LAUNCH((gemm_rows_pair_kernel<EPI_HEADS, MTV, true, true, 2, true>), grid, block, shs, stream, r, g, nres);       \
+        else MG_LAUNCH((gemm_rows_pair_kernel<EPI_HEADS, MTV, true, true, 1, true>), grid, block, shs, stream, r, g, nres);                \
+        return;
+        switch (mt) { MG_RPS(3) MG_RPS(4) MG_RPS(5) MG_RPS(6) MG_RPS(7) MG_RPS(8) default: break; }
+#undef MG_RPS
+    }
     if (ft2) {
 #define MG_RPF(MTV) case MTV: MG_LAUNCH((gemm_rows_pair_kernel<EPI_HEADS, MTV, true, true, 2>), grid, block, sh, stream, r, g, nres); return;
         switch (mt) { MG_RPF(3) MG_RPF(4) MG_RPF(5) MG_RPF(6) MG_RPF(7) MG_RPF(8) default: break; }
diff --git a/markushgrapher_amd/csrc/k_gemm_epi.h b/markushgrapher_amd/csrc/k_gemm_epi.h
--- a/markushgrapher_amd/csrc/k_gemm_epi.h
+++ b/markushgrapher_amd/csrc/k_gemm_epi.h
@@ -23,31 +23,47 @@
     }
 }
 
-struct RsRegs { float4 v[4]; bool fast; };
-MG_DEV void rs_issue(const RowScale& rs, int M, int nrows, int tid, int nthreads, RsRegs& r) {
-    const int per = rs.nparts >> 3;
-    r.fast = rs.part && nrows <= (nthreads >> 3) && per <= 16 && (per & 3) == 0;
-#pragma unroll
-    for (int i = 0; i < 4; ++i) r.v[i] = make_float4(0.f, 0.f, 0.f, 0.f);
+template <int NP = 1>
+struct RsRegs { float4 v[NP][4]; bool fast; };
+constexpr int rs_passes(int rows, int nthreads, int cap) {
+    const int need = (rows + (nthreads >> 3) - 1) / (nthreads >> 3);
+    return need < 1 ? 1 : (need > cap ? 1 : need);
+}
+template <int NP>
+MG_DEV void rs_issue(const RowScale& rs, int M, int nrows, int tid, int nthreads, RsRegs<NP>& r) {
+    const int per = rs.nparts >> 3, rpp = nthreads >> 3;
+    r.fast = rs.part && nrows <= NP * rpp && per <= 16 && (per & 3) == 0;
+#pragma unroll
+    for (int q = 0; q < NP; ++q)
+#pragma unroll
+        for (int i = 0; i < 4; ++i) r.v[q][i] = make_float4(0.f, 0.f, 0.f, 0.f);
     if (r.fast) {
-        const int row = tid >> 3, j = tid & 7;
-        if (row < nrows) {
-            const int mr = row < M ? row : M - 1;
-            const float* p = rs.part + (size_t)mr * rs.nparts + j * per;
-#pragma unroll
-            for (int i = 0; i < 4; ++i)
-                if (4 * i < per) r.v[i] = *(const float4*)(p + 4 * i);
-        }
-    }
-}
-MG_DEV void rs_finish(const RowScale& rs, int M, int nrows, float* out, int tid, int nthreads, const RsRegs& r) {
+        const int j = tid & 7;
+#pragma unroll
+        for (int q = 0; q < NP; ++q) {
+            const int row = q * rpp + (tid >> 3);
+            if (row < nrows) {
+                const int mr = row < M ? row : M - 1;
+                const float* p = rs.part + (size_t)mr * rs.nparts + j * per;
+#pragma unroll
+                for (int i = 0; i < 4; ++i)
+                    if (4 * i < per) r.v[q][i] = *(const float4*)(p + 4 * i);
+            }
+        }
+    }
+}
+template <int NP>
+MG_DEV void rs_finish(const RowScale& rs, int M, int nrows, float* out, int tid, int nthreads, const RsRegs<NP>& r) {
     if (!r.fast) { block_row_scales(rs, M, nrows, out, tid, nthreads); return; }
-    float s = 0.f;
-#pragma unroll
-    for (int i = 0; i < 4; ++i) s += (r.v[i].x + r.v[i].y) + (r.v[i].z + r.v[i].w);
-    s = sum8(s);
-    const int row = tid >> 3;
-    if ((tid & 7) == 0 && row < nrows) out[row] = rsqrtf(s * rs.inv_d + rs.eps);
+#pragma unroll
+    for (int q = 0; q < NP; ++q) {
+        float s = 0.f;
+#pragma unroll
+        for (int i = 0; i < 4; ++i) s += (r.v[q][i].x + r.v[q][i].y) + (r.v[q][i].z + r.v[q][i].w);
+        s = sum8(s);
+        const int row = q * (nthreads >> 3) + (tid >> 3);
+        if ((tid & 7) == 0 && row < nrows) out[row] = rsqrtf(s * rs.inv_d + rs.eps);
+    }
 }
 
 MG_DEV void heads_store(const HeadsOut& ho, int ri, int h, int m, int dim0, const uint4& c) {
diff --git a/markushgrapher_amd/csrc/mg_kernels.h b/markushgrapher_amd/csrc/mg_kernels.h
--- a/markushgrapher_amd/csrc/mg_kernels.h
+++ b/markushgrapher_amd/csrc/mg_kernels.h
@@ -60,6 +60,7 @@
     int both_halves;
     int pp_colgroup;
     int pp_balance;
+    int small_lds;
     int pp_part, pp_parts;
 };
 void gemm(const GemmArgs& a, int epi, mgStream_t stream);
@@ -72,6 +73,17 @@
 void gemm_rows_set_resid_f16(int on);
 void gemm_rows_set_mt(int on);
 void gemm_rows_set_ft2(int mode);
+void gemm_rows_set_small_lds(int mode);
+enum { RL_ROWS16 = 0,
+       RL_ROWS16_FT2,
+       RL_ROWS32,
+       RL_PAIR16,
+       RL_PAIR16_FT2,
+       RL_PAIR32,
+       RL_RESID8,
+       RL_RESID16,
+       RL_KINDS };
+size_t gemm_rows_lds_bytes(int kind, int mt, int small);
 void gemm_rows_set_split(int mode);
 
 int splitk_factor(int N, int K);
@@ -104,6 +116,7 @@
     int wide_tiles;
     float* kpart;
     int* ticket;
+    int small_lds;
 };
 void gemm_rows_resid(const ResidArgs& r, mgStream_t stream);
 void gemm_rows_resid_trace(const ResidArgs& r, long long* trace, mgStream_t stream);
```

Result: no change. 153.3 (-0.1%).
